# cremebrule/rgb-proprioceptive-pose-estimator

Hardware: AMD Instinct MI355X
Metric: images/sec (train step, 224x224 bs256 per GPU) (higher is better)
Workload: dtype bf16; 1 GPU; NaiveObjectStateEstimator train step (BASELINE.json configs[1]): ResNet-50 trunk + bn1 aux head + proprio MLP [1024,256,64] + PoseDistanceLoss(combined, alpha 0.5) + Adam; model=no, images_per_gpu=256, global_batch=256, resolution=224, latent_dim=512, parallelism=dp1, launch=eager, nan_loss_steps=0, params_finite=True

## Files before the change

### include/rpe_hip.h

```cpp
#ifndef RPE_HIP_H
#define RPE_HIP_H

#ifdef __cplusplus
extern "C" {
#endif

#define RPE_ABI_VERSION 3

enum { RPE_F32 = 0, RPE_BF16 = 1, RPE_F16 = 2 };
enum {
    RPE_OK = 0,
    RPE_ERR_SHAPE = 1,
    RPE_ERR_DTYPE = 2,
    RPE_ERR_ALIGN = 3,
    RPE_ERR_HIP = 4,
    RPE_ERR_WORKSPACE = 5,
    RPE_ERR_STATE = 6
};

int rpe_abi_version(void);
const char* rpe_build_id(void);
const char* rpe_last_error(void);

typedef struct {
// ... 57 lines not shown
                             const float* invstd, const float* mean, const float* c1c2, float* dw, void* scratch, long scratch_bytes, void* stream);
long rpe_conv1x1_dgrad_bn_t_workspace_bytes(const rpe_conv_desc* d, int P);
int rpe_conv1x1_dgrad_bn_t(const rpe_conv_desc* d, int dtype, const void* dy, const void* w_crsk, void* dz, const void* addend, const rpe_bn_bwd_epilogue* bn,
                           const void* a_prev, int P, float* t_out, void* workspace, long workspace_bytes, void* stream);
int rpe_bn_backward_coeffs_t(int dtype, const float* stats_part, int tiles, int C, long rows, const float* dzt_a, const void* w, int Ci, const float* mean,
                             const float* invstd, float* dgamma, float* dbeta, float* c1c2, double* dpart, void* stream);
int rpe_conv1x1_wgrad_combine(const rpe_conv_desc* d, const float* dzt_a, const float* gram, const float* w_master, const float* gamma, const float* invstd,
                              const float* mean, const float* c1c2, float* dw, void* stream);
int rpe_bn_backward_coeffs(const float* stats_part, int tiles, int C, long rows, float* dgamma, float* dbeta, float* c1c2, double* dpart, void* stream);
int rpe_bn_backward_apply_dz(int dtype, const void* dz, const void* y, const float* mean, const float* invstd, const float* gamma, const float* c1c2,
                             void* dy, long rows, int C, void* stream);
int rpe_conv2d_wgrad(const rpe_conv_desc* d, int dtype, const void* x, const void* dy, float* dw_krsc, void* stream);
long rpe_conv2d_wgrad_workspace_bytes(const rpe_conv_desc* d, int dtype);
int rpe_conv2d_wgrad_det(const rpe_conv_desc* d, int dtype, const void* x, const void* dy, float* dw_krsc, void* workspace, long workspace_bytes,
                         void* stream);

#define RPE_STEM_PAD 3
long rpe_x4_bytes(int dtype, int B, int H, int W);
int rpe_stem_conv_fwd(int dtype, const void* x4, const void* w_packed, void* y, float* stats_part, int B, int H, int W, void* stream);
int rpe_stem_conv_fwd_affine(int dtype, const void* x4, const void* w_packed, void* out, const float* bias, int relu, int B, int H, int W,
                             void* stream);
int rpe_stem_conv_wgrad(int dtype, const void* x4, const void* dy, float* dw_packed, int B, int H, int W, void* stream);
long rpe_stem_conv_wgrad_workspace_bytes(int dtype, int B, int H, int W);
int rpe_stem_conv_wgrad_det(int dtype, const void* x4, const void* dy, float* dw_packed, int B, int H, int W, void* workspace, long workspace_bytes,
                            void* stream);

int rpe_pack_conv_weight(int dtype, const float* w_krsc, void* w_fwd, void* w_dgrad, int Co, int R, int S, int Ci, void* stream);
typedef struct {
    const float* src;
    void* wf;
    void* wd;
    int Co, RS, Ci;
    int pad_;
    long start;
    const float* scale;
} rpe_pack_desc;
int rpe_pack_conv_weights_multi(int dtype, const rpe_pack_desc* table_dev, int nlayers, long total, void* stream);
int rpe_pack_stem_weight(int dtype, const float* w_oihw, const float* scale, void* out, void* stream);
int rpe_unpack_stem_grad(const float* d_packed, float* dw_oihw, void* stream);

int rpe_stage_image_nhwc4(int dtype, const float* img_nchw, void* out, int B, int H, int W, void* stream);

int rpe_stage_frames_u8(int dtype, const unsigned char* frames, void* out, int B, int Hs, int Ws, int H, int W, const float* mean3_host,
                        const float* std3_host, void* stream);
int rpe_stage_frames_u8_resized(int dtype, const unsigned char* frames, void* out, int B, int Hs, int Ws, int Hr, int Wr, int top, int left, int H, int W,
                                const int* xb, const int* xk, int ksx, const int* yb, const int* yk, int ksy, unsigned char* tmp, const float* mean3_host,
                                const float* std3_host, void* stream);

int rpe_stage_depth_f32_resized(const float* frames, float* out, int B, int Hs, int Ws, int Hr, int Wr, int top, int left, int H, int W,
                                const int* xb, const double* xk, int ksx, const int* yb, const double* yk, int ksy, void* stream);

typedef struct {
    unsigned long long seed;
    int qb_lo, qb_hi, qc_lo, qc_hi, qs_lo, qs_hi;
    int noise_q;
    unsigned erase_thresh;
    int eh_lo, eh_hi, ew_lo, ew_hi;
    int fill_mode;
    unsigned char fill_rgb[3];
    int group;
} rpe_augment_desc;
int rpe_augment_frames_u8(const unsigned char* in, unsigned char* out, int B, int Hs, int Ws, const rpe_augment_desc* d, unsigned* state, int* params,
                          unsigned long long* sums, void* stream);

typedef struct {
    unsigned long long seed;
    unsigned gauss_thresh, motion_thresh;
    int n_levels;
    int radius[8];
    int taps[8][9];
    int n_lengths;
    int n_dirs;
    int dir_cx[16], dir_cy[16];
    int group;
} rpe_blur_desc;
int rpe_blur_frames_u8(const unsigned char* in, unsigned char* out, int B, int Hs, int Ws, const rpe_blur_desc* d, const unsigned* state, int* params,
                       void* stream);

typedef struct {
    unsigned long long seed;
    int E, T, S, stride, N;
    int shuffle;
} rpe_sample_desc;
int rpe_sample_windows(const rpe_sample_desc* d, const int* sel, unsigned* state, int* index, void* stream);
int rpe_sample_windows_ragged(const rpe_sample_desc* d, const int* sel, const int* lengths, unsigned* state, int* index, void* stream);
int rpe_gather_rows(const void* pool, void* out, long row_bytes, long T, const int* index, int S, int N, void* stream);

typedef struct {
    unsigned long long seed;
    int S, N;
    int num_scales;
    double sigma[8];
    double rho;
} rpe_measure_desc;
int rpe_measurement_noise(const float* x0, float* out, const rpe_measure_desc* d, unsigned* state, int* picks, void* stream);

typedef struct {
    unsigned long long seed;
    double n0, n1, n2;
    double q, inv_q;
    double lo, hi;
    unsigned drop_thresh;
    int hole_lo, hole_hi;
    int hh_lo, hh_hi, hw_lo, hw_hi;
    float hole_value, occluder_value;
    int group;
} rpe_depth_augment_desc;
int rpe_augment_depth_f32(const float* in, float* out, int B, int Hs, int Ws, const rpe_depth_augment_desc* d, unsigned* state, int* params,
                          const int* rgb_params, int rgb_group, void* stream);

typedef struct {
    unsigned long long seed;
    unsigned thresh;
    float scale;
} rpe_dropout_desc;
int rpe_dropout_begin(unsigned* state, int* picks, void* stream);
int rpe_dropout_rows_f32(const float* x, float* out, long n, int ld, int c0, int c1, int site, const int* picks, const rpe_dropout_desc* d, void* stream);

#define RPE_BN_DPART_DOUBLES(C) ((long)RPE_BN_MAX_SLICES * 2 * (C) + 64)
#define RPE_BN_MAX_SLICES 256
int rpe_bn_finalize(const float* part, int tiles, int C, long count, const float* gamma, const float* beta, float* running_mean,
                    float* running_var, long long* num_batches, float momentum, float eps, float* scale, float* shift,
                    float* save_mean, float* save_invstd, double* dpart, void* stream);
int rpe_bn_eval_affine(int C, const float* gamma, const float* beta, const float* running_mean, const float* running_var, float eps,
                       float* scale, float* shift, void* stream);
int rpe_bn_apply(int dtype, const void* y, const void* residual, void* out, const float* scale, const float* shift, long rows, int C,
                 int relu, void* stream);
int rpe_bn_apply_mask(int dtype, const void* y, const void* residual, void* out, const float* scale, const float* shift, long rows, int C,
                      unsigned char* relu_mask, void* stream);
int rpe_bn_apply_res_bn(int dtype, const void* y, const void* res_y, const float* res_scale, const float* res_shift, void* out, const float* scale,
                        const float* shift, long rows, int C, int relu, unsigned char* relu_mask, void* stream);
int rpe_bn_backward(int dtype, const void* dA, const void* a_out, const void* y, const float* mean, const float* invstd,
                    const float* gamma, float* dgamma, float* dbeta, void* dy, void* dz_out, long rows, int C, float* part,
                    long part_floats, float* c1c2, double* dpart, void* stream);

int rpe_bn_backward_reduce(int dtype, const void* dA, const void* a_out, const void* y, const float* mean, const float* invstd, const float* gamma,
                           float* dgamma, float* dbeta, long rows, int C, float* part, long part_floats, float* c1c2, double* dpart, void* stream);
int rpe_bn_backward_from_dz(int dtype, const void* dz, const void* y, const float* mean, const float* invstd, const float* gamma,
                            const float* stats_part, int tiles, float* dgamma, float* dbeta, void* dy, long rows, int C, float* c1c2,
                            double* dpart, void* stream);

int rpe_maxpool3x3s2_fwd(int dtype, const void* x, void* out, unsigned char* idx, int B, int H, int W, int C, void* stream);
int rpe_bn_apply_maxpool3x3s2(int dtype, const void* y, const float* scale, const float* shift, void* a, void* out, unsigned char* idx, int B, int H,
                              int W, int C, void* stream);
int rpe_bn_apply_maxpool3x3s2_aux(int dtype, const void* y, const float* scale, const float* shift, void* a, void* out, unsigned char* idx, int B, int H,
                                  int W, const float* aux_w, const float* aux_bias, const float* depth_feat, float* aux_out, long ld_aux_out, float* aux_raw,
                                  unsigned char* aux_idx, void* stream);
int rpe_maxpool3x3s2_bwd(int dtype, const void* dout, const unsigned char* idx, const void* addend, void* dx, int B, int H, int W, int C,
                         void* stream);
int rpe_stem_bwd(int dtype, const void* dpool, const unsigned char* pool_idx, const void* y, const float* scale, const float* shift, const float* mean,
                 const float* invstd, const float* gamma, const float* aux_dout, long aux_ld, const float* aux_depth_feat,
                 const unsigned char* aux_idx, const float* aux_w, float* dgamma, float* dbeta, void* dy, int B, int H, int W, float* part,
                 long part_floats, float* c1c2, double* dpart, void* stream);
int rpe_avgpool_fwd(int dtype, const void* x, float* out, int B, int HW, int C, void* stream);
int rpe_avgpool_bwd(int dtype, const float* dout, void* dx, int B, int HW, int C, void* stream);

int rpe_aux_head_fwd(int dtype, const void* a1, const float* w, const float* bias, const float* depth_feat, float* out, long ld_out,
                     float* raw, unsigned char* idx, int B, int H, int W, void* stream);
int rpe_aux_head_bwd(int dtype, const float* dout, long ld_dout, const void* a1, const float* w, const float* depth_feat, const float* raw,
                     const unsigned char* idx, void* d_a1, float* dw, float* dbias, float* d_depth_feat, int B, int H, int W, void* stream);
long rpe_aux_head_bwd_workspace_floats(int dtype, int B, int H, int W);
int rpe_aux_head_bwd_det(int dtype, const float* dout, long ld_dout, const void* a1, const float* w, const float* depth_feat, const float* raw,
                         const unsigned char* idx, void* d_a1, float* dw, float* dbias, float* d_depth_feat, int B, int H, int W, float* workspace,
                         long workspace_floats, void* stream);
int rpe_aux_head_bwd_det_y(int dtype, const float* dout, long ld_dout, const void* y, const float* bn_scale, const float* bn_shift, const float* w,
                           const float* depth_feat, const float* raw, const unsigned char* idx, float* dw, float* dbias, float* d_depth_feat, int B, int H,
                           int W, float* workspace, long workspace_floats, void* stream);
int rpe_depth_head_fwd(const float* depth, const float* w, const float* b, float* feat, float* xhat, int B, int H, int W, void* stream);
int rpe_depth_head_bwd(const float* d_feat, const float* xhat, long n, float* dw, float* db, void* stream);
int rpe_aux_head_fwd_c(int dtype, const void* x, int C, const float* w, const float* bias, const float* depth_feat, float* out, long ld_out,
                       float* raw, unsigned char* idx, int B, int H, int W, void* stream);
int rpe_aux_head_bwd_c(int dtype, const float* dout, long ld_dout, const void* x, int C, const float* w, const float* depth_feat, const float* raw,
                       const unsigned char* idx, void* d_x, float* dw, float* dbias, float* d_depth_feat, int B, int H, int W, void* stream);
int rpe_depth_head_fwd_pools(const float* depth, const float* w, const float* b, float* feat, float* xhat, int B, int H, int W, int pools, void* stream);
int rpe_tensor_add(int dtype, void* dst, const void* src, long n, void* stream);

int rpe_feature_planes(int dtype, const void* x_nhwc, int image, int H, int W, int C, float* out_chw_f32, float* minmax, void* stream);
int rpe_feature_planes_batch(int dtype, const void* x_nhwc, int B, int H, int W, int C, float* out_bchw_f32, float* minmax, void* stream);
int rpe_feature_mosaic(const float* planes, const float* minmax, int C, int H, int W, int cols, int gutter, int flip_y, unsigned char* out_u8,
                       void* stream);

typedef struct {
    int Hs, Ws;
    int ph, pw;
    int sy, sx;
    unsigned char fill_rgb[3];
} rpe_occlusion_desc;
long rpe_occlusion_grid(const rpe_occlusion_desc* d, int* gy, int* gx);
int rpe_occlude_grid_u8(const unsigned char* frame, unsigned char* out, int B, int k0, const rpe_occlusion_desc* d, void* stream);
int rpe_pose_displacement(const float* pred, const float* ref, long n, float* pos, float* ori, void* stream);
int rpe_saliency_map(const float* scores, int M, const rpe_occlusion_desc* d, float* maps, float* minmax, void* stream);
int rpe_saliency_overlay_u8(const unsigned char* frame, const float* map, const float* minmax, const unsigned char* table, int Hs, int Ws,
                            int alpha_q8, int fade, unsigned char* out, void* stream);

#define RPE_OVERLAY_INVALID (-2147483647 - 1)
#define RPE_OVERLAY_NEAR 0.0009765625
#define RPE_OVERLAY_CLAMP_Q4 131072
#define RPE_OVERLAY_AXIS_Q4 8192
#define RPE_OVERLAY_MAX_SETS 4
#define RPE_OVERLAY_MAX_TRAIL 64
#define RPE_OVERLAY_MAX_RADIUS_Q4 256
#define RPE_OVERLAY_MAX_SIDE 4096
int rpe_project_poses(const float* poses, const double* cam, const int* cam_index, long F, int G, int C, double axis_len, const float* pos_err,
                      const float* ori_err, double pos_full, double ori_full, int width, int* points, int* bars, void* stream);
typedef struct {
    unsigned char rgb[3];
    unsigned char axis_rgb[9];
    int alpha_q8;
    int r_q4;
    int hw_q4;
    int trail;
    int trail_r_q4;
} rpe_overlay_style;
int rpe_draw_poses_u8(const unsigned char* frames, unsigned char* out, long n, int Hs, int Ws, const int* points, const int* bars, long first, int G,
                      const rpe_overlay_style* styles, int frames_per_episode, int bar_px, const unsigned char* bar_rgb, int flip, void* stream);

int rpe_linear_fwd(int dtype, const void* x, int ldx, const void* w, int ldw, const float* bias, void* y, int ldy, int M, int N, int K,
                   int relu, const void* addend, int ld_add, void* stream);
long rpe_linear_fwd_workspace_bytes(int dtype, int M, int N, int K);
int rpe_linear_fwd_ws(int dtype, const void* x, int ldx, const void* w, int ldw, const float* bias, void* y, int ldy, int M, int N, int K,
                      int relu, const void* addend, int ld_add, void* workspace, long workspace_bytes, void* stream);
int rpe_linear_wgrad(int dtype, const void* dy, int lddy, const void* x, int ldx, float* dw, int lddw, int M, int N, int K, void* stream);
long rpe_linear_wgrad_workspace_bytes(int dtype, int M, int N, int K);
int rpe_linear_wgrad_det(int dtype, const void* dy, int lddy, const void* x, int ldx, float* dw, int lddw, int M, int N, int K, int accumulate,
                         void* workspace, long workspace_bytes, void* stream);
int rpe_transpose_f32(const float* in, float* out, int rows, int cols, int ldi, int ldo, void* stream);
int rpe_relu_bwd(const float* out, const float* dy, float* dx, long n, void* stream);
int rpe_colsum(const float* x, long rows, int cols, int ld, float* out, int accumulate, void* stream);
int rpe_copy2d(const float* src, int ld_src, float* dst, int ld_dst, long rows, int cols, void* stream);

int rpe_lstm_cell_fwd(float* gates, const float* b_ih, const float* b_hh, const float* c_prev, float* c_out, float* h_out, int N, int Hd,
                      void* stream);
int rpe_lstm_cell_bwd(const float* gates_act, const float* c_prev, const float* c_cur, const float* dh, float* dc_io, float* dgates, int N,
                      int Hd, void* stream);

int rpe_pose_loss(const float* pred, const float* truth, long n, int metric, int mode, float scale, float alpha, float eps, float* out3,
                  float* grad, void* stream);

int rpe_pose_loss_masked(const float* pred, const float* truth, const unsigned char* valid, long n, int metric, int mode, float scale, float alpha,
                         float eps, float* out3, float* grad, void* stream);

int rpe_pose_errors(const float* pred, const float* truth, long n, float eps, float* pos_err, float* ori_err, float* pose_unit,
                    void* stream);

int rpe_error_stats(const float* err, int E, int T, double* out, void* stream);
int rpe_error_stats_ragged(const float* err, int E, int T, const int* lengths, double* out, void* stream);

int rpe_adam_step(float* p, const float* g, float* m, float* v, long n, double lr, double beta1, double beta2, double eps, int step,
                  void* stream);

int rpe_amp_unscale(float* grads, long n, float* state, void* stream);
int rpe_amp_update(float* state, float growth_factor, float backoff_factor, int growth_interval, void* stream);
int rpe_adam_step_amp(float* p, const float* g, float* m, float* v, long n, double lr, double beta1, double beta2, double eps, const float* state,
                      void* stream);

long rpe_grad_sumsq_rows(long n);
int rpe_grad_sumsq(const float* g, long n, double* partials, void* stream);
int rpe_clip_coef(const double* partials, long rows, double max_norm, float* state, void* stream);
int rpe_adamw_step_clip(float* p, const float* g, float* m, float* v, long n, double lr, double beta1, double beta2, double eps,
                        double weight_decay, const float* state, int use_clip, void* stream);

int rpe_lr_schedule(const float* state, int kind, long warmup_steps, double warmup_start_factor, long total_steps, double min_factor,
                    long step_size, double gamma, float* sched, void* stream);
int rpe_adamw_step_sched(float* p, const float* g, float* m, float* v, float* ema, long n, double lr, double beta1, double beta2, double eps,
                         double weight_decay, double ema_decay, const float* state, const float* sched, int use_clip, void* stream);
int rpe_swap_f32(float* a, float* b, long n, void* stream);

#define RPE_PARAM_STATS_COLS 10
#define RPE_PARAM_STATS_PART_COLS 8
long rpe_param_stats_rows(long numel);
int rpe_param_stats(const float* p, const float* g, const float* m, const float* v, const long* table, const long* table_host, int T,
                    double* partials, double beta1, double beta2, double eps, const float* state, long every, void* stream);
int rpe_param_stats_finalize(const double* partials, const long* table, int T, double* out, const float* state, long every, void* stream);

typedef struct rpe_resnet50 rpe_resnet50_t;

#define RPE_RESNET50_NUM_CONV 53
#define RPE_RESNET50_NUM_PARAMS 161
#define RPE_RESNET50_NUM_BUFFERS 106

int rpe_resnet50_create(rpe_resnet50_t** out, int batch, int height, int width, int dtype, int latent_dim);
int rpe_resnet_create(rpe_resnet50_t** out, int depth, int batch, int height, int width, int dtype, int latent_dim);
void rpe_resnet50_destroy(rpe_resnet50_t* e);
long rpe_resnet50_workspace_bytes(const rpe_resnet50_t* e);
const char* rpe_resnet50_param_name(const rpe_resnet50_t* e, int i);
long rpe_resnet50_param_numel(const rpe_resnet50_t* e, int i);
int rpe_resnet50_bind(rpe_resnet50_t* e, void* workspace, long workspace_bytes, float* const* params_host, float* const* grads_host,
                      float* const* running_host, long long* const* num_batches_host);
int rpe_resnet50_pack_weights(rpe_resnet50_t* e, void* stream);
int rpe_resnet50_weights_changed(rpe_resnet50_t* e);
int rpe_resnet50_side_stream_info(const rpe_resnet50_t* e, int* candidates, int* concurrent);
int rpe_resnet50_set_aux_head(rpe_resnet50_t* e, const float* w, const float* bias, const float* depth_feat, float* out, long ld_out, float* raw,
                              unsigned char* idx);
int rpe_resnet50_aux_head_bwd(rpe_resnet50_t* e, const float* dout, long ld_dout, const float* w, const float* depth_feat, const float* raw,
                              const unsigned char* idx, float* dw, float* dbias, float* d_depth_feat, float* workspace, long workspace_floats, void* stream);
int rpe_resnet50_forward(rpe_resnet50_t* e, const float* img_nchw, float* features, long ld_features, int training, void* stream);
int rpe_resnet50_forward_u8(rpe_resnet50_t* e, const unsigned char* frames, int Hs, int Ws, const float* mean3_host, const float* std3_host,
                            float* features, long ld_features, int training, void* stream);
typedef struct {
    int Hr, Wr, top, left, ksx, ksy;
    const int *xb, *xk, *yb, *yk;
    unsigned char* tmp;
} rpe_resize_plan;
int rpe_resnet50_forward_u8_resized(rpe_resnet50_t* e, const unsigned char* frames, int Hs, int Ws, const rpe_resize_plan* rs, const float* mean3_host,
                                    const float* std3_host, float* features, long ld_features, int training, void* stream);
const void* rpe_resnet50_early_feature(const rpe_resnet50_t* e);
// ... 25 lines not shown
```

### rgb-proprioceptive-pose-estimator_amd/_lib.py

```python
import ctypes
import os

import torch
from ctypes import POINTER, Structure, c_char_p, c_double, c_float, c_int, c_long, c_void_p

_HERE = os.path.dirname(os.path.abspath(__file__))
LIB_PATH = os.environ.get("RPE_LIB_PATH") or os.path.join(_HERE, "librpe_hip.so")

RPE_F32, RPE_BF16, RPE_F16 = 0, 1, 2
ABI_VERSION = 3
PARAM_STATS_COLS, PARAM_STATS_PART_COLS = 10, 8


class RpeError(RuntimeError):
    """A librpe_hip.so entry point returned a non-zero status."""


class BnBwdEpilogue(Structure):
    _fields_ = [(n, c_void_p) for n in ("y", "a_out", "mean", "invstd", "scale", "shift", "stats_part", "a_mask")]


class ResizePlan(Structure):
    _fields_ = [(n, c_int) for n in ("Hr", "Wr", "top", "left", "ksx", "ksy")] + [(n, c_void_p) for n in ("xb", "xk", "yb", "yk", "tmp")]


class ConvDesc(Structure):
    _fields_ = [(n, c_int) for n in ("batch", "in_h", "in_w", "in_c", "out_c", "kh", "kw", "stride", "pad")]


class PackDesc(Structure):
    _fields_ = [("src", c_void_p), ("wf", c_void_p), ("wd", c_void_p), ("Co", c_int), ("RS", c_int), ("Ci", c_int), ("pad_", c_int), ("start", c_long),
                ("scale", c_void_p)]


class AugmentDesc(Structure):
    _fields_ = ([("seed", ctypes.c_ulonglong)] + [(n, c_int) for n in ("qb_lo", "qb_hi", "qc_lo", "qc_hi", "qs_lo", "qs_hi", "noise_q")]
                + [("erase_thresh", ctypes.c_uint)] + [(n, c_int) for n in ("eh_lo", "eh_hi", "ew_lo", "ew_hi", "fill_mode")]
                + [("fill_rgb", ctypes.c_ubyte * 3), ("group", c_int)])


class BlurDesc(Structure):
    _fields_ = [("seed", ctypes.c_ulonglong), ("gauss_thresh", ctypes.c_uint), ("motion_thresh", ctypes.c_uint), ("n_levels", c_int), ("radius", c_int * 8),
                ("taps", (c_int * 9) * 8), ("n_lengths", c_int), ("n_dirs", c_int), ("dir_cx", c_int * 16), ("dir_cy", c_int * 16), ("group", c_int)]


class SampleDesc(Structure):
    _fields_ = [("seed", ctypes.c_ulonglong)] + [(n, c_int) for n in ("E", "T", "S", "stride", "N", "shuffle")]


class MeasureDesc(Structure):
    _fields_ = [("seed", ctypes.c_ulonglong)] + [(n, c_int) for n in ("S", "N", "num_scales")] + [("sigma", c_double * 8), ("rho", c_double)]


class DropoutDesc(Structure):
    _fields_ = [("seed", ctypes.c_ulonglong), ("thresh", ctypes.c_uint), ("scale", c_float)]


class DepthAugmentDesc(Structure):
    _fields_ = ([("seed", ctypes.c_ulonglong)] + [(n, c_double) for n in ("n0", "n1", "n2", "q", "inv_q", "lo", "hi")] + [("drop_thresh", ctypes.c_uint)]
                + [(n, c_int) for n in ("hole_lo", "hole_hi", "hh_lo", "hh_hi", "hw_lo", "hw_hi")] + [("hole_value", c_float), ("occluder_value", c_float),
                                                                                                       ("group", c_int)])


class OcclusionDesc(Structure):
    _fields_ = [(n, c_int) for n in ("Hs", "Ws", "ph", "pw", "sy", "sx")] + [("fill_rgb", ctypes.c_ubyte * 3)]


class OverlayStyle(Structure):
    _fields_ = [("rgb", ctypes.c_ubyte * 3), ("axis_rgb", ctypes.c_ubyte * 9)] + [(n, c_int) for n in ("alpha_q8", "r_q4", "hw_q4", "trail", "trail_r_q4")]


OVERLAY_INVALID, OVERLAY_NEAR, OVERLAY_CLAMP_Q4, OVERLAY_AXIS_Q4 = -2 ** 31, 2.0 ** -10, 2 ** 17, 2 ** 13
OVERLAY_MAX_SETS, OVERLAY_MAX_TRAIL, OVERLAY_MAX_RADIUS_Q4, OVERLAY_MAX_SIDE = 4, 64, 256, 4096

P, I, L, F, D = c_void_p, c_int, c_long, c_float, c_double
PD = POINTER(ConvDesc)

_SPEC = {
    "rpe_abi_version": (I, []),
    "rpe_last_error": (c_char_p, []),
    "rpe_build_id": (c_char_p, []),
    "rpe_x4_bytes": (L, [I, I, I, I]),
    "rpe_conv_out_hw": (I, [PD, POINTER(c_int), POINTER(c_int)]),
    "rpe_conv_stats_tiles": (L, [L]),
    "rpe_conv2d_fwd": (I, [PD, I, P, P, P, P, P]),
    "rpe_conv2d_fwd_affine": (I, [PD, I, P, P, P, P, P, I, P]),
    "rpe_conv2d_fwd_affine_workspace_bytes": (L, [PD, I]),
    "rpe_conv2d_fwd_affine_ws": (I, [PD, I, P, P, P, P, P, I, P, L, P]),
    "rpe_conv2d_dgrad": (I, [PD, I, P, P, P, P, P]),
    "rpe_conv2d_dgrad_stats_tiles": (L, [PD, I]),
    "rpe_conv2d_fwd_stats_tiles": (L, [PD, I]),
    "rpe_conv2d_dgrad_bn": (I, [PD, I, P, P, P, P, POINTER(BnBwdEpilogue), P]),
    "rpe_conv1x1s2_dgrad_compact": (I, [PD, I, P, P, P, P]),
    "rpe_conv2d_dgrad_sub": (I, [PD, I, P, P, P, P, P]),
    "rpe_conv2d_dgrad_bn_sub": (I, [PD, I, P, P, P, P, POINTER(BnBwdEpilogue), P]),
    "rpe_conv1x1_dgrad_kcat_y_sub": (I, [PD, I, P, P, P, P, P, P, POINTER(BnBwdEpilogue), P]),
    "rpe_bn_backward_reduce": (I, [I, P, P, P, P, P, P, P, P, L, I, P, L, P, P, P]),
    "rpe_bn_backward_from_dz": (I, [I, P, P, P, P, P, P, I, P, P, P, L, I, P, P, P]),
    "rpe_bn_bwd_fold_scratch_bytes": (L, [I, I, I]),
    "rpe_bn_bwd_fold_conv1x1": (I, [I, I, I, P, P, P, P, P, P, P, P, P, L, P]),
    "rpe_conv1x1_dgrad_kcat": (I, [PD, I, P, P, P, P, P, POINTER(BnBwdEpilogue), P]),
    "rpe_bn_bwd_fold_y_conv1x1": (I, [I, I, I, P, P, P, P, P, P, P, P]),
    "rpe_conv1x1_dgrad_kcat_y": (I, [PD, I, P, P, P, P, P, P, POINTER(BnBwdEpilogue), P]),
    "rpe_conv1x1_wgrad_folded_y_scratch_bytes": (L, [PD, I]),
    "rpe_conv1x1_wgrad_folded_y": (I, [PD, I, P, P, P, P, P, P, P, P, P, L, P]),
    "rpe_conv1x1_wgrad_folded_scratch_bytes": (L, [PD, I]),
    "rpe_conv1x1_wgrad_folded": (I, [PD, I, P, P, P, P, P, P, P, P, P, L, P]),
    "rpe_bn_backward_coeffs": (I, [P, I, I, L, P, P, P, P, P]),
    "rpe_bn_backward_apply_dz": (I, [I, P, P, P, P, P, P, P, L, I, P]),
    "rpe_conv2d_wgrad": (I, [PD, I, P, P, P, P]),
    "rpe_conv2d_wgrad_workspace_bytes": (L, [PD, I]),
    "rpe_conv2d_wgrad_det": (I, [PD, I, P, P, P, P, L, P]),
    "rpe_stem_conv_fwd": (I, [I, P, P, P, P, I, I, I, P]),
    "rpe_stem_conv_fwd_affine": (I, [I, P, P, P, P, I, I, I, I, P]),
    "rpe_stem_conv_wgrad": (I, [I, P, P, P, I, I, I, P]),
    "rpe_stem_conv_wgrad_workspace_bytes": (L, [I, I, I, I]),
    "rpe_stem_conv_wgrad_det": (I, [I, P, P, P, I, I, I, P, L, P]),
    "rpe_pack_conv_weight": (I, [I, P, P, P, I, I, I, I, P]),
    "rpe_pack_conv_weights_multi": (I, [I, P, I, L, P]),
    "rpe_pack_stem_weight": (I, [I, P, P, P, P]),
    "rpe_unpack_stem_grad": (I, [P, P, P]),
    "rpe_stage_image_nhwc4": (I, [I, P, P, I, I, I, P]),
    "rpe_stage_frames_u8": (I, [I, P, P, I, I, I, I, I, POINTER(c_float), POINTER(c_float), P]),
    "rpe_stage_frames_u8_resized": (I, [I, P, P, I, I, I, I, I, I, I, I, I, P, P, I, P, P, I, P, POINTER(c_float), POINTER(c_float), P]),
    "rpe_stage_depth_f32_resized": (I, [P, P, I, I, I, I, I, I, I, I, I, P, P, I, P, P, I, P]),
    "rpe_augment_frames_u8": (I, [P, P, I, I, I, POINTER(AugmentDesc), P, P, P, P]),
    "rpe_blur_frames_u8": (I, [P, P, I, I, I, POINTER(BlurDesc), P, P, P]),
    "rpe_augment_depth_f32": (I, [P, P, I, I, I, POINTER(DepthAugmentDesc), P, P, P, I, P]),
    "rpe_sample_windows": (I, [POINTER(SampleDesc), P, P, P, P]),
    "rpe_sample_windows_ragged": (I, [POINTER(SampleDesc), P, P, P, P, P]),
    "rpe_gather_rows": (I, [P, P, L, L, P, I, I, P]),
    "rpe_measurement_noise": (I, [P, P, POINTER(MeasureDesc), P, P, P]),
    "rpe_dropout_begin": (I, [P, P, P]),
    "rpe_dropout_rows_f32": (I, [P, P, L, I, I, I, I, P, POINTER(DropoutDesc), P]),
    "rpe_bn_finalize": (I, [P, I, I, L, P, P, P, P, P, F, F, P, P, P, P, P, P]),
    "rpe_bn_eval_affine": (I, [I, P, P, P, P, F, P, P, P]),
    "rpe_bn_apply": (I, [I, P, P, P, P, P, L, I, I, P]),
    "rpe_bn_apply_mask": (I, [I, P, P, P, P, P, L, I, P, P]),
    "rpe_conv1x1_dgrad_bn_t_workspace_bytes": (L, [PD, I]),
    "rpe_conv1x1_dgrad_bn_t": (I, [PD, I, P, P, P, P, POINTER(BnBwdEpilogue), P, I, P, P, L, P]),
    "rpe_bn_backward_coeffs_t": (I, [I, P, I, I, L, P, P, I, P, P, P, P, P, P, P]),
    "rpe_conv1x1_wgrad_combine": (I, [PD, P, P, P, P, P, P, P, P, P]),
    "rpe_bn_apply_gram_workspace_bytes": (L, [I, L, I]),
    "rpe_bn_apply_gram": (I, [I, P, P, P, P, L, I, P, P, L, P]),
    "rpe_gram_ones_row": (L, [I]),
    "rpe_gram_workspace_bytes": (L, [I, L, I]),
    "rpe_gram": (I, [I, P, L, I, P, P, L, P]),
    "rpe_bn_stats_from_gram": (I, [I, P, I, I, P, I, L, P, P, P, P, P, c_float, c_float, P, P, P, P, P]),
    "rpe_conv1x1_fwd_bn": (I, [PD, I, P, P, P, P, P, P, P, P, P, P, P]),
    "rpe_bn_apply_res_bn": (I, [I, P, P, P, P, P, P, P, L, I, I, P, P]),
    "rpe_bn_backward": (I, [I, P, P, P, P, P, P, P, P, P, P, L, I, P, L, P, P, P]),
    "rpe_maxpool3x3s2_fwd": (I, [I, P, P, P, I, I, I, I, P]),
    "rpe_bn_apply_maxpool3x3s2": (I, [I, P, P, P, P, P, P, I, I, I, I, P]),
    "rpe_maxpool3x3s2_bwd": (I, [I, P, P, P, P, I, I, I, I, P]),
    "rpe_stem_bwd": (I, [I, P, P, P, P, P, P, P, P, P, L, P, P, P, P, P, P, I, I, I, P, L, P, P, P]),
    "rpe_avgpool_fwd": (I, [I, P, P, I, I, I, P]),
    "rpe_avgpool_bwd": (I, [I, P, P, I, I, I, P]),
    "rpe_aux_head_fwd": (I, [I, P, P, P, P, P, L, P, P, I, I, I, P]),
    "rpe_aux_head_bwd": (I, [I, P, L, P, P, P, P, P, P, P, P, P, I, I, I, P]),
    "rpe_aux_head_bwd_workspace_floats": (L, [I, I, I, I]),
    "rpe_aux_head_bwd_det": (I, [I, P, L, P, P, P, P, P, P, P, P, P, I, I, I, P, L, P]),
    "rpe_depth_head_fwd": (I, [P, P, P, P, P, I, I, I, P]),
    "rpe_depth_head_bwd": (I, [P, P, L, P, P, P]),
    "rpe_linear_fwd": (I, [I, P, I, P, I, P, P, I, I, I, I, I, P, I, P]),
    "rpe_linear_fwd_workspace_bytes": (L, [I, I, I, I]),
    "rpe_linear_fwd_ws": (I, [I, P, I, P, I, P, P, I, I, I, I, I, P, I, P, L, P]),
    "rpe_linear_wgrad": (I, [I, P, I, P, I, P, I, I, I, I, P]),
    "rpe_linear_wgrad_workspace_bytes": (L, [I, I, I, I]),
    "rpe_linear_wgrad_det": (I, [I, P, I, P, I, P, I, I, I, I, I, P, L, P]),
    "rpe_transpose_f32": (I, [P, P, I, I, I, I, P]),
    "rpe_relu_bwd": (I, [P, P, P, L, P]),
    "rpe_colsum": (I, [P, L, I, I, P, I, P]),
    "rpe_copy2d": (I, [P, I, P, I, L, I, P]),
    "rpe_lstm_cell_fwd": (I, [P, P, P, P, P, P, I, I, P]),
    "rpe_lstm_cell_bwd": (I, [P, P, P, P, P, P, I, I, P]),
    "rpe_pose_loss": (I, [P, P, L, I, I, F, F, F, P, P, P]),
    "rpe_pose_loss_masked": (I, [P, P, P, L, I, I, F, F, F, P, P, P]),
    "rpe_pose_errors": (I, [P, P, L, F, P, P, P, P]),
    "rpe_error_stats": (I, [P, I, I, P, P]),
    "rpe_error_stats_ragged": (I, [P, I, I, P, P, P]),
    "rpe_adam_step": (I, [P, P, P, P, L, D, D, D, D, I, P]),
    "rpe_amp_unscale": (I, [P, L, P, P]),
    "rpe_amp_update": (I, [P, F, F, I, P]),
    "rpe_adam_step_amp": (I, [P, P, P, P, L, D, D, D, D, P, P]),
    "rpe_grad_sumsq_rows": (L, [L]),
    "rpe_grad_sumsq": (I, [P, L, P, P]),
    "rpe_clip_coef": (I, [P, L, D, P, P]),
    "rpe_adamw_step_clip": (I, [P, P, P, P, L, D, D, D, D, D, P, I, P]),
    "rpe_lr_schedule": (I, [P, I, L, D, L, D, L, D, P, P]),
    "rpe_adamw_step_sched": (I, [P, P, P, P, P, L, D, D, D, D, D, D, P, P, I, P]),
    "rpe_swap_f32": (I, [P, P, L, P]),
    "rpe_param_stats_rows": (L, [L]),
    "rpe_param_stats": (I, [P, P, P, P, P, P, I, P, D, D, D, P, L, P]),
    "rpe_param_stats_finalize": (I, [P, P, I, P, P, L, P]),
    "rpe_resnet50_create": (I, [POINTER(c_void_p), I, I, I, I, I]),
    "rpe_resnet_create": (I, [POINTER(c_void_p), I, I, I, I, I, I]),
    "rpe_resnet50_destroy": (None, [P]),
    "rpe_resnet50_workspace_bytes": (L, [P]),
    "rpe_resnet50_param_name": (c_char_p, [P, I]),
    "rpe_resnet50_param_numel": (L, [P, I]),
    "rpe_resnet50_bind": (I, [P, P, L, POINTER(c_void_p), POINTER(c_void_p), POINTER(c_void_p), POINTER(c_void_p)]),
    "rpe_resnet50_pack_weights": (I, [P, P]),
    "rpe_resnet50_weights_changed": (I, [P]),
    "rpe_resnet50_forward": (I, [P, P, P, L, I, P]),
    "rpe_resnet50_forward_u8": (I, [P, P, I, I, POINTER(c_float), POINTER(c_float), P, L, I, P]),
    "rpe_resnet50_forward_u8_resized": (I, [P, P, I, I, POINTER(ResizePlan), POINTER(c_float), POINTER(c_float), P, L, I, P]),
    "rpe_resnet50_early_feature": (c_void_p, [P]),
    "rpe_resnet50_early_grad": (c_void_p, [P]),
    "rpe_resnet50_backward": (I, [P, P, L, I, P]),
    "rpe_resnet50_profile": (I, [P, I]),
    "rpe_resnet50_profile_read": (I, [P, POINTER(c_float), POINTER(c_int), POINTER(c_double), POINTER(c_double)]),
    "rpe_resnet50_backward_begin": (I, [P, P, L, P]),
    "rpe_resnet50_backward_blocks": (I, [P, I, I, P]),
    "rpe_resnet50_backward_end": (I, [P, I, P]),
    "rpe_resnet50_backward_frozen": (I, [P, P, L, P]),
    "rpe_resnet50_set_aux_grad": (I, [P, P, L, P, P, P]),
    "rpe_resnet50_profile_kernels": (L, [P, P, L]),
    "rpe_last_kernel_name": (c_char_p, []),
    "rpe_set_walk_direction": (None, [I]),
    "rpe_conv2d_wgrad_halo_min_width": (I, [I]),
    "rpe_resnet50_set_aux_head": (I, [P, P, P, P, P, L, P, P]),
    "rpe_resnet50_aux_head_bwd": (I, [P, P, L, P, P, P, P, P, P, P, P, L, P]),
    "rpe_aux_head_bwd_det_y": (I, [I, P, L, P, P, P, P, P, P, P, P, P, P, I, I, I, P, L, P]),
    "rpe_bn_apply_maxpool3x3s2_aux": (I, [I, P, P, P, P, P, P, I, I, I, P, P, P, P, L, P, P, P]),
    "rpe_resnet50_side_stream_info": (I, [P, POINTER(c_int), POINTER(c_int)]),
    "rpe_resnet50_tensor": (I, [P, c_char_p, POINTER(c_void_p), POINTER(c_long), POINTER(c_int)]),
    "rpe_resnet50_set_hook_grad": (I, [P, I, P]),
    "rpe_resnet50_set_stem_raw": (I, [P, I]),
    "rpe_aux_head_fwd_c": (I, [I, P, I, P, P, P, P, L, P, P, I, I, I, P]),
    "rpe_aux_head_bwd_c": (I, [I, P, L, P, I, P, P, P, P, P, P, P, P, I, I, I, P]),
    "rpe_depth_head_fwd_pools": (I, [P, P, P, P, P, I, I, I, I, P]),
    "rpe_tensor_add": (I, [I, P, P, L, P]),
    "rpe_feature_planes": (I, [I, P, I, I, I, I, P, P, P]),
    "rpe_feature_planes_batch": (I, [I, P, I, I, I, I, P, P, P]),
    "rpe_feature_mosaic": (I, [P, P, I, I, I, I, I, I, P, P]),
    "rpe_occlusion_grid": (L, [POINTER(OcclusionDesc), POINTER(c_int), POINTER(c_int)]),
    "rpe_occlude_grid_u8": (I, [P, P, I, I, POINTER(OcclusionDesc), P]),
    "rpe_pose_displacement": (I, [P, P, L, P, P, P]),
    "rpe_saliency_map": (I, [P, I, POINTER(OcclusionDesc), P, P, P]),
    "rpe_saliency_overlay_u8": (I, [P, P, P, P, I, I, I, I, P, P]),
    "rpe_project_poses": (I, [P, P, P, L, I, I, D, P, P, D, D, I, P, P, P]),
    "rpe_draw_poses_u8": (I, [P, P, L, I, I, P, P, L, I, POINTER(OverlayStyle), I, I, POINTER(ctypes.c_ubyte), I, P]),
}
_NOT_STATUS = {"rpe_abi_version", "rpe_conv2d_wgrad_halo_min_width", "rpe_grad_sumsq_rows", "rpe_param_stats_rows"}

EXPORTS = tuple(_SPEC)


def _load():
    if not os.path.exists(LIB_PATH):
        raise ImportError(
            "librpe_hip.so not found at %s -- build it with `python __graft_entry__.py build` "
            "(hipcc --offload-arch=gfx950); there is no fallback path." % LIB_PATH
        )
    lib = ctypes.CDLL(LIB_PATH)
    for name, (res, args) in _SPEC.items():
        try:
            fn = getattr(lib, name)
        except AttributeError as e:
            raise ImportError("librpe_hip.so does not export %s (stale build?)" % name) from e
        fn.restype = res
        fn.argtypes = args
    if lib.rpe_abi_version() != ABI_VERSION:
        raise ImportError("librpe_hip.so ABI version %d != expected %d" % (lib.rpe_abi_version(), ABI_VERSION))
    return lib


_raw = _load()


class _Checked:

    def __getattr__(self, name):
        fn = getattr(_raw, name)
        res = _SPEC[name][0]
        if res is I and name not in _NOT_STATUS:

            def call(*a, _fn=fn, _name=name):
                rc = _fn(*a)
                if rc != 0:
                    raise RpeError("%s failed (%d): %s" % (_name, rc, _raw.rpe_last_error().decode()))
                return 0

            setattr(self, name, call)
            return call
        setattr(self, name, fn)
        return fn


lib = _Checked()
raw = _raw
```

### rgb-proprioceptive-pose-estimator_amd/csrc/engine.hip

```cpp
#include <stdlib.h>
#include <string.h>

#include <string>
#include <vector>

#include "common.h"

using namespace rpe;

namespace {

struct ConvL {
    std::string name, bn;
    rpe_conv_desc d;
    int Ho, Wo;
    long rows;
    int p_w, p_g, p_b;
    int bn_i;
    void* wf = nullptr;
    void* wd = nullptr;
    void* y = nullptr;
    void* a = nullptr;
    void* dy = nullptr;
    float *scale = nullptr, *shift = nullptr, *mean = nullptr, *invstd = nullptr;
    float* c1c2 = nullptr;
};

struct Block {
    int c1, c2, c3, cd;
    int out = -1;
    int layer = 0;
    bool first = false;
    void* dz = nullptr;
    float* gram = nullptr;
    float* dzt_a = nullptr;
    bool t_ready = false;
    unsigned char* relu_mask = nullptr;
};

struct Named {
    std::string name;
    const void* ptr;
    long rows;
    int ch;
};

}

struct rpe_resnet50 {
    int B, H, W, dtype, latent;
    int feat = 2048;
    bool basic = false;
    size_t esz;
    std::vector<ConvL> convs;
    std::vector<Block> blocks;
    std::vector<std::string> pnames;
    std::vector<long> pnumel;
    std::vector<float*> params, grads, running;
    std::vector<long long*> nbt;
    bool bound = false, fwd_done = false;
    long ws_bytes = 0;
    char* ws = nullptr;
    struct Slot { void** dst; long bytes; };
    std::vector<Slot> slots;
    void* x4 = nullptr;
    void* pool = nullptr;
    unsigned char* pool_idx = nullptr;
    float* pooled = nullptr;
    float* d_pooled = nullptr;
    float* fc_wt = nullptr;
    int latent_pad = 0;
    void* early_grad = nullptr;
    void* G[2] = {nullptr, nullptr};
    void* d_pool = nullptr;
    float* stats_part = nullptr;
    float* stats_part2 = nullptr;
    long stats_floats = 0;
    float* bwd_part = nullptr;
    long bwd_part_floats = 0;
    float* c1c2 = nullptr;
    double* dpart = nullptr;
    double* dpart2 = nullptr;
    const float* aux_dout = nullptr; long aux_ld = 0; const float* aux_df = nullptr; const unsigned char* aux_idx = nullptr; const float* aux_w = nullptr;
    struct { const float *w = nullptr, *bias = nullptr, *depth_feat = nullptr; float* out = nullptr; long ld = 0; float* raw = nullptr; unsigned char* idx = nullptr; } aux_fwd;
    bool a1_valid = false;
    float* stem_dw = nullptr;
    bool fold = true;
    void* w_kcat = nullptr;
    float* fold_bias = nullptr;
    void* fold_scratch = nullptr;
    long fold_scratch_bytes = 0;
    void* wfold_scratch = nullptr;
    long wfold_scratch_bytes = 0;
    bool fold1 = false;
    int fold1_max = 128;
    bool fold_w = true;
    int fold_w_max = 256;
    void* main_slab = nullptr;
    long main_slab_bytes = 0;
    void* wg_slab = nullptr;
    long wg_slab_bytes = 0;
    std::vector<Named> named;
    int train_mode = 0;
    int fused_tiles = 0;
    int bwd_next = -2;
    rpe_pack_desc* pack_tab = nullptr;
    const void* hook_grad[4] = {nullptr, nullptr, nullptr, nullptr};
    bool stem_raw = false;
    void* fc_ws = nullptr;
    long fc_ws_bytes = 0;
    bool y3free = false;
    bool y3_keep = false;
    bool t_fused = false;
    bool apply_gram = true;
    int y3free_max = 128;
    void* gram_ws = nullptr;
    long gram_ws_bytes = 0;
    void* sk_ws = nullptr;
    long sk_ws_bytes = 0;
    rpe_pack_desc* pack_tab_fold = nullptr;
    int pack_state = 0;
    long pack_total = 0;
    char* gspan_lo = nullptr;
    size_t gspan_bytes = 0;
    bool profiling = false;
    struct Span { int cat; hipEvent_t a, b; int name_id; double flops, bytes; };
    std::vector<std::string> kernel_names;
    double pending_flops = 0, pending_bytes = 0;
    std::vector<Span> spans;
    std::vector<hipEvent_t> ev_pool;
    size_t ev_next = 0;
    hipEvent_t cur_a = nullptr;
    int cur_cat = 0;
    hipStream_t side = nullptr;
    bool overlap = true;
    int side_tries = 0;
    int side_concurrent = -1;
    std::vector<hipStream_t> side_rejects;
    bool capturing = false;
    bool walk_alt = getenv("RPE_NO_WALK_ALT") == nullptr;
    int walk_next = 0;
    std::vector<hipEvent_t> sync_pool;
    size_t sync_next = 0;
    double flops[RPE_PROF_NUM] = {0};
    double bytes[RPE_PROF_NUM] = {0};
};

extern "C" const char* rpe_last_kernel_name(void);
static int kernel_id(rpe_resnet50* e) {
    const char* n = rpe_last_kernel_name();
    for (size_t i = 0; i < e->kernel_names.size(); ++i)
        if (e->kernel_names[i] == n) return (int)i;
    e->kernel_names.push_back(n);
    return (int)e->kernel_names.size() - 1;
}

static hipEvent_t next_event(rpe_resnet50* e) {
    if (e->ev_next == e->ev_pool.size()) {
        hipEvent_t ev;
        if (hipEventCreate(&ev) != hipSuccess) return nullptr;
        e->ev_pool.push_back(ev);
    }
    return e->ev_pool[e->ev_next++];
}

static void prof_close(rpe_resnet50* e, hipStream_t s, bool reopen) {
    hipEvent_t b = next_event(e);
    if (!e->cur_a || !b) { e->cur_a = nullptr; return; }
    (void)hipEventRecord(b, s);
    e->spans.push_back({e->cur_cat, e->cur_a, b, kernel_id(e), e->pending_flops, e->pending_bytes});
    e->pending_flops = 0; e->pending_bytes = 0;
    e->cur_a = reopen ? b : nullptr;
}
static void prof_hook_split(void* ctx, hipStream_t s) { prof_close((rpe_resnet50*)ctx, s, true); }
#define PROF(e, cat, stream, call)                                                   \
    do {                                                                             \
        if ((e)->profiling) { (e)->cur_a = next_event(e); (e)->cur_cat = (cat);      \
            if ((e)->cur_a) (void)hipEventRecord((e)->cur_a, (hipStream_t)(stream)); \
            rpe::g_prof_hook = {prof_hook_split, (e)}; }                             \
        const int err__ = (call);                                                    \
        rpe::g_prof_hook = {nullptr, nullptr};                                       \
        if (err__) return err__;                                                     \
        if ((e)->profiling) prof_close((e), (hipStream_t)(stream), false);           \
    } while (0)

struct WalkScope {
    rpe_resnet50* e; bool alt; int mode0, next0;
    WalkScope(rpe_resnet50* e_, bool alt_) : e(e_), alt(alt_ && e_->walk_alt), mode0(rpe::g_walk_mode), next0(rpe::g_walk_next) {
        rpe::g_walk_mode = alt ? 2 : 0;
        if (alt) rpe::g_walk_next = e->walk_next;
    }
    ~WalkScope() {
        if (alt) e->walk_next = rpe::g_walk_next;
        rpe::g_walk_mode = mode0; rpe::g_walk_next = next0;
    }
};

static int add_conv(rpe_resnet50* e, const std::string& name, const std::string& bn, int in_h, int in_w, int in_c, int out_c, int k,
                    int stride, int pad) {
    ConvL c;
    c.name = name; c.bn = bn;
    c.d = rpe_conv_desc{e->B, in_h, in_w, in_c, out_c, k, k, stride, pad};
    c.Ho = (in_h + 2 * pad - k) / stride + 1;
    c.Wo = (in_w + 2 * pad - k) / stride + 1;
    c.rows = (long)e->B * c.Ho * c.Wo;
    c.bn_i = (int)e->convs.size();
    c.p_w = (int)e->pnames.size();
    e->pnames.push_back(name + ".weight"); e->pnumel.push_back((long)out_c * in_c * k * k);
    c.p_g = (int)e->pnames.size();
    e->pnames.push_back(bn + ".weight"); e->pnumel.push_back(out_c);
    c.p_b = (int)e->pnames.size();
    e->pnames.push_back(bn + ".bias"); e->pnumel.push_back(out_c);
    e->convs.push_back(c);
    return (int)e->convs.size() - 1;
}

static void want(rpe_resnet50* e, void** dst, long bytes) {
    bytes = (bytes + 255) / 256 * 256;
    e->slots.push_back({dst, bytes});
    e->ws_bytes += bytes;
}

extern "C" int rpe_resnet_create(rpe_resnet50_t** out, int depth, int batch, int height, int width, int dtype, int latent_dim);
extern "C" int rpe_resnet50_create(rpe_resnet50_t** out, int batch, int height, int width, int dtype, int latent_dim) {
    return rpe_resnet_create(out, 50, batch, height, width, dtype, latent_dim);
}

extern "C" int rpe_resnet_create(rpe_resnet50_t** out, int depth, int batch, int height, int width, int dtype, int latent_dim) {
    if (!out) return rpe_set_error(RPE_ERR_SHAPE, "resnet50_create: null out");
    if (depth != 18 && depth != 34 && depth != 50 && depth != 101 && depth != 152)
        return rpe_set_error(RPE_ERR_SHAPE, "resnet_create: depth must be 18, 34 (BasicBlock) or 50, 101, 152 (bottleneck)");
    if (batch <= 0 || latent_dim <= 0) return rpe_set_error(RPE_ERR_SHAPE, "resnet50_create: bad batch/latent");
    if (height < 32 || width < 32 || (height % 32) || (width % 32)) return rpe_set_error(RPE_ERR_SHAPE, "resnet50_create: H, W must be multiples of 32");
    if (dtype != RPE_F32 && dtype != RPE_BF16 && dtype != RPE_F16) return rpe_set_error(RPE_ERR_DTYPE, "resnet50_create: dtype must be RPE_F32, RPE_BF16 or RPE_F16");
    rpe_resnet50* e = new rpe_resnet50();
    e->B = batch; e->H = height; e->W = width; e->dtype = dtype; e->latent = latent_dim;
    e->esz = dtype == RPE_F32 ? 4 : 2;
    e->basic = depth == 18 || depth == 34;
    e->feat = e->basic ? 512 : 2048;
    add_conv(e, "conv1", "bn1", height, width, 3, 64, 7, 2, 3);
    int h = e->convs[0].Ho / 2, w = e->convs[0].Wo / 2;
    int inpl = 64;
    const int planes[4] = {64, 128, 256, 512}, strides[4] = {1, 2, 2, 2};
    const int nblk18[4] = {2, 2, 2, 2};
    const int nblk50[4] = {3, depth == 152 ? 8 : 4, (depth == 50 || depth == 34) ? 6 : (depth == 101 ? 23 : 36), 3};
    const int* nblk = depth == 18 ? nblk18 : nblk50;
    for (int li = 0; li < 4; ++li) {
        for (int b = 0; b < nblk[li]; ++b) {
            const std::string p = "layer" + std::to_string(li + 1) + "." + std::to_string(b);
            const int s = b == 0 ? strides[li] : 1;
            Block blk;
            blk.layer = li + 1; blk.first = b == 0;
            if (e->basic) {
                blk.c1 = add_conv(e, p + ".conv1", p + ".bn1", h, w, inpl, planes[li], 3, s, 1);
                const int h2 = e->convs[blk.c1].Ho, w2 = e->convs[blk.c1].Wo;
                blk.c2 = add_conv(e, p + ".conv2", p + ".bn2", h2, w2, planes[li], planes[li], 3, 1, 1);
                blk.c3 = -1; blk.cd = -1; blk.out = blk.c2;
                if (b == 0 && (s != 1 || inpl != planes[li])) blk.cd = add_conv(e, p + ".downsample.0", p + ".downsample.1", h, w, inpl, planes[li], 1, s, 0);
                e->blocks.push_back(blk);
                inpl = planes[li];
                h = h2; w = w2;
                continue;
            }
            blk.c1 = add_conv(e, p + ".conv1", p + ".bn1", h, w, inpl, planes[li], 1, 1, 0);
            blk.c2 = add_conv(e, p + ".conv2", p + ".bn2", h, w, planes[li], planes[li], 3, s, 1);
            const int h2 = e->convs[blk.c2].Ho, w2 = e->convs[blk.c2].Wo;
            blk.c3 = add_conv(e, p + ".conv3", p + ".bn3", h2, w2, planes[li], planes[li] * 4, 1, 1, 0);
            blk.cd = -1; blk.out = blk.c3;
            if (b == 0) blk.cd = add_conv(e, p + ".downsample.0", p + ".downsample.1", h, w, inpl, planes[li] * 4, 1, s, 0);
            e->blocks.push_back(blk);
            inpl = planes[li] * 4;
            h = h2; w = w2;
        }
    }
    e->pnames.push_back("fc.weight"); e->pnumel.push_back((long)latent_dim * e->feat);
    e->pnames.push_back("fc.bias"); e->pnumel.push_back(latent_dim);
    e->latent_pad = (latent_dim + 3) / 4 * 4;

    const size_t es = e->esz;
    want(e, &e->x4, rpe_x4_bytes(dtype, batch, height, width));
    long max_act = 0;
    for (auto& c : e->convs) {
        const long n = c.rows * c.d.out_c;
        if (n > max_act) max_act = n;
        want(e, &c.y, n * es);
        want(e, &c.a, n * es);
        want(e, &c.dy, n * es);
        const long wn = (long)c.d.out_c * c.d.kh * c.d.kw * c.d.in_c;
        if (&c == &e->convs[0]) {
            want(e, &c.wf, 64L * 256 * es);
        } else {
            want(e, &c.wf, wn * es);
            want(e, &c.wd, wn * es);
        }
        want(e, (void**)&c.scale, c.d.out_c * 4L);
        want(e, (void**)&c.shift, c.d.out_c * 4L);
        want(e, (void**)&c.mean, c.d.out_c * 4L);
        want(e, (void**)&c.invstd, c.d.out_c * 4L);
        want(e, (void**)&c.c1c2, 2L * c.d.out_c * 4);
        const long sf = (rpe_conv2d_fwd_stats_tiles(&c.d, dtype) + 2) * 2 * c.d.out_c;
        if (sf > e->stats_floats) e->stats_floats = sf;
        const long sf2 = (rpe_conv2d_dgrad_stats_tiles(&c.d, dtype) + 4) * 2 * c.d.in_c;
        if (sf2 > e->stats_floats) e->stats_floats = sf2;
    }
    const ConvL& st = e->convs[0];
    const long pool_n = (long)batch * (st.Ho / 2) * (st.Wo / 2) * 64;
    want(e, &e->pool, pool_n * es);
    want(e, (void**)&e->pool_idx, pool_n);
    want(e, (void**)&e->pooled, (long)batch * e->feat * 4);
    want(e, (void**)&e->d_pooled, (long)batch * e->feat * 4);
    want(e, (void**)&e->fc_wt, (long)e->feat * e->latent_pad * 4);
    want(e, &e->early_grad, st.rows * 64 * es);
    for (int i = 0; i < 2; ++i) want(e, &e->G[i], max_act * es);
    for (auto& b : e->blocks) {
        const ConvL& c3 = e->convs[b.out];
        want(e, &b.dz, c3.rows * c3.d.out_c * es);
        if (dtype != RPE_F32) want(e, (void**)&b.relu_mask, c3.rows * c3.d.out_c / 8);
    }
    want(e, &e->d_pool, (long)batch * (e->convs[0].Ho / 2) * (e->convs[0].Wo / 2) * 64 * es);
    want(e, (void**)&e->stats_part, e->stats_floats * 4);
    want(e, (void**)&e->stats_part2, e->stats_floats * 4);
    e->bwd_part_floats = 1024L * 2 * 2048;
    want(e, (void**)&e->bwd_part, e->bwd_part_floats * 4);
    want(e, (void**)&e->c1c2, 2 * 2048 * 4L);
    want(e, (void**)&e->dpart, RPE_BN_DPART_DOUBLES(2048) * 8);
    want(e, (void**)&e->dpart2, RPE_BN_DPART_DOUBLES(2048) * 8);
    want(e, (void**)&e->stem_dw, 64L * 256 * 4);
    e->fold = !e->basic && getenv("RPE_NO_BN_FOLD") == nullptr;
    if (e->fold) {
        long wk = 0;
        for (auto& b : e->blocks) {
            const rpe_conv_desc& d = e->convs[b.c3].d;
            const long sb = rpe_bn_bwd_fold_scratch_bytes(dtype, d.out_c, d.in_c);
            if (sb > e->fold_scratch_bytes) e->fold_scratch_bytes = sb;
            const long w = (long)d.in_c * (d.out_c + d.in_c) * (long)es;
            if (w > wk) wk = w;
            const rpe_conv_desc& d1 = e->convs[b.c1].d;
            const long w1 = (long)d1.in_c * 2 * d1.out_c * (long)es;
            if (w1 > wk) wk = w1;
        }
        e->fold1 = getenv("RPE_BN1_FOLD") != nullptr;
        if (getenv("RPE_BN1_FOLD_MAX")) e->fold1_max = atoi(getenv("RPE_BN1_FOLD_MAX"));
        e->fold_w = getenv("RPE_NO_WGRAD_FOLD") == nullptr;
        if (e->fold_w) {
            if (getenv("RPE_WGRAD_FOLD_MAX")) e->fold_w_max = atoi(getenv("RPE_WGRAD_FOLD_MAX"));
            for (auto& b : e->blocks) {
                if (e->convs[b.c3].d.in_c > e->fold_w_max) continue;
                const long sb = rpe_conv1x1_wgrad_folded_scratch_bytes(&e->convs[b.c3].d, dtype);
                if (sb > e->wfold_scratch_bytes) e->wfold_scratch_bytes = sb;
            }
            if (e->fold1)
                for (auto& b : e->blocks) {
                    if (e->convs[b.c1].d.out_c > e->fold1_max) continue;
                    const long sb = rpe_conv1x1_wgrad_folded_y_scratch_bytes(&e->convs[b.c1].d, dtype);
                    if (sb > e->wfold_scratch_bytes) e->wfold_scratch_bytes = sb;
                }
            if (e->wfold_scratch_bytes > 0) want(e, &e->wfold_scratch, e->wfold_scratch_bytes);
        }
        want(e, &e->w_kcat, wk);
        want(e, (void**)&e->fold_bias, 2048L * 4);
        want(e, &e->fold_scratch, e->fold_scratch_bytes);
    }
    e->y3free = dtype != RPE_F32 && e->fold && e->fold_w && !e->fold1 && !getenv("RPE_NO_Y3FREE") && !getenv("RPE_NO_RELU_MASK") &&
                !getenv("RPE_WGRAD_ATOMIC");
    long y3_slab = 0;
    if (e->y3free) {
        if (getenv("RPE_Y3FREE_MAX")) e->y3free_max = atoi(getenv("RPE_Y3FREE_MAX"));
        e->y3_keep = getenv("RPE_Y3_KEEP") != nullptr;
        e->apply_gram = getenv("RPE_NO_APPLY_GRAM") == nullptr;
        e->t_fused = getenv("RPE_T_FUSE") != nullptr;
        for (auto& b : e->blocks) {
            const ConvL& c3 = e->convs[b.c3];
            if (c3.d.in_c > e->y3free_max || c3.d.in_c > 256 || (c3.d.in_c % 64)) continue;
            want(e, (void**)&b.gram, (long)(rpe_gram_ones_row(c3.d.in_c) + 1) * c3.d.in_c * 4);
            want(e, (void**)&b.dzt_a, (long)c3.d.out_c * c3.d.in_c * 4);
            const long wsb = rpe_gram_workspace_bytes(dtype, c3.rows, c3.d.in_c);
            if (wsb > e->gram_ws_bytes) e->gram_ws_bytes = wsb;
            const long wsb2 = rpe_bn_apply_gram_workspace_bytes(dtype, c3.rows, c3.d.in_c);
            if (wsb2 > e->gram_ws_bytes) e->gram_ws_bytes = wsb2;
            const long tb = rpe_conv2d_wgrad_workspace_bytes(&c3.d, dtype);
            if (tb > y3_slab) y3_slab = tb;
            rpe_conv_desc dn = c3.d; dn.in_c = c3.d.out_c; dn.out_c = c3.d.in_c;
            const long tb2 = rpe_conv1x1_dgrad_bn_t_workspace_bytes(&dn, c3.d.in_c);
            if (tb2 > y3_slab) y3_slab = tb2;
        }
        if (e->gram_ws_bytes > 0) want(e, &e->gram_ws, e->gram_ws_bytes);
    }
    if (!getenv("RPE_WGRAD_ATOMIC")) {
        for (size_t i = 1; i < e->convs.size(); ++i) {
            const long b = rpe_conv2d_wgrad_workspace_bytes(&e->convs[i].d, dtype);
            if (b > e->wg_slab_bytes) e->wg_slab_bytes = b;
        }
        if (e->wg_slab_bytes > 0) want(e, &e->wg_slab, e->wg_slab_bytes);
        e->main_slab_bytes = rpe_stem_conv_wgrad_workspace_bytes(dtype, batch, height, width);
        const long fcb = rpe_linear_wgrad_workspace_bytes(RPE_F32, batch, latent_dim, e->feat);
        if (fcb > e->main_slab_bytes) e->main_slab_bytes = fcb;
        if (y3_slab > e->main_slab_bytes) e->main_slab_bytes = y3_slab;
        if (e->main_slab_bytes > 0) want(e, &e->main_slab, e->main_slab_bytes);
    }
    {
        const long f = rpe_linear_fwd_workspace_bytes(RPE_F32, batch, latent_dim, e->feat), d = rpe_linear_fwd_workspace_bytes(RPE_F32, batch, e->feat, e->latent_pad);
        e->fc_ws_bytes = f > d ? f : d;
        if (e->fc_ws_bytes > 0 && getenv("RPE_NO_LINEAR_SPLITK") == nullptr) want(e, &e->fc_ws, e->fc_ws_bytes);
    }
    if (getenv("RPE_NO_SPLITK") == nullptr) {
        for (size_t i = 1; i < e->convs.size(); ++i) {
            const long sb = rpe_conv2d_fwd_affine_workspace_bytes(&e->convs[i].d, dtype);
            if (sb > e->sk_ws_bytes) e->sk_ws_bytes = sb;
        }
        if (e->sk_ws_bytes > 0) want(e, &e->sk_ws, e->sk_ws_bytes);
    }
    want(e, (void**)&e->pack_tab, (long)(e->convs.size() + 8) * sizeof(rpe_pack_desc));
    want(e, (void**)&e->pack_tab_fold, (long)(e->convs.size() + 8) * sizeof(rpe_pack_desc));
    for (auto& c : e->convs) {
        const double mnk = 2.0 * (double)c.rows * c.d.out_c * (double)(c.d.kh * c.d.kw * c.d.in_c);
        const double in_b = (double)batch * c.d.in_h * c.d.in_w * c.d.in_c * es, out_b = (double)c.rows * c.d.out_c * es;
        e->flops[RPE_PROF_CONV_FWD] += mnk;   e->bytes[RPE_PROF_CONV_FWD] += in_b + out_b;
        e->flops[RPE_PROF_CONV_WGRAD] += mnk; e->bytes[RPE_PROF_CONV_WGRAD] += in_b + out_b;
        if (&c != &e->convs[0]) { e->flops[RPE_PROF_CONV_DGRAD] += mnk; e->bytes[RPE_PROF_CONV_DGRAD] += in_b + out_b; }
        e->bytes[RPE_PROF_BN_FWD] += 2 * out_b;
        e->bytes[RPE_PROF_BN_BWD] += 3 * out_b;
    }
    *out = e;
    return 0;
}

extern "C" int rpe_resnet50_profile(rpe_resnet50_t* e, int enable) {
    if (!e) return rpe_set_error(RPE_ERR_STATE, "resnet50_profile: null engine");
    e->profiling = enable != 0;
    e->spans.clear();
    e->ev_next = 0;
    return 0;
}

extern "C" int rpe_resnet50_profile_read(rpe_resnet50_t* e, float* ms, int* launches, double* flops, double* bytes) {
    if (!e) return rpe_set_error(RPE_ERR_STATE, "resnet50_profile_read: null engine");
    for (int i = 0; i < RPE_PROF_NUM; ++i) { ms[i] = 0.f; launches[i] = 0; flops[i] = e->flops[i]; bytes[i] = e->bytes[i]; }
    for (auto& sp : e->spans) {
        if (hipError_t he = hipEventSynchronize(sp.b)) return rpe_set_error_hip(he, __FILE__, __LINE__);
        float t = 0.f;
        if (hipError_t he = hipEventElapsedTime(&t, sp.a, sp.b)) return rpe_set_error_hip(he, __FILE__, __LINE__);
        ms[sp.cat] += t;
        launches[sp.cat] += 1;
    }
    return 0;
}

extern "C" long rpe_resnet50_profile_kernels(rpe_resnet50_t* e, char* buf, long buflen) {
    if (!e || !buf || buflen <= 0) return -1;
    const size_t nk = e->kernel_names.size();
    std::vector<double> ms(nk, 0.0), fl(nk, 0.0), by(nk, 0.0);
    std::vector<int> cnt(nk, 0);
    for (auto& sp : e->spans) {
        if (sp.name_id < 0 || (size_t)sp.name_id >= nk) continue;
        if (hipEventSynchronize(sp.b) != hipSuccess) return -1;
        float t = 0.f;
        if (hipEventElapsedTime(&t, sp.a, sp.b) != hipSuccess) return -1;
        ms[sp.name_id] += t; fl[sp.name_id] += sp.flops; by[sp.name_id] += sp.bytes; cnt[sp.name_id] += 1;
    }
    long off = 0;
    for (size_t i = 0; i < nk; ++i) {
        if (!cnt[i]) continue;
        const int w = snprintf(buf + off, (size_t)(buflen - off), "%s;%d;%.6f;%.0f;%.0f\n", e->kernel_names[i].c_str(), cnt[i], ms[i], fl[i], by[i]);
        if (w < 0 || off + w >= buflen) break;
        off += w;
    }
    return off;
}

extern "C" void rpe_resnet50_destroy(rpe_resnet50_t* e) {
    if (!e) return;
    for (auto ev : e->ev_pool) (void)hipEventDestroy(ev);
    for (auto ev : e->sync_pool) (void)hipEventDestroy(ev);
    if (e->side) (void)hipStreamDestroy(e->side);
    for (auto st : e->side_rejects) (void)hipStreamDestroy(st);
    delete e;
}
extern "C" long rpe_resnet50_workspace_bytes(const rpe_resnet50_t* e) { return e ? e->ws_bytes : 0; }
extern "C" const char* rpe_resnet50_param_name(const rpe_resnet50_t* e, int i) {
    return (e && i >= 0 && i < (int)e->pnames.size()) ? e->pnames[i].c_str() : nullptr;
}
extern "C" long rpe_resnet50_param_numel(const rpe_resnet50_t* e, int i) {
    return (e && i >= 0 && i < (int)e->pnumel.size()) ? e->pnumel[i] : -1;
}

extern "C" int rpe_resnet50_bind(rpe_resnet50_t* e, void* workspace, long workspace_bytes, float* const* params_host, float* const* grads_host,
                                 float* const* running_host, long long* const* num_batches_host) {
    if (!e || !workspace || !params_host) return rpe_set_error(RPE_ERR_SHAPE, "resnet50_bind: null argument");
    if (workspace_bytes < e->ws_bytes) return rpe_set_error(RPE_ERR_WORKSPACE, "resnet50_bind: workspace smaller than rpe_resnet50_workspace_bytes()");
    if (((uintptr_t)workspace) & 255) return rpe_set_error(RPE_ERR_ALIGN, "resnet50_bind: workspace must be 256-byte aligned");
    e->ws = (char*)workspace;
    char* p = e->ws;
    for (auto& s : e->slots) { *s.dst = p; p += s.bytes; }
    const int np = (int)e->pnames.size(), nb = (int)e->convs.size();
    e->params.assign(params_host, params_host + np);
    if (grads_host) e->grads.assign(grads_host, grads_host + np); else e->grads.assign(np, nullptr);
    if (running_host) e->running.assign(running_host, running_host + 2 * nb); else e->running.assign(2 * nb, nullptr);
    if (num_batches_host) e->nbt.assign(num_batches_host, num_batches_host + nb); else e->nbt.assign(nb, nullptr);
    for (int i = 0; i < np; ++i)
        if (!e->params[i] || (((uintptr_t)e->params[i]) & 15)) return rpe_set_error(RPE_ERR_ALIGN, "resnet50_bind: parameter pointers must be non-null and 16-byte aligned");
    e->named.clear();
    for (auto& c : e->convs) {
        e->named.push_back({c.name + ".y", c.y, c.rows, c.d.out_c});
        e->named.push_back({c.name + ".a", c.a, c.rows, c.d.out_c});
    }
    e->named.push_back({"pool", e->pool, (long)e->B * (e->convs[0].Ho / 2) * (e->convs[0].Wo / 2), 64});
    e->named.push_back({"x4", e->x4, (long)e->B * (e->H + 2 * RPE_STEM_PAD) * (e->W + 2 * RPE_STEM_PAD), 4});
    for (int i = 0; i < 2; ++i) e->named.push_back({"G" + std::to_string(i), e->G[i], 0, 0});
    {
        std::vector<rpe_pack_desc> tab;
        long start = 0;
        for (size_t i = 1; i < e->convs.size(); ++i) {
            ConvL& c = e->convs[i];
            rpe_pack_desc d;
            d.src = e->params[c.p_w];
            d.wf = e->dtype == RPE_F32 ? nullptr : c.wf;
            d.wd = c.wd;
            d.Co = c.d.out_c; d.RS = c.d.kh * c.d.kw; d.Ci = c.d.in_c; d.pad_ = 0;
            d.scale = nullptr;
            d.start = start;
            start += (long)d.Co * d.RS * d.Ci;
            tab.push_back(d);
        }
        e->pack_total = start;
        if (hipError_t he = hipMemcpy(e->pack_tab, tab.data(), tab.size() * sizeof(rpe_pack_desc), hipMemcpyHostToDevice))
            return rpe_set_error_hip(he, __FILE__, __LINE__);
        for (size_t i = 1; i < e->convs.size(); ++i) {
            ConvL& c = e->convs[i];
            tab[i - 1].wf = c.wf;
            tab[i - 1].wd = nullptr;
            tab[i - 1].scale = c.scale;
        }
        if (hipError_t he = hipMemcpy(e->pack_tab_fold, tab.data(), tab.size() * sizeof(rpe_pack_desc), hipMemcpyHostToDevice))
            return rpe_set_error_hip(he, __FILE__, __LINE__);
        e->pack_state = 0;
        if (hipError_t he = hipMemset(e->x4, 0, (size_t)rpe_x4_bytes(e->dtype, e->B, e->H, e->W))) return rpe_set_error_hip(he, __FILE__, __LINE__);
        if (hipError_t he = hipMemset(e->dpart, 0, 64 * sizeof(double))) return rpe_set_error_hip(he, __FILE__, __LINE__);
        if (hipError_t he = hipMemset(e->dpart2, 0, 64 * sizeof(double))) return rpe_set_error_hip(he, __FILE__, __LINE__);
    }
    e->gspan_lo = nullptr; e->gspan_bytes = 0;
    if (grads_host) {
        char *lo = nullptr, *hi = nullptr;
        size_t sum = 0;
        bool ok = true;
        for (int i = 0; i < np; ++i) {
            if (!e->grads[i]) { ok = false; break; }
            char* a = (char*)e->grads[i];
            char* b = a + (size_t)e->pnumel[i] * 4;
            if (!lo || a < lo) lo = a;
            if (!hi || b > hi) hi = b;
// ... 42 lines not shown

static double conv_in_bytes(const rpe_resnet50* e, const ConvL& c) { return (double)c.d.batch * c.d.in_h * c.d.in_w * c.d.in_c * e->esz; }
static double conv_out_bytes(const rpe_resnet50* e, const ConvL& c) { return (double)c.rows * c.d.out_c * e->esz; }
static double conv_flops(const ConvL& c) { return 2.0 * (double)c.rows * c.d.out_c * (double)(c.d.kh * c.d.kw * c.d.in_c); }

static const void* fwd_weight(rpe_resnet50* e, ConvL& c) {
    return (e->dtype == RPE_F32 && &c != &e->convs[0] && e->train_mode) ? (const void*)e->params[c.p_w] : c.wf;
}

static int fold_for_eval(rpe_resnet50* e, void* stream) {
    for (auto& c : e->convs) {
        float* rm = e->running[2 * c.bn_i];
        float* rv = e->running[2 * c.bn_i + 1];
        if (!rm || !rv) return rpe_set_error(RPE_ERR_STATE, "resnet50_forward: eval mode needs running statistics");
        TRY(rpe_bn_eval_affine(c.d.out_c, e->params[c.p_g], e->params[c.p_b], rm, rv, 1e-5f, c.scale, c.shift, stream));
    }
    TRY(rpe_pack_stem_weight(e->dtype, e->params[e->convs[0].p_w], e->stem_raw ? nullptr : e->convs[0].scale, e->convs[0].wf, stream));
    TRY(rpe_pack_conv_weights_multi(e->dtype, e->pack_tab_fold, (int)e->convs.size() - 1, e->pack_total, stream));
    e->pack_state = 2;
    return 0;
}

extern char** environ;
static bool profiler_attached() {
    const char* pre = getenv("LD_PRELOAD");
    if (pre && (strstr(pre, "rocprof") || strstr(pre, "rocprofiler"))) return true;
    for (char** e = environ; e && *e; ++e)
        if (!strncmp(*e, "ROCPROF", 7) || !strncmp(*e, "ROCP_TOOL", 9)) return true;
    return false;
}
__global__ void side_probe_spin_kernel(long ticks) {
    const long t0 = wall_clock64();
    while (wall_clock64() - t0 < ticks) __builtin_amdgcn_s_sleep(16);
}
__global__ void side_probe_empty_kernel() {}
static int side_probe(hipStream_t caller, hipStream_t cand) {
    hipEvent_t spin_done = nullptr, cand_done = nullptr;
    if (hipEventCreateWithFlags(&spin_done, hipEventDisableTiming) != hipSuccess || hipEventCreateWithFlags(&cand_done, hipEventDisableTiming) != hipSuccess) return -1;
    int res = -1;
    hipLaunchKernelGGL(side_probe_spin_kernel, dim3(1), dim3(64), 0, caller, 20000L);
    if (hipEventRecord(spin_done, caller) == hipSuccess) {
        hipLaunchKernelGGL(side_probe_empty_kernel, dim3(1), dim3(64), 0, cand);
        if (hipEventRecord(cand_done, cand) == hipSuccess && hipEventSynchronize(cand_done) == hipSuccess) {
            const hipError_t q = hipEventQuery(spin_done);
            res = q == hipErrorNotReady ? 1 : (q == hipSuccess ? 0 : -1);
        }
    }
    (void)hipEventSynchronize(spin_done);
    (void)hipGetLastError();
    (void)hipEventDestroy(spin_done);
    (void)hipEventDestroy(cand_done);
    return res;
}

static int ensure_side(rpe_resnet50* e, hipStream_t caller = nullptr) {
    if (e->overlap && !e->side) {
        if (getenv("RPE_NO_OVERLAP")) e->overlap = false;
        else {
            int least = 0, greatest = 0;
            HIPTRY(hipDeviceGetStreamPriorityRange(&least, &greatest));
            static const bool low = getenv("RPE_SIDE_LOW_PRIO") != nullptr;
            const int skip = getenv("RPE_TEST_STREAM_SKIP") ? atoi(getenv("RPE_TEST_STREAM_SKIP")) : 0;
            for (int i = 0; i < skip; ++i) { hipStream_t d; HIPTRY(hipStreamCreateWithFlags(&d, hipStreamNonBlocking)); }
            static const bool no_probe = getenv("RPE_NO_SIDE_PROBE") != nullptr || profiler_attached();
            for (int t = 0; t < 4 && !e->side; ++t) {
                hipStream_t cand = nullptr;
                HIPTRY(hipStreamCreateWithPriority(&cand, hipStreamNonBlocking, low ? least : 0));
                e->side_tries = t + 1;
                const int r = (no_probe || e->capturing) ? -1 : side_probe(caller, cand);
                if (r != 0 || t == 3) { e->side = cand; e->side_concurrent = r; }
                else e->side_rejects.push_back(cand);
            }
        }
    }
    return 0;
}

static int conv_bn(rpe_resnet50* e, ConvL& c, const void* x, const void* residual, int relu, void* stream, bool second_set = false,
                   unsigned char* relu_mask = nullptr, const ConvL* res_bn = nullptr, bool stats_only = false, float* gram_out = nullptr) {
    const bool train = e->train_mode != 0;
    float* stats = second_set ? e->stats_part2 : e->stats_part;
    double* dpart = second_set ? e->dpart2 : e->dpart;
    e->pending_flops = conv_flops(c);
    e->pending_bytes = conv_in_bytes(e, c) + conv_out_bytes(e, c);
    if (!train) {
        if (&c == &e->convs[0] && e->stem_raw) {
            PROF(e, RPE_PROF_CONV_FWD, stream, rpe_stem_conv_fwd(e->dtype, x, c.wf, c.y, nullptr, e->B, e->H, e->W, stream));
            PROF(e, RPE_PROF_BN_FWD, stream, rpe_bn_apply(e->dtype, c.y, nullptr, c.a, c.scale, c.shift, c.rows, c.d.out_c, relu, stream));
        } else
        if (&c == &e->convs[0]) PROF(e, RPE_PROF_CONV_FWD, stream, rpe_stem_conv_fwd_affine(e->dtype, x, c.wf, c.a, c.shift, relu, e->B, e->H, e->W, stream));
        else if (e->sk_ws && !second_set)
            PROF(e, RPE_PROF_CONV_FWD, stream, rpe_conv2d_fwd_affine_ws(&c.d, e->dtype, x, c.wf, c.a, c.shift, residual, relu, e->sk_ws, e->sk_ws_bytes, stream));
        else PROF(e, RPE_PROF_CONV_FWD, stream, rpe_conv2d_fwd_affine(&c.d, e->dtype, x, c.wf, c.a, c.shift, residual, relu, stream));
        return 0;
    }
    if (&c == &e->convs[0]) PROF(e, RPE_PROF_CONV_FWD, stream, rpe_stem_conv_fwd(e->dtype, x, c.wf, c.y, stats, e->B, e->H, e->W, stream));
    else PROF(e, RPE_PROF_CONV_FWD, stream, rpe_conv2d_fwd(&c.d, e->dtype, x, fwd_weight(e, c), c.y, stats, stream));
    float* rm = e->running[2 * c.bn_i];
    float* rv = e->running[2 * c.bn_i + 1];
    e->pending_bytes = 0;
    PROF(e, RPE_PROF_BN_FWD, stream, rpe_bn_finalize(stats, (int)rpe_conv2d_fwd_stats_tiles(&c.d, e->dtype), c.d.out_c, c.rows, e->params[c.p_g], e->params[c.p_b], rm, rv,
                        e->nbt[c.bn_i], 0.1f, 1e-5f, c.scale, c.shift, c.mean, c.invstd, dpart, stream));
    if (stats_only) return 0;
    e->pending_bytes = conv_out_bytes(e, c) * (2.0 + (residual ? 1.0 : 0.0) + ((relu_mask && relu) ? 1.0 / 16 : 0.0));
    if (res_bn) {
        PROF(e, RPE_PROF_BN_FWD, stream, rpe_bn_apply_res_bn(e->dtype, c.y, res_bn->y, res_bn->scale, res_bn->shift, c.a, c.scale, c.shift, c.rows, c.d.out_c, relu,
                                                            relu ? relu_mask : nullptr, stream));
        return 0;
    }
    if (gram_out) {
        if (residual || !relu) return rpe_set_error(RPE_ERR_STATE, "trunk engine: the fused apply + Gram pass takes no residual");
        PROF(e, RPE_PROF_BN_FWD, stream, rpe_bn_apply_gram(e->dtype, c.y, c.a, c.scale, c.shift, c.rows, c.d.out_c, gram_out, e->gram_ws, e->gram_ws_bytes, stream));
        return 0;
    }
    if (relu_mask && relu) PROF(e, RPE_PROF_BN_FWD, stream, rpe_bn_apply_mask(e->dtype, c.y, residual, c.a, c.scale, c.shift, c.rows, c.d.out_c, relu_mask, stream));
    else PROF(e, RPE_PROF_BN_FWD, stream, rpe_bn_apply(e->dtype, c.y, residual, c.a, c.scale, c.shift, c.rows, c.d.out_c, relu, stream));
    return 0;
}

static int capture_guard(rpe_resnet50* e, void* stream, const char* who) {
    hipStreamCaptureStatus st = hipStreamCaptureStatusNone;
    if (hipStreamIsCapturing((hipStream_t)stream, &st) != hipSuccess) { (void)hipGetLastError(); e->capturing = false; return 0; }
    e->capturing = st != hipStreamCaptureStatusNone;
    if (!e->capturing) return 0;
    if (e->profiling) return rpe_set_error(RPE_ERR_STATE, "trunk engine: per-launch profiling events cannot be recorded inside a stream capture");
    if (e->overlap && !e->side && !getenv("RPE_NO_OVERLAP")) {
        char msg[160];
        snprintf(msg, sizeof(msg), "%s: called under stream capture before any eager pass created the second stream -- run the step eagerly once, then capture", who);
        return rpe_set_error(RPE_ERR_STATE, msg);
    }
    return 0;
}

static int forward_impl(rpe_resnet50_t* e, const float* img_nchw, const unsigned char* frames, int Hs, int Ws, const float* mean3, const float* std3,
                        float* features, long ld_features, int training, void* stream, const rpe_resize_plan* rs = nullptr) {
    if (!e || !e->bound) return rpe_set_error(RPE_ERR_STATE, "resnet50_forward: engine not bound");
    if ((!img_nchw && !frames) || !features || ld_features < e->latent) return rpe_set_error(RPE_ERR_SHAPE, "resnet50_forward: bad img/features");
    TRY(capture_guard(e, stream, "resnet50_forward"));
    e->train_mode = training;
    if (training) e->walk_next = 0;
    WalkScope walk(e, training != 0);
    if (training && e->pack_state != 1) TRY(rpe_resnet50_pack_weights(e, stream));
    if (!training && e->pack_state != 2) TRY(fold_for_eval(e, stream));
    if (frames && rs) PROF(e, RPE_PROF_OTHER, stream, rpe_stage_frames_u8_resized(e->dtype, frames, e->x4, e->B, Hs, Ws, rs->Hr, rs->Wr, rs->top, rs->left, e->H, e->W,
                                                                                    rs->xb, rs->xk, rs->ksx, rs->yb, rs->yk, rs->ksy, rs->tmp, mean3, std3, stream));
    else if (frames) PROF(e, RPE_PROF_OTHER, stream, rpe_stage_frames_u8(e->dtype, frames, e->x4, e->B, Hs, Ws, e->H, e->W, mean3, std3, stream));
    else PROF(e, RPE_PROF_OTHER, stream, rpe_stage_image_nhwc4(e->dtype, img_nchw, e->x4, e->B, e->H, e->W, stream));
    ConvL& st = e->convs[0];
    TRY(ensure_side(e, (hipStream_t)stream));
    e->sync_next = 0;
    static const bool pool_fuse_ok = getenv("RPE_NO_POOL_FUSE") == nullptr;
    const bool aux_here = e->aux_fwd.w != nullptr;
    e->a1_valid = true;
    if (training && pool_fuse_ok && !((st.Ho | st.Wo) & 1)) {
        TRY(conv_bn(e, st, e->x4, nullptr, 1, stream, false, nullptr, nullptr, true));
        if (aux_here) {
            e->pending_bytes = conv_out_bytes(e, st) * 1.25 + (double)e->B * (st.Ho / 2) * (st.Wo / 2) * (64 + 9);
            PROF(e, RPE_PROF_BN_FWD, stream, rpe_bn_apply_maxpool3x3s2_aux(e->dtype, st.y, st.scale, st.shift, nullptr, e->pool, e->pool_idx, e->B, st.Ho, st.Wo,
                                                                          e->aux_fwd.w, e->aux_fwd.bias, e->aux_fwd.depth_feat, e->aux_fwd.out, e->aux_fwd.ld,
                                                                          e->aux_fwd.raw, e->aux_fwd.idx, stream));
            e->a1_valid = false;
        } else {
        e->pending_bytes = conv_out_bytes(e, st) * 2.25 + (double)e->B * (st.Ho / 2) * (st.Wo / 2) * 64;
        PROF(e, RPE_PROF_BN_FWD, stream, rpe_bn_apply_maxpool3x3s2(e->dtype, st.y, st.scale, st.shift, st.a, e->pool, e->pool_idx, e->B, st.Ho, st.Wo, 64, stream));
        }
    } else {
        TRY(conv_bn(e, st, e->x4, nullptr, 1, stream));
        e->pending_bytes = conv_out_bytes(e, st) * 1.25 + (double)e->B * (st.Ho / 2) * (st.Wo / 2) * 64;
        PROF(e, RPE_PROF_OTHER, stream, rpe_maxpool3x3s2_fwd(e->dtype, st.a, e->pool, e->pool_idx, e->B, st.Ho, st.Wo, 64, stream));
        if (aux_here)
            TRY(rpe_aux_head_fwd(e->dtype, st.a, e->aux_fwd.w, e->aux_fwd.bias, e->aux_fwd.depth_feat, e->aux_fwd.out, e->aux_fwd.ld, e->aux_fwd.raw, e->aux_fwd.idx,
                                 e->B, st.Ho, st.Wo, stream));
    }
    e->aux_fwd.w = nullptr;
    const void* x = e->pool;
    static const bool fwd_overlap = getenv("RPE_NO_FWD_OVERLAP") == nullptr;
    static const bool ds_fuse_ok = getenv("RPE_NO_DS_FUSE") == nullptr;
    const bool fuse_ds = ds_fuse_ok && training;
    for (auto& b : e->blocks) {
        ConvL &c1 = e->convs[b.c1], &c2 = e->convs[b.c2], &c3 = e->convs[b.out];
        const void* idn = x;
        hipEvent_t ds_done = nullptr;
        if (b.cd >= 0 && e->overlap && e->side && fwd_overlap && training) {
            ConvL& cd = e->convs[b.cd];
            hipEvent_t x_ready = sync_event(e);
            ds_done = sync_event(e);
            if (!x_ready || !ds_done) return event_error(e);
            HIPTRY(hipEventRecord(x_ready, (hipStream_t)stream));
            HIPTRY(hipStreamWaitEvent(e->side, x_ready, 0));
            { WalkScope up(e, false); TRY(conv_bn(e, cd, x, nullptr, 0, e->side, true, nullptr, nullptr, fuse_ds)); }
            HIPTRY(hipEventRecord(ds_done, e->side));
            idn = cd.a;
        }
        TRY(conv_bn(e, c1, x, nullptr, 1, stream));
        if (e->basic) {
            static const bool use_mask_b = getenv("RPE_NO_RELU_MASK") == nullptr;
            if (b.cd >= 0 && !ds_done) { ConvL& cd = e->convs[b.cd]; TRY(conv_bn(e, cd, x, nullptr, 0, stream, false, nullptr, nullptr, fuse_ds)); idn = cd.a; }
            if (ds_done) HIPTRY(hipStreamWaitEvent((hipStream_t)stream, ds_done, 0));
            if (b.cd >= 0 && fuse_ds) TRY(conv_bn(e, c2, c1.a, e->convs[b.cd].y, 1, stream, false, use_mask_b ? b.relu_mask : nullptr, &e->convs[b.cd]));
            else TRY(conv_bn(e, c2, c1.a, idn, 1, stream, false, use_mask_b ? b.relu_mask : nullptr));
            x = c2.a;
            continue;
        }
        const bool y3f_fwd = training && b.gram && b.relu_mask;
        const bool fused_gram = y3f_fwd && e->apply_gram && (c2.d.out_c == 64 || c2.d.out_c == 128);
        TRY(conv_bn(e, c2, c1.a, nullptr, 1, stream, false, nullptr, nullptr, false, fused_gram ? b.gram : nullptr));
        if (b.cd >= 0 && !ds_done) { ConvL& cd = e->convs[b.cd]; TRY(conv_bn(e, cd, x, nullptr, 0, stream, false, nullptr, nullptr, fuse_ds)); idn = cd.a; }
        if (ds_done) HIPTRY(hipStreamWaitEvent((hipStream_t)stream, ds_done, 0));
        static const bool use_mask = getenv("RPE_NO_RELU_MASK") == nullptr;
        if (y3f_fwd) {
            const ConvL* cdp = (b.cd >= 0 && fuse_ds) ? &e->convs[b.cd] : nullptr;
            if (!fused_gram) {
                e->pending_flops = 2.0 * (double)c3.rows * c3.d.in_c * c3.d.in_c;
                e->pending_bytes = conv_in_bytes(e, c3);
                PROF(e, RPE_PROF_BN_FWD, stream, rpe_gram(e->dtype, c2.a, c3.rows, c3.d.in_c, b.gram, e->gram_ws, e->gram_ws_bytes, stream));
            }
            e->pending_bytes = 0;
            PROF(e, RPE_PROF_BN_FWD, stream, rpe_bn_stats_from_gram(e->dtype, c3.wf, c3.d.out_c, c3.d.in_c, b.gram, (int)rpe_gram_ones_row(c3.d.in_c), c3.rows,
                                                                    e->params[c3.p_g], e->params[c3.p_b], e->running[2 * c3.bn_i], e->running[2 * c3.bn_i + 1],
                                                                    e->nbt[c3.bn_i], 0.1f, 1e-5f, c3.scale, c3.shift, c3.mean, c3.invstd, stream));
            e->pending_flops = conv_flops(c3);
            e->pending_bytes = conv_in_bytes(e, c3) + conv_out_bytes(e, c3) * (2.0 + (e->y3_keep ? 1.0 : 0.0) + 1.0 / 16);
            PROF(e, RPE_PROF_CONV_FWD, stream, rpe_conv1x1_fwd_bn(&c3.d, e->dtype, c2.a, c3.wf, c3.a, e->y3_keep ? c3.y : nullptr, c3.scale, c3.shift,
                                                                 cdp ? cdp->y : idn, cdp ? cdp->scale : nullptr, cdp ? cdp->shift : nullptr, b.relu_mask, stream));
        } else
        if (b.cd >= 0 && fuse_ds) TRY(conv_bn(e, c3, c2.a, e->convs[b.cd].y, 1, stream, false, use_mask ? b.relu_mask : nullptr, &e->convs[b.cd]));
        else
        TRY(conv_bn(e, c3, c2.a, idn, 1, stream, false, use_mask ? b.relu_mask : nullptr));
        x = c3.a;
    }
    ConvL& last = e->convs[e->blocks.back().out];
    TRY(rpe_avgpool_fwd(e->dtype, last.a, e->pooled, e->B, last.Ho * last.Wo, e->feat, stream));
    const int np = (int)e->pnames.size();
    TRY(rpe_linear_fwd_ws(RPE_F32, e->pooled, e->feat, e->params[np - 2], e->feat, e->params[np - 1], features, (int)ld_features, e->B, e->latent, e->feat, 0,
                          nullptr, 0, e->fc_ws, e->fc_ws ? e->fc_ws_bytes : 0, stream));
    e->fwd_done = training != 0;
    return 0;
}

extern "C" int rpe_resnet50_forward(rpe_resnet50_t* e, const float* img_nchw, float* features, long ld_features, int training, void* stream) {
    return forward_impl(e, img_nchw, nullptr, 0, 0, nullptr, nullptr, features, ld_features, training, stream);
}

extern "C" int rpe_resnet50_forward_u8(rpe_resnet50_t* e, const unsigned char* frames, int Hs, int Ws, const float* mean3_host,
                                       const float* std3_host, float* features, long ld_features, int training, void* stream) {
    if (!frames) return rpe_set_error(RPE_ERR_SHAPE, "resnet50_forward_u8: null frames");
    return forward_impl(e, nullptr, frames, Hs, Ws, mean3_host, std3_host, features, ld_features, training, stream);
}

extern "C" int rpe_resnet50_forward_u8_resized(rpe_resnet50_t* e, const unsigned char* frames, int Hs, int Ws, const rpe_resize_plan* rs,
                                               const float* mean3_host, const float* std3_host, float* features, long ld_features, int training, void* stream) {
    if (!frames || !rs) return rpe_set_error(RPE_ERR_SHAPE, "resnet50_forward_u8_resized: null frames / resize plan");
    return forward_impl(e, nullptr, frames, Hs, Ws, mean3_host, std3_host, features, ld_features, training, stream, rs);
}

extern "C" const void* rpe_resnet50_early_feature(const rpe_resnet50_t* e) { return (e && e->a1_valid) ? e->convs[0].a : nullptr; }
extern "C" void* rpe_resnet50_early_grad(rpe_resnet50_t* e) { return e ? e->early_grad : nullptr; }

static int bn_back(rpe_resnet50* e, ConvL& c, const void* dA, int relu, void* dy, void* dz_out, void* stream) {
    e->pending_bytes = conv_out_bytes(e, c) * ((relu ? 3.0 : 2.0) + 3.0 + (dz_out ? 1.0 : 0.0));
    PROF(e, RPE_PROF_BN_BWD, stream, rpe_bn_backward(e->dtype, dA, relu ? c.a : nullptr, c.y, c.mean, c.invstd, e->params[c.p_g], e->grads[c.p_g], e->grads[c.p_b], dy,
                           dz_out, c.rows, c.d.out_c, e->bwd_part, e->bwd_part_floats, e->c1c2, e->dpart, stream));
    return 0;
}

static int dgrad_fused(rpe_resnet50* e, ConvL& c, const void* dy, void* dz, const void* addend, ConvL* bnl, int mask_mode, void* stream,
                       const unsigned char* relu_mask = nullptr, bool no_y = false, const void* t_a = nullptr, int t_p = 0, float* t_out = nullptr,
                       bool sub_addend = false) {
    rpe_bn_bwd_epilogue ep;
    ep.y = no_y ? nullptr : bnl->y;
    ep.a_mask = mask_mode == 1 ? relu_mask : nullptr;
    ep.a_out = (mask_mode == 1 && !ep.a_mask) ? bnl->a : nullptr;
    ep.mean = bnl->mean; ep.invstd = bnl->invstd;
    ep.scale = mask_mode == 2 ? bnl->scale : nullptr;
    ep.shift = mask_mode == 2 ? bnl->shift : nullptr;
    ep.stats_part = e->stats_part;
    e->pending_flops = conv_flops(c);
    e->pending_bytes = conv_out_bytes(e, c) + conv_in_bytes(e, c) * ((no_y ? 1.0 : 2.0) + (mask_mode == 1 ? (ep.a_mask ? 1.0 / 16 : 1.0) : 0.0) +
                                                                      (addend ? (sub_addend ? 0.25 : 1.0) : 0.0));
    e->fused_tiles = (int)rpe_conv2d_dgrad_stats_tiles(&c.d, e->dtype);
    if (t_out) {
        e->pending_flops += 2.0 * (double)c.rows * c.d.in_c * t_p;
        e->pending_bytes += conv_in_bytes(e, c) * (double)t_p / c.d.in_c;
        PROF(e, RPE_PROF_CONV_DGRAD, stream, rpe_conv1x1_dgrad_bn_t(&c.d, e->dtype, dy, c.wd, dz, addend, &ep, t_a, t_p, t_out, e->main_slab, e->main_slab_bytes, stream));
        return 0;
    }
    if (sub_addend) PROF(e, RPE_PROF_CONV_DGRAD, stream, rpe_conv2d_dgrad_bn_sub(&c.d, e->dtype, dy, c.wd, dz, addend, &ep, stream));
    else PROF(e, RPE_PROF_CONV_DGRAD, stream, rpe_conv2d_dgrad_bn(&c.d, e->dtype, dy, c.wd, dz, addend, &ep, stream));
    return 0;
}

static int bn_from_dz(rpe_resnet50* e, ConvL& c, const void* dz, void* dy, void* stream) {
    e->pending_bytes = conv_out_bytes(e, c) * 3.0;
    PROF(e, RPE_PROF_BN_BWD, stream, rpe_bn_backward_from_dz(e->dtype, dz, c.y, c.mean, c.invstd, e->params[c.p_g], e->stats_part,
                                                              e->fused_tiles, e->grads[c.p_g], e->grads[c.p_b], dy, c.rows,
                                                              c.d.out_c, e->c1c2, e->dpart, stream));
    return 0;
}

static int wgrad_on(rpe_resnet50* e, ConvL& c, const void* x, const void* dy, hipStream_t run) {
    float* dw = e->grads[c.p_w];
    e->pending_flops = conv_flops(c);
    e->pending_bytes = conv_in_bytes(e, c) + conv_out_bytes(e, c);
    if (e->wg_slab) {
        PROF(e, RPE_PROF_CONV_WGRAD, run, rpe_conv2d_wgrad_det(&c.d, e->dtype, x, dy, dw, e->wg_slab, e->wg_slab_bytes, run));
        return 0;
    }
    if (!e->gspan_lo) HIPTRY(hipMemsetAsync(dw, 0, (size_t)e->pnumel[c.p_w] * 4, run));
    PROF(e, RPE_PROF_CONV_WGRAD, run, rpe_conv2d_wgrad(&c.d, e->dtype, x, dy, dw, run));
    return 0;
}

template <typename F> static int to_side(rpe_resnet50* e, void* stream, F work) {
    if (!(e->overlap && e->side)) return work((hipStream_t)stream);
    hipEvent_t ready = sync_event(e);
    if (!ready) return event_error(e);
    HIPTRY(hipEventRecord(ready, (hipStream_t)stream));
    HIPTRY(hipStreamWaitEvent(e->side, ready, 0));
    WalkScope up(e, false);
    return work(e->side);
}
static int wgrad(rpe_resnet50* e, ConvL& c, const void* x, const void* dy, void* stream) {
    ConvL* cp = &c;
    return to_side(e, stream, [e, cp, x, dy](hipStream_t run) { return wgrad_on(e, *cp, x, dy, run); });
}
static int conv1x1_backward_folded(rpe_resnet50* e, ConvL& c, const void* dz, ConvL& behind, void* stream, const Block* y3f = nullptr) {
    const void* x = behind.a;
    if (y3f) {
        e->pending_flops = conv_flops(c);
        e->pending_bytes = conv_in_bytes(e, c) + conv_out_bytes(e, c);
        if (y3f->t_ready) {
        } else
        PROF(e, RPE_PROF_CONV_WGRAD, stream, rpe_conv2d_wgrad_det(&c.d, e->dtype, x, dz, y3f->dzt_a, e->main_slab, e->main_slab_bytes, stream));
        e->pending_bytes = 0;
        PROF(e, RPE_PROF_BN_BWD, stream, rpe_bn_backward_coeffs_t(e->dtype, e->stats_part, e->fused_tiles, c.d.out_c, c.rows, y3f->dzt_a, c.wf, c.d.in_c, c.mean, c.invstd,
                                                                   e->grads[c.p_g], e->grads[c.p_b], c.c1c2, e->dpart, stream));
    } else {
    e->pending_bytes = 0;
    PROF(e, RPE_PROF_BN_BWD, stream, rpe_bn_backward_coeffs(e->stats_part, e->fused_tiles, c.d.out_c, c.rows, e->grads[c.p_g], e->grads[c.p_b], c.c1c2, e->dpart, stream));
    }
    ConvL* cp = &c;
    auto side_part = [e, cp, dz, x, y3f](hipStream_t run) -> int {
    ConvL& c = *cp;
    float* dw = e->grads[c.p_w];
    if (y3f) {
        e->pending_flops = 2.0 * (double)c.d.out_c * c.d.in_c * c.d.in_c;
        e->pending_bytes = 0;
        PROF(e, RPE_PROF_CONV_WGRAD, run, rpe_conv1x1_wgrad_combine(&c.d, y3f->dzt_a, y3f->gram, e->params[c.p_w], e->params[c.p_g], c.invstd, c.mean, c.c1c2, dw, run));
    } else
    if (e->fold_w && e->wfold_scratch && c.d.in_c <= e->fold_w_max) {
        e->pending_flops = conv_flops(c) * (1.0 + (double)c.d.in_c / c.d.out_c);
        e->pending_bytes = conv_out_bytes(e, c) + 3.0 * conv_in_bytes(e, c);
        PROF(e, RPE_PROF_CONV_WGRAD, run, rpe_conv1x1_wgrad_folded(&c.d, e->dtype, dz, x, e->params[c.p_w], e->params[c.p_g], c.invstd, c.mean, c.c1c2, dw,
                                                                  e->wfold_scratch, e->wfold_scratch_bytes, run));
    } else {
    e->pending_bytes = conv_out_bytes(e, c) * 3.0;
    PROF(e, RPE_PROF_BN_BWD, run, rpe_bn_backward_apply_dz(e->dtype, dz, c.y, c.mean, c.invstd, e->params[c.p_g], c.c1c2, c.dy, c.rows, c.d.out_c, run));
    e->pending_flops = conv_flops(c);
    e->pending_bytes = conv_in_bytes(e, c) + conv_out_bytes(e, c);
    if (e->wg_slab) {
        PROF(e, RPE_PROF_CONV_WGRAD, run, rpe_conv2d_wgrad_det(&c.d, e->dtype, x, c.dy, dw, e->wg_slab, e->wg_slab_bytes, run));
    } else {
        if (!e->gspan_lo) HIPTRY(hipMemsetAsync(dw, 0, (size_t)e->pnumel[c.p_w] * 4, run));
        PROF(e, RPE_PROF_CONV_WGRAD, run, rpe_conv2d_wgrad(&c.d, e->dtype, x, c.dy, dw, run));
    }
    }
    return 0;
    };
    TRY(to_side(e, stream, side_part));
    e->pending_bytes = 0;
    PROF(e, RPE_PROF_BN_BWD, stream, rpe_bn_bwd_fold_conv1x1(e->dtype, c.d.out_c, c.d.in_c, fwd_weight(e, c), c.wd, e->params[c.p_g], c.invstd, c.mean, c.c1c2,
                                                              e->w_kcat, e->fold_bias, e->fold_scratch, e->fold_scratch_bytes, stream));
    rpe_bn_bwd_epilogue ep;
    ep.y = behind.y; ep.a_mask = nullptr; ep.a_out = nullptr;
    ep.mean = behind.mean; ep.invstd = behind.invstd; ep.scale = behind.scale; ep.shift = behind.shift;
    ep.stats_part = e->stats_part;
    e->pending_flops = conv_flops(c) * (1.0 + (double)c.d.in_c / c.d.out_c);
    e->pending_bytes = conv_out_bytes(e, c) + conv_in_bytes(e, c) * 3.0;
    e->fused_tiles = (int)rpe_conv2d_dgrad_stats_tiles(&c.d, e->dtype);
    PROF(e, RPE_PROF_CONV_DGRAD, stream, rpe_conv1x1_dgrad_kcat(&c.d, e->dtype, dz, x, e->w_kcat, e->fold_bias, behind.dy, &ep, stream));
    return 0;
}

static int join_side(rpe_resnet50* e, hipStream_t s) {
    if (e->overlap && e->side) {
        hipEvent_t done = sync_event(e);
        if (!done) return event_error(e);
        HIPTRY(hipEventRecord(done, e->side));
// ... 61 lines not shown
            TRY(bn_from_dz(e, c1, c1.dy, c1.dy, stream));
            TRY(wgrad(e, c1, x_in, c1.dy, stream));
            const void* shortcut = gA;
            if (b.cd >= 0) {
                ConvL& cd = e->convs[b.cd];
                shortcut = e->G[0];
                TRY(bn_back(e, cd, gA, 0, cd.dy, nullptr, stream));
                TRY(wgrad(e, cd, x_in, cd.dy, stream));
                e->pending_flops = conv_flops(cd);
                e->pending_bytes = conv_out_bytes(e, cd) + conv_in_bytes(e, cd) * (hook_in ? 2.0 : 1.0);
                PROF(e, RPE_PROF_CONV_DGRAD, stream, rpe_conv2d_dgrad(&cd.d, e->dtype, cd.dy, cd.wd, e->G[0], hook_in, stream));
            }
            static const bool use_mask_b = getenv("RPE_NO_RELU_MASK") == nullptr;
            if (bi > 0) {
                const Block& pb = e->blocks[bi - 1];
                TRY(dgrad_fused(e, c1, c1.dy, gD, shortcut, &e->convs[pb.out], 1, stream, use_mask_b ? pb.relu_mask : nullptr));
            } else {
                e->pending_flops = conv_flops(c1);
                e->pending_bytes = conv_out_bytes(e, c1) + conv_in_bytes(e, c1) * 2.0;
                PROF(e, RPE_PROF_CONV_DGRAD, stream, rpe_conv2d_dgrad(&c1.d, e->dtype, c1.dy, c1.wd, gD, shortcut, stream));
            }
            continue;
        }
        static const bool ds_fold_ok = getenv("RPE_NO_DS_FOLD") == nullptr;
        const bool y3f = b.gram && b.relu_mask && !e->y3_keep;
        if (e->fold && c3.d.in_c <= 256 && e->train_mode) {
            TRY(conv1x1_backward_folded(e, c3, gA, c2, stream, y3f ? &b : nullptr));
        } else {
            if (bi == (int)e->blocks.size() - 1) TRY(bn_back(e, c3, gA, 1, c3.dy, gA, stream));
            else TRY(bn_from_dz(e, c3, gA, c3.dy, stream));
            TRY(wgrad(e, c3, c2.a, c3.dy, stream));
            TRY(dgrad_fused(e, c3, c3.dy, c2.dy, nullptr, &c2, 2, stream));
        }
        TRY(bn_from_dz(e, c2, c2.dy, c2.dy, stream));
        TRY(wgrad(e, c2, c1.a, c2.dy, stream));
        TRY(dgrad_fused(e, c2, c2.dy, c1.dy, nullptr, &c1, 2, stream));
        const bool fold_c1 = e->fold && e->fold1 && e->fold_w && e->wfold_scratch && e->train_mode && c1.d.out_c <= e->fold1_max && (c1.d.out_c % 64) == 0 &&
                             (c1.d.in_c % 64) == 0;
        if (fold_c1) {
            e->pending_bytes = 0;
            PROF(e, RPE_PROF_BN_BWD, stream, rpe_bn_backward_coeffs(e->stats_part, e->fused_tiles, c1.d.out_c, c1.rows, e->grads[c1.p_g], e->grads[c1.p_b], c1.c1c2,
                                                                    e->dpart, stream));
            ConvL* cp = &c1;
            TRY(to_side(e, stream, [e, cp, x_in](hipStream_t run) -> int {
                ConvL& c = *cp;
                e->pending_flops = conv_flops(c) * 2.0;
                e->pending_bytes = 2.0 * conv_out_bytes(e, c) + conv_in_bytes(e, c);
                PROF(e, RPE_PROF_CONV_WGRAD, run, rpe_conv1x1_wgrad_folded_y(&c.d, e->dtype, c.dy, c.y, x_in, e->params[c.p_g], c.invstd, c.mean, c.c1c2, e->grads[c.p_w],
                                                                            e->wfold_scratch, e->wfold_scratch_bytes, run));
                return 0;
            }));
        } else {
            TRY(bn_from_dz(e, c1, c1.dy, c1.dy, stream));
            TRY(wgrad(e, c1, x_in, c1.dy, stream));
        }
        bool t_here = false;
        if (!fold_c1 && bi > 0) {
            const Block& pb = e->blocks[bi - 1];
            const ConvL& p3 = e->convs[pb.c3];
            t_here = pb.gram && pb.relu_mask && !e->y3_keep && e->t_fused && (p3.d.in_c == 64 || p3.d.in_c == 128) && (c1.d.in_c % 128) == 0 && c1.d.kh == 1 &&
                     c1.d.stride == 1;
        }
        const void* shortcut = gA;
        bool sub_addend = false;
        if (b.cd >= 0) {
            ConvL& cd = e->convs[b.cd];
            shortcut = e->G[0];
            const long zero_filled_tiles = 4L * (((long)cd.d.batch * (cd.d.in_h / 2) * (cd.d.in_w / 2) + 127) / 128) * ((cd.d.in_c + 127) / 128);
            sub_addend = zero_filled_tiles >= compact_min_tiles() && !hook_in && !t_here && cd.d.kh == 1 && cd.d.kw == 1 && cd.d.stride == 2 && cd.d.pad == 0 && !(cd.d.in_h & 1) && !(cd.d.in_w & 1) &&
                         c1.d.kh == 1 && c1.d.kw == 1 && c1.d.stride == 1 && c1.d.pad == 0;
            if (ds_fold_ok && e->fold && e->train_mode && e->fold_w && e->wfold_scratch && !hook_in && cd.d.kh == 1 && cd.d.stride == 1 &&
                       cd.d.pad == 0 && cd.d.in_c <= e->fold_w_max && (cd.d.out_c % 128) == 0 && (cd.d.in_c % 64) == 0) {
                e->pending_bytes = conv_out_bytes(e, cd) * 2.0;
                PROF(e, RPE_PROF_BN_BWD, stream, rpe_bn_backward_reduce(e->dtype, gA, nullptr, cd.y, cd.mean, cd.invstd, e->params[cd.p_g], e->grads[cd.p_g],
                                                                        e->grads[cd.p_b], cd.rows, cd.d.out_c, e->bwd_part, e->bwd_part_floats, cd.c1c2, e->dpart, stream));
                {
                    ConvL* cp = &cd;
                    auto side_part = [e, cp, gA, x_in](hipStream_t run) -> int {
                        ConvL& c = *cp;
                        e->pending_flops = conv_flops(c) * (1.0 + (double)c.d.in_c / c.d.out_c);
                        e->pending_bytes = conv_out_bytes(e, c) + 3.0 * conv_in_bytes(e, c);
                        PROF(e, RPE_PROF_CONV_WGRAD, run, rpe_conv1x1_wgrad_folded(&c.d, e->dtype, gA, x_in, e->params[c.p_w], e->params[c.p_g], c.invstd, c.mean, c.c1c2,
                                                                                  e->grads[c.p_w], e->wfold_scratch, e->wfold_scratch_bytes, run));
                        return 0;
                    };
                    TRY(to_side(e, stream, side_part));
                }
                e->pending_bytes = 0;
                PROF(e, RPE_PROF_BN_BWD, stream, rpe_bn_bwd_fold_conv1x1(e->dtype, cd.d.out_c, cd.d.in_c, fwd_weight(e, cd), cd.wd, e->params[cd.p_g], cd.invstd, cd.mean,
                                                                          cd.c1c2, e->w_kcat, e->fold_bias, e->fold_scratch, e->fold_scratch_bytes, stream));
                e->pending_flops = conv_flops(cd) * (1.0 + (double)cd.d.in_c / cd.d.out_c);
                e->pending_bytes = conv_out_bytes(e, cd) + conv_in_bytes(e, cd) * 2.0;
                PROF(e, RPE_PROF_CONV_DGRAD, stream, rpe_conv1x1_dgrad_kcat(&cd.d, e->dtype, gA, x_in, e->w_kcat, e->fold_bias, e->G[0], nullptr, stream));
            } else {
                TRY(bn_back(e, cd, gA, 0, cd.dy, nullptr, stream));
                TRY(wgrad(e, cd, x_in, cd.dy, stream));
                e->pending_flops = conv_flops(cd);
                if (sub_addend) {
                    e->pending_bytes = conv_out_bytes(e, cd) + conv_in_bytes(e, cd) * 0.25;
                    PROF(e, RPE_PROF_CONV_DGRAD, stream, rpe_conv1x1s2_dgrad_compact(&cd.d, e->dtype, cd.dy, cd.wd, e->G[0], stream));
                } else {
                    e->pending_bytes = conv_out_bytes(e, cd) + conv_in_bytes(e, cd) * (hook_in ? 2.0 : 1.0);
                    PROF(e, RPE_PROF_CONV_DGRAD, stream, rpe_conv2d_dgrad(&cd.d, e->dtype, cd.dy, cd.wd, e->G[0], hook_in, stream));
                }
            }
        }
        static const bool use_mask = getenv("RPE_NO_RELU_MASK") == nullptr;
        if (fold_c1) {
            e->pending_bytes = 0;
            PROF(e, RPE_PROF_BN_BWD, stream, rpe_bn_bwd_fold_y_conv1x1(e->dtype, c1.d.out_c, c1.d.in_c, c1.wd, e->params[c1.p_g], c1.invstd, c1.mean, c1.c1c2, e->w_kcat,
                                                                        e->fold_bias, stream));
            rpe_bn_bwd_epilogue ep;
            const rpe_bn_bwd_epilogue* epp = nullptr;
            double extra = 0.0;
            if (bi > 0) {
                ConvL& p3 = e->convs[e->blocks[bi - 1].c3];
                unsigned char* mk = use_mask ? e->blocks[bi - 1].relu_mask : nullptr;
                ep.y = p3.y; ep.a_mask = mk; ep.a_out = mk ? nullptr : p3.a;
                ep.mean = p3.mean; ep.invstd = p3.invstd; ep.scale = nullptr; ep.shift = nullptr;
                ep.stats_part = e->stats_part;
                epp = &ep;
                extra = 1.0 + (mk ? 1.0 / 16 : 1.0);
            }
            e->pending_flops = conv_flops(c1) * 2.0;
            e->pending_bytes = 2.0 * conv_out_bytes(e, c1) + conv_in_bytes(e, c1) * ((sub_addend ? 1.25 : 2.0) + extra);
            e->fused_tiles = (int)rpe_conv2d_dgrad_stats_tiles(&c1.d, e->dtype);
            if (sub_addend) PROF(e, RPE_PROF_CONV_DGRAD, stream, rpe_conv1x1_dgrad_kcat_y_sub(&c1.d, e->dtype, c1.dy, c1.y, e->w_kcat, e->fold_bias, gD, shortcut, epp, stream));
            else PROF(e, RPE_PROF_CONV_DGRAD, stream, rpe_conv1x1_dgrad_kcat_y(&c1.d, e->dtype, c1.dy, c1.y, e->w_kcat, e->fold_bias, gD, shortcut, epp, stream));
        } else
        if (bi > 0) {
            const Block& pb = e->blocks[bi - 1];
            const bool pb_y3f = pb.gram && pb.relu_mask && !e->y3_keep;
            const ConvL& p3 = e->convs[pb.c3];
            e->blocks[bi - 1].t_ready = t_here;
            TRY(dgrad_fused(e, c1, c1.dy, gD, shortcut, &e->convs[pb.c3], 1, stream, use_mask ? pb.relu_mask : nullptr, pb_y3f,
                            t_here ? e->convs[pb.c2].a : nullptr, p3.d.in_c, t_here ? pb.dzt_a : nullptr, sub_addend));
        } else if (sub_addend) {
            PROF(e, RPE_PROF_CONV_DGRAD, stream, rpe_conv2d_dgrad_sub(&c1.d, e->dtype, c1.dy, c1.wd, gD, shortcut, stream));
        } else {
            PROF(e, RPE_PROF_CONV_DGRAD, stream, rpe_conv2d_dgrad(&c1.d, e->dtype, c1.dy, c1.wd, gD, shortcut, stream));
        }
    }
    e->bwd_next = bi;
    if (join) TRY(join_side(e, (hipStream_t)stream));
    return 0;
}

extern "C" int rpe_resnet50_backward_end(rpe_resnet50_t* e, int use_d_early, void* stream) {
    if (!e || !e->bound || e->bwd_next != -1) return rpe_set_error(RPE_ERR_STATE, "resnet50_backward_end: blocks not finished");
    hipStream_t s = (hipStream_t)stream;
    WalkScope walk(e, true);
    void *g0 = e->d_pool, *g1 = e->convs[0].dy;
    ConvL& st = e->convs[0];
    static const bool unfused = getenv("RPE_STEM_UNFUSED") != nullptr;
    if ((use_d_early && !e->aux_dout) || unfused || e->hook_grad[0]) {
        if (use_d_early && e->aux_dout) return rpe_set_error(RPE_ERR_STATE, "resnet50_backward_end: the unfused stem backward (RPE_STEM_UNFUSED, a hook on conv1) needs the dense early gradient");
        PROF(e, RPE_PROF_OTHER, stream, rpe_maxpool3x3s2_bwd(e->dtype, g0, e->pool_idx, use_d_early ? e->early_grad : nullptr, g1, e->B, st.Ho, st.Wo, 64, stream));
        TRY(bn_back(e, st, g1, 1, g1, nullptr, stream));
        if (e->hook_grad[0]) TRY(rpe_tensor_add(e->dtype, g1, e->hook_grad[0], st.rows * 64, stream));
    } else {
        const bool aux = use_d_early != 0;
        e->pending_bytes = conv_out_bytes(e, st) * 3.0 + 2.0 * (double)e->B * (st.Ho / 2) * (st.Wo / 2) * 64 * (e->esz + 1);
        PROF(e, RPE_PROF_BN_BWD, stream, rpe_stem_bwd(e->dtype, g0, e->pool_idx, st.y, st.scale, st.shift, st.mean, st.invstd, e->params[st.p_g],
                                                      aux ? e->aux_dout : nullptr, e->aux_ld, aux ? e->aux_df : nullptr, aux ? e->aux_idx : nullptr,
                                                      aux ? e->aux_w : nullptr, e->grads[st.p_g], e->grads[st.p_b], g1, e->B, st.Ho, st.Wo,
                                                      e->bwd_part, e->bwd_part_floats, e->c1c2, e->dpart, stream));
    }
    e->aux_dout = nullptr;
    for (int i = 0; i < 4; ++i) e->hook_grad[i] = nullptr;
    if (hipError_t he = hipMemsetAsync(e->stem_dw, 0, 64 * 256 * 4, s)) return rpe_set_error_hip(he, __FILE__, __LINE__);
    if (e->main_slab) PROF(e, RPE_PROF_CONV_WGRAD, stream, rpe_stem_conv_wgrad_det(e->dtype, e->x4, g1, e->stem_dw, e->B, e->H, e->W, e->main_slab, e->main_slab_bytes, stream));
    else PROF(e, RPE_PROF_CONV_WGRAD, stream, rpe_stem_conv_wgrad(e->dtype, e->x4, g1, e->stem_dw, e->B, e->H, e->W, stream));
    TRY(rpe_unpack_stem_grad(e->stem_dw, e->grads[st.p_w], stream));
    TRY(join_side(e, s));
    e->bwd_next = -2;
    return 0;
}

extern "C" int rpe_resnet50_set_aux_head(rpe_resnet50_t* e, const float* w, const float* bias, const float* depth_feat, float* out, long ld_out, float* raw,
                                         unsigned char* idx) {
    if (!e) return rpe_set_error(RPE_ERR_STATE, "resnet50_set_aux_head: null engine");
    if (w && (!bias || !out || !raw || !idx || ld_out < (long)(e->convs[0].Ho / 2) * (e->convs[0].Wo / 2)))
        return rpe_set_error(RPE_ERR_SHAPE, "resnet50_set_aux_head: bias, the output columns (row pitch >= (H/4)(W/4)), raw and idx are required");
    e->aux_fwd.w = w; e->aux_fwd.bias = bias; e->aux_fwd.depth_feat = depth_feat; e->aux_fwd.out = out; e->aux_fwd.ld = ld_out; e->aux_fwd.raw = raw; e->aux_fwd.idx = idx;
    return 0;
}

extern "C" int rpe_resnet50_aux_head_bwd(rpe_resnet50_t* e, const float* dout, long ld_dout, const float* w, const float* depth_feat, const float* raw,
                                         const unsigned char* idx, float* dw, float* dbias, float* d_depth_feat, float* workspace, long workspace_floats,
                                         void* stream) {
    if (!e || !e->bound || !e->fwd_done) return rpe_set_error(RPE_ERR_STATE, "resnet50_aux_head_bwd: no training-mode forward to differentiate");
    const ConvL& st = e->convs[0];
    return rpe_aux_head_bwd_det_y(e->dtype, dout, ld_dout, st.y, st.scale, st.shift, w, depth_feat, raw, idx, dw, dbias, d_depth_feat, e->B, st.Ho, st.Wo, workspace,
                                  workspace_floats, stream);
}

extern "C" int rpe_resnet50_side_stream_info(const rpe_resnet50_t* e, int* candidates, int* concurrent) {
    if (!e || !candidates || !concurrent) return rpe_set_error(RPE_ERR_SHAPE, "resnet50_side_stream_info: null argument");
    *candidates = e->side_tries; *concurrent = e->side_concurrent;
    return 0;
}

extern "C" int rpe_resnet50_set_aux_grad(rpe_resnet50_t* e, const float* aux_dout, long aux_ld, const float* aux_depth_feat,
                                         const unsigned char* aux_idx, const float* aux_w) {
    if (!e) return rpe_set_error(RPE_ERR_STATE, "resnet50_set_aux_grad: null engine");
    if (aux_dout && (!aux_idx || !aux_w || aux_ld <= 0)) return rpe_set_error(RPE_ERR_SHAPE, "resnet50_set_aux_grad: winner indices, weight and row pitch are required");
    e->aux_dout = aux_dout; e->aux_ld = aux_ld; e->aux_df = aux_depth_feat; e->aux_idx = aux_idx; e->aux_w = aux_w;
    return 0;
}

extern "C" int rpe_resnet50_set_hook_grad(rpe_resnet50_t* e, int layer, const void* dense_grad) {
    if (!e || layer < 0 || layer > 3) return rpe_set_error(RPE_ERR_SHAPE, "resnet50_set_hook_grad: layer 0 (conv1's raw output) or 1..3 (layer outputs)");
    e->hook_grad[layer] = dense_grad;
    return 0;
}

extern "C" int rpe_resnet50_set_stem_raw(rpe_resnet50_t* e, int on) {
    if (!e) return rpe_set_error(RPE_ERR_STATE, "resnet50_set_stem_raw: null engine");
    if (e->stem_raw != (on != 0)) { e->stem_raw = on != 0; if (e->pack_state == 2) e->pack_state = 0; }
    return 0;
}

extern "C" int rpe_resnet50_backward_frozen(rpe_resnet50_t* e, const float* d_features, long ld_d_features, void* stream) {
    if (!e || !e->bound) return rpe_set_error(RPE_ERR_STATE, "resnet50_backward_frozen: engine not bound");
    if (!e->fwd_done) return rpe_set_error(RPE_ERR_STATE, "resnet50_backward_frozen: no training-mode forward to differentiate");
    const int np = (int)e->pnames.size();
    if (!d_features || !e->grads[np - 2] || !e->grads[np - 1]) return rpe_set_error(RPE_ERR_STATE, "resnet50_backward_frozen: fc gradient tensors were not bound");
    hipStream_t s = (hipStream_t)stream;
    float* dWfc = e->grads[np - 2];
    if (e->main_slab) {
        TRY(rpe_linear_wgrad_det(RPE_F32, d_features, (int)ld_d_features, e->pooled, e->feat, dWfc, e->feat, e->B, e->latent, e->feat, 0, e->main_slab, e->main_slab_bytes, stream));
    } else {
        HIPTRY(hipMemsetAsync(dWfc, 0, (size_t)e->latent * e->feat * 4, s));
        TRY(rpe_linear_wgrad(RPE_F32, d_features, (int)ld_d_features, e->pooled, e->feat, dWfc, e->feat, e->B, e->latent, e->feat, stream));
    }
    TRY(rpe_colsum(d_features, e->B, e->latent, (int)ld_d_features, e->grads[np - 1], 0, stream));
    e->aux_dout = nullptr;
    for (int i = 0; i < 4; ++i) e->hook_grad[i] = nullptr;
    e->bwd_next = -2;
    return 0;
}

extern "C" int rpe_resnet50_backward(rpe_resnet50_t* e, const float* d_features, long ld_d_features, int use_d_early, void* stream) {
    TRY(rpe_resnet50_backward_begin(e, d_features, ld_d_features, stream));
    TRY(rpe_resnet50_backward_blocks(e, 1 << 20, 0, stream));
    return rpe_resnet50_backward_end(e, use_d_early, stream);
}

extern "C" int rpe_resnet50_tensor(const rpe_resnet50_t* e, const char* name, const void** ptr, long* rows, int* channels) {
    if (!e || !e->bound || !name) return rpe_set_error(RPE_ERR_STATE, "resnet50_tensor: engine not bound");
    for (auto& n : e->named)
        if (n.name == name) { *ptr = n.ptr; *rows = n.rows; *channels = n.ch; return 0; }
    return rpe_set_error(RPE_ERR_SHAPE, "resnet50_tensor: unknown tensor name");
}
```

### rgb-proprioceptive-pose-estimator_amd/csrc/norm.hip

```cpp
#include "common.h"
#include <cstdlib>

namespace rpe {

struct BnFwdFin {
    double count;
    const float *gamma, *beta;
    float *running_mean, *running_var;
    long long* num_batches;
    float momentum, eps;
    float *scale, *shift, *save_mean, *save_invstd;
    __device__ void operator()(int c, double s, double q) const {
        const float g = gamma[c], bt = beta[c];
        const float* rmp = running_mean ? running_mean : gamma;
        const float* rvp = running_var ? running_var : gamma;
        const float rm = rmp[c], rv = rvp[c];
        const double mean = s / count;
        double var = q / count - mean * mean;
        if (var < 0.0) var = 0.0;
        const float invstd = (float)(1.0 / sqrt(var + (double)eps));
        const float sc = g * invstd;
        scale[c] = sc;
        shift[c] = bt - (float)mean * sc;
        save_mean[c] = (float)mean;
        save_invstd[c] = invstd;
        if (running_mean) {
            const double unb = count > 1.0 ? var * count / (count - 1.0) : var;
            running_mean[c] = (1.f - momentum) * rm + momentum * (float)mean;
            running_var[c] = (1.f - momentum) * rv + momentum * (float)unb;
        }
        if (num_batches && c == 0) *num_batches += 1;
    }
};
struct BnBwdFin {
    double count;
    float *dgamma, *dbeta, *c1, *c2;
    __device__ void operator()(int c, double s, double q) const {
        if (dbeta) dbeta[c] = (float)s;
        if (dgamma) dgamma[c] = (float)q;
        c1[c] = (float)(s / count);
        c2[c] = (float)(q / count);
    }
};

template <typename T> struct BnBwdFinT {
    static constexpr bool kDot = true;
    double count;
    float *dgamma, *dbeta, *c1, *c2;
    const float* Tm;
    const T* w;
    int Ci;
    const float *mean, *invstd;
    __device__ double dot(int c, int part, int nparts) const {
        double r = 0.0;
        for (int k0 = part; k0 < Ci; k0 += 16 * nparts) {
            float tv[16], wv[16];
#pragma unroll
            for (int u = 0; u < 16; ++u) {
                const int k = k0 + u * nparts;
                tv[u] = k < Ci ? Tm[(long)c * Ci + k] : 0.f;
                wv[u] = k < Ci ? Elem<T>::to_f(w[(long)c * Ci + k]) : 0.f;
            }
#pragma unroll
            for (int u = 0; u < 16; ++u) r += (double)tv[u] * (double)wv[u];
        }
        return r;
    }
    __device__ void operator()(int c, double s, double d) const {
        const float is_ = invstd[c], mu_ = mean[c];
        const double q = (double)is_ * (d - (double)mu_ * s);
        if (dbeta) dbeta[c] = (float)s;
        if (dgamma) dgamma[c] = (float)q;
        c1[c] = (float)(s / count);
        c2[c] = (float)(q / count);
    }
};
template <typename Fin, typename = void> struct FinHasDot { static constexpr bool value = false; };
template <typename Fin> struct FinHasDot<Fin, decltype((void)Fin::kDot)> { static constexpr bool value = true; };

template <typename Fin>
__global__ __launch_bounds__(256) void reduce_finalize_kernel(const float* __restrict__ part, int tiles, int C, int NS, double* dpart,
                                                             unsigned* counters, const Fin fin) {
    __shared__ double sh[2][8][32];
    __shared__ int last;
    const int cl = threadIdx.x & 31, rl = threadIdx.x >> 5;
    const int c = blockIdx.x * 32 + cl;
    double s = 0.0, q = 0.0;
    if (c < C) {
        const int st = 8 * NS;
        int t = blockIdx.y + rl * NS;
        constexpr bool NOQ = FinHasDot<Fin>::value;
        for (; t + 3 * st < tiles; t += 4 * st) {
            const float a0 = part[((long)t * 2 + 0) * C + c], b0 = NOQ ? 0.f : part[((long)t * 2 + 1) * C + c];
            const float a1 = part[((long)(t + st) * 2 + 0) * C + c], b1 = NOQ ? 0.f : part[((long)(t + st) * 2 + 1) * C + c];
            const float a2 = part[((long)(t + 2 * st) * 2 + 0) * C + c], b2 = NOQ ? 0.f : part[((long)(t + 2 * st) * 2 + 1) * C + c];
            const float a3 = part[((long)(t + 3 * st) * 2 + 0) * C + c], b3 = NOQ ? 0.f : part[((long)(t + 3 * st) * 2 + 1) * C + c];
            s += ((double)a0 + (double)a1) + ((double)a2 + (double)a3);
            q += ((double)b0 + (double)b1) + ((double)b2 + (double)b3);
        }
        for (; t < tiles; t += st) {
            s += (double)part[((long)t * 2 + 0) * C + c];
            if (!NOQ) q += (double)part[((long)t * 2 + 1) * C + c];
        }
    }
    sh[0][rl][cl] = s;
    sh[1][rl][cl] = q;
    __syncthreads();
    if (rl == 0) {
        for (int i = 1; i < 8; ++i) { s += sh[0][i][cl]; q += sh[1][i][cl]; }
    }
    if (NS > 1) {
        if (rl == 0 && c < C) {
            __hip_atomic_store(&dpart[((long)blockIdx.y * 2 + 0) * C + c], s, __ATOMIC_RELAXED, __HIP_MEMORY_SCOPE_AGENT);
            __hip_atomic_store(&dpart[((long)blockIdx.y * 2 + 1) * C + c], q, __ATOMIC_RELAXED, __HIP_MEMORY_SCOPE_AGENT);
        }
        asm volatile("s_waitcnt vmcnt(0)" ::: "memory");
        __syncthreads();
        if (threadIdx.x == 0) {
            const unsigned prev = __hip_atomic_fetch_add(&counters[blockIdx.x], 1u, __ATOMIC_RELAXED, __HIP_MEMORY_SCOPE_AGENT);
            last = prev == (unsigned)NS - 1;
            if (last) __hip_atomic_store(&counters[blockIdx.x], 0u, __ATOMIC_RELAXED, __HIP_MEMORY_SCOPE_AGENT);
        }
        __syncthreads();
        if (!last) return;
        s = 0.0; q = 0.0;
        if (c < C) {
            double vs[8], vq[8];
#pragma unroll
            for (int u = 0; u < 8; ++u) {
                const int i = rl + 8 * u, ic = i < NS ? i : 0;
                vs[u] = __hip_atomic_load(&dpart[((long)ic * 2 + 0) * C + c], __ATOMIC_RELAXED, __HIP_MEMORY_SCOPE_AGENT);
                vq[u] = __hip_atomic_load(&dpart[((long)ic * 2 + 1) * C + c], __ATOMIC_RELAXED, __HIP_MEMORY_SCOPE_AGENT);
            }
#pragma unroll
            for (int u = 0; u < 8; ++u)
                if (rl + 8 * u >= NS) { vs[u] = 0.0; vq[u] = 0.0; }
#pragma unroll
            for (int u = 0; u < 8; ++u) { s += vs[u]; q += vq[u]; }
        }
        sh[0][rl][cl] = s;
        sh[1][rl][cl] = q;
        __syncthreads();
        if (rl == 0) {
            for (int i = 1; i < 8; ++i) { s += sh[0][i][cl]; q += sh[1][i][cl]; }
        }
    }
    if constexpr (FinHasDot<Fin>::value) {
        const int dc = blockIdx.x * 32 + (threadIdx.x >> 3), part = threadIdx.x & 7;
        double d = dc < C ? fin.dot(dc, part, 8) : 0.0;
        d += __shfl_xor(d, 1); d += __shfl_xor(d, 2); d += __shfl_xor(d, 4);
        __syncthreads();
        if (part == 0) sh[0][0][threadIdx.x >> 3] = d;
        __syncthreads();
// ... 279 lines not shown
        float best[CE];
        unsigned char bi[CE];
        const unsigned char first = (unsigned char)((oh == 0 ? 3 : 0) + (ow == 0 ? 1 : 0));
#pragma unroll
        for (int e = 0; e < CE; ++e) { best[e] = -INFINITY; bi[e] = first; }
        for (int kh = 0; kh < 3; ++kh) {
            const int ih = oh * 2 - 1 + kh;
            if (ih < 0 || ih >= H) continue;
            for (int kw = 0; kw < 3; ++kw) {
                const int iw = ow * 2 - 1 + kw;
                if (iw < 0 || iw >= W) continue;
                float v[CE];
                chunk_to_f<T>(*(const u32x4*)(x + (((long)b * H + ih) * W + iw) * C + cc * CE), v);
#pragma unroll
                for (int e = 0; e < CE; ++e)
                    if (v[e] > best[e] || v[e] != v[e]) { best[e] = v[e]; bi[e] = (unsigned char)(kh * 3 + kw); }
            }
        }
        *(u32x4*)(out + i * CE) = f_to_chunk<T>(best);
        store_winners<CE>(idx + i * CE, bi);
    }
}

template <int CE>
__device__ __forceinline__ float stem_aux_dot(const float* v, const float* w) {
#pragma clang fp contract(off)
    float d = 0.f;
#pragma unroll
    for (int e = 0; e < CE; ++e) d += v[e] * w[e];
    return d;
}
struct StemAuxFwd {
    const float *w, *bias, *depth_feat;
    float* out; long ld_out;
    float* raw; unsigned char* idx;
};
template <typename T, bool AUX>
__global__ __launch_bounds__(256) void bn_apply_maxpool_kernel(const T* __restrict__ y, const float* __restrict__ scale, const float* __restrict__ shift,
                                                              T* __restrict__ a, T* __restrict__ out, unsigned char* __restrict__ idx,
                                                              int B, int H, int W, int C, int Ho, int Wo, const StemAuxFwd aux, int rev) {
    constexpr int CE = Elem<T>::kChunk;
    const int cpr = C / CE;
    const long total = (long)B * Ho * Wo * cpr;
    const long span = (long)gridDim.x * blockDim.x;
    const int bx = xcd_remap_dir(blockIdx.x, gridDim.x, rev);
    for (long i = (long)bx * blockDim.x + threadIdx.x; i < total; i += span) {
        const int cc = (int)(i % cpr);
        long pix = i / cpr;
        const int ow = (int)(pix % Wo); pix /= Wo;
        const int oh = (int)(pix % Ho);
        const int b = (int)(pix / Ho);
        float sc[CE], sh[CE], aw[CE], ad[4] = {0.f, 0.f, 0.f, 0.f};
#pragma unroll
        for (int e = 0; e < CE; ++e) { sc[e] = scale[cc * CE + e]; sh[e] = shift[cc * CE + e]; aw[e] = AUX ? aux.w[cc * CE + e] : 0.f; }
        u32x4 raw[9];
        bool ok[9];
#pragma unroll
        for (int k = 0; k < 9; ++k) {
            const int ih = oh * 2 - 1 + k / 3, iw = ow * 2 - 1 + k % 3;
            ok[k] = ih >= 0 && ih < H && iw >= 0 && iw < W;
            const int ihc = ih < 0 ? 0 : (ih >= H ? H - 1 : ih), iwc = iw < 0 ? 0 : (iw >= W ? W - 1 : iw);
            raw[k] = *(const u32x4*)(y + (((long)b * H + ihc) * W + iwc) * C + cc * CE);
        }
        float best[CE];
        unsigned char bi[CE];
#pragma unroll
        for (int e = 0; e < CE; ++e) { best[e] = -INFINITY; bi[e] = 0; }
#pragma unroll
        for (int k = 0; k < 9; ++k) {
            if (!ok[k]) continue;
            float v[CE];
            chunk_to_f<T>(raw[k], v);
#pragma unroll
            for (int e = 0; e < CE; ++e) v[e] = fmaxf(fmaf(v[e], sc[e], sh[e]), 0.f);
            const u32x4 packed = f_to_chunk<T>(v);
            if (k / 3 >= 1 && k % 3 >= 1 && a) {
                const int ih = oh * 2 - 1 + k / 3, iw = ow * 2 - 1 + k % 3;
                *(u32x4*)(a + (((long)b * H + ih) * W + iw) * C + cc * CE) = packed;
            }
            chunk_to_f<T>(packed, v);
            if (AUX && k / 3 >= 1 && k % 3 >= 1) {
                ad[(k / 3 - 1) * 2 + (k % 3 - 1)] = stem_aux_dot<CE>(v, aw);
            }
#pragma unroll
            for (int e = 0; e < CE; ++e)
                if (v[e] > best[e] || v[e] != v[e]) { best[e] = v[e]; bi[e] = (unsigned char)k; }
        }
        *(u32x4*)(out + i * CE) = f_to_chunk<T>(best);
        store_winners<CE>(idx + i * CE, bi);
        if (AUX) {
            const float bv = aux.bias[0];
            float bestd = -INFINITY;
            int bk = 0;
#pragma unroll
            for (int k = 0; k < 4; ++k) {
                float d = ad[k];
                for (int o = 1; o < cpr; o <<= 1) d += __shfl_xor(d, o);
                d += bv;
                if (d > bestd || d != d) { bestd = d; bk = k; }
            }
            if (cc == 0) {
                const long pos = (long)oh * Wo + ow, flat = (long)b * Ho * Wo + pos;
                const float df = aux.depth_feat ? aux.depth_feat[flat] : 1.f;
                aux.out[(long)b * aux.ld_out + pos] = bestd * df;
                aux.raw[flat] = bestd;
                aux.idx[flat] = (unsigned char)bk;
            }
        }
    }
}

template <typename T>
__global__ __launch_bounds__(256) void maxpool_bwd_kernel(const T* __restrict__ dout, const unsigned char* __restrict__ idx,
                                                         const T* __restrict__ addend, T* __restrict__ dx,
                                                         int B, int H, int W, int C, int Ho, int Wo) {
    constexpr int CE = Elem<T>::kChunk;
    const int cpr = C / CE;
    const long total = (long)B * H * W * cpr;
    for (long i = (long)blockIdx.x * blockDim.x + threadIdx.x; i < total; i += (long)gridDim.x * blockDim.x) {
        const int cc = (int)(i % cpr);
        long pix = i / cpr;
        const int w = (int)(pix % W); pix /= W;
        const int h = (int)(pix % H);
        const int b = (int)(pix / H);
        float acc[CE];
        if (addend) chunk_to_f<T>(*(const u32x4*)(addend + i * CE), acc);
        else {
#pragma unroll
            for (int e = 0; e < CE; ++e) acc[e] = 0.f;
        }
        for (int kh = 0; kh < 3; ++kh) {
            const int t = h + 1 - kh;
            if (t < 0 || (t & 1)) continue;
            const int oh = t >> 1;
            if (oh >= Ho) continue;
            for (int kw = 0; kw < 3; ++kw) {
                const int u = w + 1 - kw;
                if (u < 0 || (u & 1)) continue;
                const int ow = u >> 1;
                if (ow >= Wo) continue;
                const long o = (((long)b * Ho + oh) * Wo + ow) * C + cc * CE;
                float d[CE];
                chunk_to_f<T>(*(const u32x4*)(dout + o), d);
                const unsigned char* ip = idx + o;
#pragma unroll
                for (int e = 0; e < CE; ++e)
                    if (ip[e] == (unsigned char)(kh * 3 + kw)) acc[e] += d[e];
            }
        }
        *(u32x4*)(dx + i * CE) = f_to_chunk<T>(acc);
    }
}

struct StemAux {
    const float* dout;
    long ld;
    const float* depth_feat;
    const unsigned char* idx;
    const float* w;
};

template <typename T>
__device__ __forceinline__ void stem_dz_block(const T* __restrict__ dpool, const unsigned char* __restrict__ pidx, const StemAux& ax, const float* axw,
                                              const float* sc, const float* sh, const float (*yy)[Elem<T>::kChunk], int b, int oh, int ow, int c0,
                                              int Ho, int Wo, float (*dz)[Elem<T>::kChunk]) {
    constexpr int CE = Elem<T>::kChunk;
    const long o00 = (((long)b * Ho + oh) * Wo + ow) * 64 + c0;
    const bool right = ow + 1 < Wo, below = oh + 1 < Ho;
    float d[4][CE];
    unsigned long long taps[4];
    const long wo[4] = {o00, right ? o00 + 64 : o00, below ? o00 + (long)Wo * 64 : o00, (right && below) ? o00 + (long)Wo * 64 + 64 : o00};
    const bool wok[4] = {true, right, below, right && below};
    u32x4 wraw[4];
#pragma unroll
    for (int k = 0; k < 4; ++k) {
        wraw[k] = *(const u32x4*)(dpool + wo[k]);
        taps[k] = CE == 8 ? *(const unsigned long long*)(pidx + wo[k]) : (unsigned long long)*(const unsigned*)(pidx + wo[k]);
    }
    const long apos = (long)oh * Wo + ow, aflat = (long)b * Ho * Wo + apos;
    const unsigned char* awp = ax.dout ? ax.idx + aflat : pidx;
    const float* agp = ax.dout ? ax.dout + (long)b * ax.ld + apos : (const float*)dpool;
    const float* adp = (ax.dout && ax.depth_feat) ? ax.depth_feat + aflat : (const float*)dpool;
    const int awin = (int)*awp;
    const float ag = *agp, adf = *adp;
#pragma unroll
    for (int k = 0; k < 4; ++k) {
        chunk_to_f<T>(wraw[k], d[k]);
        if (!wok[k]) {
#pragma unroll
            for (int e = 0; e < CE; ++e) d[k][e] = 0.f;
            taps[k] = ~0ull;
        }
    }
#pragma unroll
    for (int e = 0; e < CE; ++e) {
        const unsigned t0 = (unsigned)(taps[0] >> (8 * e)) & 0xffu, t1 = (unsigned)(taps[1] >> (8 * e)) & 0xffu;
        const unsigned t2 = (unsigned)(taps[2] >> (8 * e)) & 0xffu, t3 = (unsigned)(taps[3] >> (8 * e)) & 0xffu;
        dz[0][e] = t0 == 4u ? d[0][e] : 0.f;
        dz[1][e] = (t0 == 5u ? d[0][e] : 0.f) + (t1 == 3u ? d[1][e] : 0.f);
        dz[2][e] = (t0 == 7u ? d[0][e] : 0.f) + (t2 == 1u ? d[2][e] : 0.f);
        dz[3][e] = (t0 == 8u ? d[0][e] : 0.f) + (t1 == 6u ? d[1][e] : 0.f) + (t2 == 2u ? d[2][e] : 0.f) + (t3 == 0u ? d[3][e] : 0.f);
    }
    if (ax.dout) {
        const int win = awin;
        float g = ag;
        if (ax.depth_feat) g *= adf;
#pragma unroll
        for (int k = 0; k < 4; ++k)
#pragma unroll
            for (int e = 0; e < CE; ++e) dz[k][e] += win == k ? g * axw[e] : 0.f;
    }
#pragma unroll
    for (int k = 0; k < 4; ++k)
#pragma unroll
        for (int e = 0; e < CE; ++e)
            if (!(fmaf(yy[k][e], sc[e], sh[e]) > 0.f)) dz[k][e] = 0.f;
}

template <typename T>
__global__ __launch_bounds__(256) void stem_bwd_reduce_kernel(const T* __restrict__ dpool, const unsigned char* __restrict__ pidx, const StemAux ax,
                                                             const T* __restrict__ y, const float* __restrict__ scale, const float* __restrict__ shift,
                                                             const float* __restrict__ mean, const float* __restrict__ invstd, int B, int H, int W,
                                                             int Ho, int Wo, int rows_per_block, float* __restrict__ part) {
    constexpr int CE = Elem<T>::kChunk, CPR = 64 / CE, PPB = 256 / CPR;
    __shared__ float sh[PPB][64][2];
    const int cc = threadIdx.x % CPR, pl = threadIdx.x / CPR, c0 = cc * CE;
    float sc[CE], sf[CE], mu[CE], is[CE], s1[CE], s2[CE];
#pragma unroll
    for (int e = 0; e < CE; ++e) { sc[e] = scale[c0 + e]; sf[e] = shift[c0 + e]; mu[e] = mean[c0 + e]; is[e] = invstd[c0 + e]; s1[e] = 0.f; s2[e] = 0.f; }
    float axw[CE];
#pragma unroll
    for (int e = 0; e < CE; ++e) axw[e] = ax.dout ? ax.w[c0 + e] : 0.f;
    const int row_end = min(B * Ho, ((int)blockIdx.x + 1) * rows_per_block);
    for (int row = blockIdx.x * rows_per_block; row < row_end; ++row) {
        const int b = row / Ho, oh = row - b * Ho;
        for (int ow = pl; ow < Wo; ow += PPB) {
            const long p00 = (((long)b * H + 2 * oh) * W + 2 * ow) * 64 + c0;
            float yy[4][CE], dz[4][CE];
            chunk_to_f<T>(*(const u32x4*)(y + p00), yy[0]);
            chunk_to_f<T>(*(const u32x4*)(y + p00 + 64), yy[1]);
            chunk_to_f<T>(*(const u32x4*)(y + p00 + (long)W * 64), yy[2]);
            chunk_to_f<T>(*(const u32x4*)(y + p00 + (long)W * 64 + 64), yy[3]);
            stem_dz_block<T>(dpool, pidx, ax, axw, sc, sf, yy, b, oh, ow, c0, Ho, Wo, dz);
#pragma unroll
            for (int k = 0; k < 4; ++k)
#pragma unroll
                for (int e = 0; e < CE; ++e) { s1[e] += dz[k][e]; s2[e] += dz[k][e] * (yy[k][e] - mu[e]) * is[e]; }
        }
    }
#pragma unroll
    for (int e = 0; e < CE; ++e) { sh[pl][c0 + e][0] = s1[e]; sh[pl][c0 + e][1] = s2[e]; }
    __syncthreads();
    if (threadIdx.x < 128) {
        const int c = threadIdx.x >> 1, which = threadIdx.x & 1;
        float t = 0.f;
        for (int k = 0; k < PPB; ++k) t += sh[k][c][which];
        part[((long)blockIdx.x * 2 + which) * 64 + c] = t;
    }
}

template <typename T>
__global__ __launch_bounds__(256) void stem_bwd_apply_kernel(const T* __restrict__ dpool, const unsigned char* __restrict__ pidx, const StemAux ax,
                                                            const T* __restrict__ y, const float* __restrict__ scale, const float* __restrict__ shift,
                                                            const float* __restrict__ mean, const float* __restrict__ invstd,
                                                            const float* __restrict__ gamma, const float* __restrict__ c1, const float* __restrict__ c2,
                                                            T* __restrict__ dy, int B, int H, int W, int Ho, int Wo, int rows_per_block) {
    constexpr int CE = Elem<T>::kChunk, CPR = 64 / CE, PPB = 256 / CPR;
    const int cc = threadIdx.x % CPR, pl = threadIdx.x / CPR, c0 = cc * CE;
    float sc[CE], sf[CE], k0[CE], k1[CE], k2[CE];
#pragma unroll
    for (int e = 0; e < CE; ++e) {
        sc[e] = scale[c0 + e]; sf[e] = shift[c0 + e];
        const float gi = gamma[c0 + e] * invstd[c0 + e];
        k0[e] = gi;
        k2[e] = -gi * invstd[c0 + e] * c2[c0 + e];
        k1[e] = -gi * c1[c0 + e] - k2[e] * mean[c0 + e];
    }
    float axw[CE];
#pragma unroll
    for (int e = 0; e < CE; ++e) axw[e] = ax.dout ? ax.w[c0 + e] : 0.f;
    const int row_end = min(B * Ho, ((int)blockIdx.x + 1) * rows_per_block);
    for (int row = blockIdx.x * rows_per_block; row < row_end; ++row) {
        const int b = row / Ho, oh = row - b * Ho;
        for (int ow = pl; ow < Wo; ow += PPB) {
            const long p00 = (((long)b * H + 2 * oh) * W + 2 * ow) * 64 + c0;
            const long off[4] = {p00, p00 + 64, p00 + (long)W * 64, p00 + (long)W * 64 + 64};
            float yy[4][CE], dz[4][CE];
#pragma unroll
            for (int k = 0; k < 4; ++k) chunk_to_f<T>(*(const u32x4*)(y + off[k]), yy[k]);
            stem_dz_block<T>(dpool, pidx, ax, axw, sc, sf, yy, b, oh, ow, c0, Ho, Wo, dz);
#pragma unroll
            for (int k = 0; k < 4; ++k) {
#pragma unroll
                for (int e = 0; e < CE; ++e) dz[k][e] = fmaf(k0[e], dz[k][e], fmaf(k2[e], yy[k][e], k1[e]));
                *(u32x4*)(dy + off[k]) = f_to_chunk<T>(dz[k]);
            }
        }
    }
}

template <typename T>
__global__ __launch_bounds__(256) void avgpool_fwd_kernel(const T* __restrict__ x, float* __restrict__ out, int B, int HW, int C) {
    constexpr int CE = Elem<T>::kChunk;
    const int cpr = C / CE;
    const long i = (long)blockIdx.x * blockDim.x + threadIdx.x;
    if (i >= (long)B * cpr) return;
    const int cc = (int)(i % cpr), b = (int)(i / cpr);
    float acc[CE];
#pragma unroll
    for (int e = 0; e < CE; ++e) acc[e] = 0.f;
    for (int p = 0; p < HW; ++p) {
        float v[CE];
        chunk_to_f<T>(*(const u32x4*)(x + ((long)b * HW + p) * C + cc * CE), v);
#pragma unroll
        for (int e = 0; e < CE; ++e) acc[e] += v[e];
    }
    const float inv = 1.f / (float)HW;
#pragma unroll
    for (int e = 0; e < CE; ++e) out[(long)b * C + cc * CE + e] = acc[e] * inv;
}

template <typename T>
__global__ __launch_bounds__(256) void avgpool_fwd_few_kernel(const T* __restrict__ x, float* __restrict__ out, int B, int HW, int C) {
    constexpr int CE = Elem<T>::kChunk;
    const int cpr = C / CE;
    const long i = ((long)blockIdx.x * blockDim.x + threadIdx.x) >> 3;
    const int sub = threadIdx.x & 7;
    const bool ok = i < (long)B * cpr;
    const int cc = ok ? (int)(i % cpr) : 0, b = ok ? (int)(i / cpr) : 0;
    float acc[CE];
#pragma unroll
    for (int e = 0; e < CE; ++e) acc[e] = 0.f;
    for (int p = sub; p < HW; p += 8) {
        float v[CE];
        chunk_to_f<T>(*(const u32x4*)(x + ((long)b * HW + p) * C + cc * CE), v);
#pragma unroll
        for (int e = 0; e < CE; ++e) acc[e] += v[e];
    }
#pragma unroll
    for (int e = 0; e < CE; ++e) {
        acc[e] += __shfl_xor(acc[e], 1, 64);
        acc[e] += __shfl_xor(acc[e], 2, 64);
        acc[e] += __shfl_xor(acc[e], 4, 64);
    }
    if (ok && sub == 0) {
        const float inv = 1.f / (float)HW;
#pragma unroll
        for (int e = 0; e < CE; ++e) out[(long)b * C + cc * CE + e] = acc[e] * inv;
    }
}

template <typename T>
__global__ __launch_bounds__(256) void avgpool_bwd_kernel(const float* __restrict__ dout, T* __restrict__ dx, int B, int HW, int C) {
    constexpr int CE = Elem<T>::kChunk;
    const int cpr = C / CE;
    const long total = (long)B * HW * cpr;
    const float inv = 1.f / (float)HW;
    for (long i = (long)blockIdx.x * blockDim.x + threadIdx.x; i < total; i += (long)gridDim.x * blockDim.x) {
        const int cc = (int)(i % cpr);
        const int b = (int)(i / ((long)cpr * HW));
        float v[CE];
#pragma unroll
        for (int e = 0; e < CE; ++e) v[e] = dout[(long)b * C + cc * CE + e] * inv;
        *(u32x4*)(dx + i * CE) = f_to_chunk<T>(v);
    }
}

__device__ __forceinline__ long x4_index(long b, int h, int w, int H, int W) {
    return ((b * (H + 2 * RPE_STEM_PAD) + h + RPE_STEM_PAD) * (long)(W + 2 * RPE_STEM_PAD) + w + RPE_STEM_PAD) * 4;
}
template <typename T>
// ... 553 lines not shown
```

Before: 14740 images/s.

## Fold stem BN backward into conv1 weight gradient via forward-side precomputed terms

Adds a folded stem backward path that computes the conv1 weight gradient directly from the BN-backward dz terms. During the forward pass it precomputes y-weighted im2col sums (s2) and im2col column sums, overlapped on a side stream. In backward, one kernel produces dz-weighted im2col partials and the dz statistics, and a combine kernel applies the BN backward algebra to yield dw, dgamma and dbeta. This avoids materialising the full stem dy tensor and running a separate wgrad over it, at the cost of extra forward-side work, new workspace, and only supporting 16-bit dtypes and large inputs.

```diff
diff --git a/include/rpe_hip.h b/include/rpe_hip.h
--- a/include/rpe_hip.h
+++ b/include/rpe_hip.h
@@ -233,6 +233,16 @@
                  const float* invstd, const float* gamma, const float* aux_dout, long aux_ld, const float* aux_depth_feat,
                  const unsigned char* aux_idx, const float* aux_w, float* dgamma, float* dbeta, void* dy, int B, int H, int W, float* part,
                  long part_floats, float* c1c2, double* dpart, void* stream);
+long rpe_stem_wgrad_dz_workspace_bytes(int dtype, int B, int H, int W);
+int rpe_stem_wgrad_dz_geometry(int dtype, int B, int H, int W, int* workgroups, int* tiles, int* tile_rows, int* tiles_per_workgroup);
+int rpe_stem_wgrad_dz(int dtype, const void* dpool, const unsigned char* pool_idx, const void* y, const float* scale, const float* shift, const float* mean,
+                      const float* invstd, const float* aux_dout, long aux_ld, const float* aux_depth_feat, const unsigned char* aux_idx,
+                      const float* aux_w, const void* x4, int B, int H, int W, void* workspace, long workspace_bytes, void* stream);
+long rpe_stem_im2col_colsum_workspace_bytes(int B, int H, int W);
+int rpe_stem_im2col_colsum(int dtype, const void* x4, float* colsum, int B, int H, int W, void* workspace, long workspace_bytes, void* stream);
+int rpe_stem_wgrad_combine(int dtype, void* workspace, long workspace_bytes, const float* s2_packed, const float* colsum, const float* mean,
+                           const float* invstd, const float* gamma, float* dgamma, float* dbeta, float* c1c2, float* dw_oihw, int B, int H, int W,
+                           void* stream);
 int rpe_avgpool_fwd(int dtype, const void* x, float* out, int B, int HW, int C, void* stream);
 int rpe_avgpool_bwd(int dtype, const float* dout, void* dx, int B, int HW, int C, void* stream);
 
diff --git a/rgb-proprioceptive-pose-estimator_amd/_lib.py b/rgb-proprioceptive-pose-estimator_amd/_lib.py
--- a/rgb-proprioceptive-pose-estimator_amd/_lib.py
+++ b/rgb-proprioceptive-pose-estimator_amd/_lib.py
@@ -154,6 +154,12 @@
     "rpe_bn_apply_maxpool3x3s2": (I, [I, P, P, P, P, P, P, I, I, I, I, P]),
     "rpe_maxpool3x3s2_bwd": (I, [I, P, P, P, P, I, I, I, I, P]),
     "rpe_stem_bwd": (I, [I, P, P, P, P, P, P, P, P, P, L, P, P, P, P, P, P, I, I, I, P, L, P, P, P]),
+    "rpe_stem_wgrad_dz_workspace_bytes": (L, [I, I, I, I]),
+    "rpe_stem_wgrad_dz_geometry": (I, [I, I, I, I, POINTER(c_int), POINTER(c_int), POINTER(c_int), POINTER(c_int)]),
+    "rpe_stem_wgrad_dz": (I, [I, P, P, P, P, P, P, P, P, L, P, P, P, P, I, I, I, P, L, P]),
+    "rpe_stem_im2col_colsum_workspace_bytes": (L, [I, I, I]),
+    "rpe_stem_im2col_colsum": (I, [I, P, P, I, I, I, P, L, P]),
+    "rpe_stem_wgrad_combine": (I, [I, P, L, P, P, P, P, P, P, P, P, P, I, I, I, P]),
     "rpe_avgpool_fwd": (I, [I, P, P, I, I, I, P]),
     "rpe_avgpool_bwd": (I, [I, P, P, I, I, I, P]),
     "rpe_aux_head_fwd": (I, [I, P, P, P, P, P, L, P, P, I, I, I, P]),
diff --git a/rgb-proprioceptive-pose-estimator_amd/csrc/engine.hip b/rgb-proprioceptive-pose-estimator_amd/csrc/engine.hip
--- a/rgb-proprioceptive-pose-estimator_amd/csrc/engine.hip
+++ b/rgb-proprioceptive-pose-estimator_amd/csrc/engine.hip
@@ -85,6 +85,9 @@
     struct { const float *w = nullptr, *bias = nullptr, *depth_feat = nullptr; float* out = nullptr; long ld = 0; float* raw = nullptr; unsigned char* idx = nullptr; } aux_fwd;
     bool a1_valid = false;
     float* stem_dw = nullptr;
+    bool stem_fold = false, stem_fold_ready = false;
+    float* stem_s2 = nullptr;
+    float* stem_colsum = nullptr;
     bool fold = true;
     void* w_kcat = nullptr;
     float* fold_bias = nullptr;
@@ -215,6 +218,12 @@
     return (int)e->convs.size() - 1;
 }
 
+static long stem_fold_min_rows() { return 1L << 19; }
+static bool stem_unfused() {
+    static const bool unfused = getenv("RPE_STEM_UNFUSED") != nullptr;
+    return unfused;
+}
+
 static void want(rpe_resnet50* e, void** dst, long bytes) {
     bytes = (bytes + 255) / 256 * 256;
     e->slots.push_back({dst, bytes});
@@ -396,6 +405,15 @@
         const long fcb = rpe_linear_wgrad_workspace_bytes(RPE_F32, batch, latent_dim, e->feat);
         if (fcb > e->main_slab_bytes) e->main_slab_bytes = fcb;
         if (y3_slab > e->main_slab_bytes) e->main_slab_bytes = y3_slab;
+        const long sfb = dtype != RPE_F32 ? rpe_stem_wgrad_dz_workspace_bytes(dtype, batch, st.Ho, st.Wo) : -1;
+        const long scb = rpe_stem_im2col_colsum_workspace_bytes(batch, st.Ho, st.Wo);
+        e->stem_fold = sfb > 0 && scb > 0 && st.rows >= stem_fold_min_rows() && e->main_slab_bytes > 0;
+        if (e->stem_fold) {
+            if (sfb > e->main_slab_bytes) e->main_slab_bytes = sfb;
+            if (scb > e->main_slab_bytes) e->main_slab_bytes = scb;
+            want(e, (void**)&e->stem_s2, 64L * 256 * 4);
+            want(e, (void**)&e->stem_colsum, 256L * 4);
+        }
         if (e->main_slab_bytes > 0) want(e, &e->main_slab, e->main_slab_bytes);
     }
     {
@@ -744,8 +762,39 @@
     static const bool pool_fuse_ok = getenv("RPE_NO_POOL_FUSE") == nullptr;
     const bool aux_here = e->aux_fwd.w != nullptr;
     e->a1_valid = true;
+    static const bool fwd_overlap = getenv("RPE_NO_FWD_OVERLAP") == nullptr;
+    hipEvent_t fold_done = nullptr;
+    e->stem_fold_ready = false;
+    auto stem_fold_fwd = [&]() -> int {
+        if (!(training && e->stem_fold && e->main_slab && !stem_unfused() && e->grads[st.p_w])) return 0;
+        hipStream_t run = (hipStream_t)stream;
+        const bool side = e->overlap && e->side && fwd_overlap;
+        if (side) {
+            hipEvent_t y_ready = sync_event(e);
+            fold_done = sync_event(e);
+            if (!y_ready || !fold_done) return event_error(e);
+            HIPTRY(hipEventRecord(y_ready, (hipStream_t)stream));
+            HIPTRY(hipStreamWaitEvent(e->side, y_ready, 0));
+            run = e->side;
+        }
+        auto work = [&]() -> int {
+            const double x4_bytes = (double)e->B * (e->H + 2 * RPE_STEM_PAD) * (e->W + 2 * RPE_STEM_PAD) * 4 * e->esz;
+            e->pending_flops = 2.0 * (double)st.rows * 64 * 256;
+            e->pending_bytes = conv_out_bytes(e, st) + x4_bytes;
+            PROF(e, RPE_PROF_CONV_WGRAD, run, rpe_stem_conv_wgrad_det(e->dtype, e->x4, st.y, e->stem_s2, e->B, e->H, e->W, e->main_slab, e->main_slab_bytes, run));
+            e->pending_bytes = x4_bytes;
+            PROF(e, RPE_PROF_CONV_WGRAD, run, rpe_stem_im2col_colsum(e->dtype, e->x4, e->stem_colsum, e->B, st.Ho, st.Wo, e->main_slab, e->main_slab_bytes, run));
+            return 0;
+        };
+        if (side) { WalkScope up(e, false); TRY(work()); }
+        else TRY(work());
+        if (side) HIPTRY(hipEventRecord(fold_done, e->side));
+        e->stem_fold_ready = true;
+        return 0;
+    };
     if (training && pool_fuse_ok && !((st.Ho | st.Wo) & 1)) {
         TRY(conv_bn(e, st, e->x4, nullptr, 1, stream, false, nullptr, nullptr, true));
+        TRY(stem_fold_fwd());
         if (aux_here) {
             e->pending_bytes = conv_out_bytes(e, st) * 1.25 + (double)e->B * (st.Ho / 2) * (st.Wo / 2) * (64 + 9);
             PROF(e, RPE_PROF_BN_FWD, stream, rpe_bn_apply_maxpool3x3s2_aux(e->dtype, st.y, st.scale, st.shift, nullptr, e->pool, e->pool_idx, e->B, st.Ho, st.Wo,
@@ -758,6 +807,7 @@
         }
     } else {
         TRY(conv_bn(e, st, e->x4, nullptr, 1, stream));
+        TRY(stem_fold_fwd());
         e->pending_bytes = conv_out_bytes(e, st) * 1.25 + (double)e->B * (st.Ho / 2) * (st.Wo / 2) * 64;
         PROF(e, RPE_PROF_OTHER, stream, rpe_maxpool3x3s2_fwd(e->dtype, st.a, e->pool, e->pool_idx, e->B, st.Ho, st.Wo, 64, stream));
         if (aux_here)
@@ -766,7 +816,6 @@
     }
     e->aux_fwd.w = nullptr;
     const void* x = e->pool;
-    static const bool fwd_overlap = getenv("RPE_NO_FWD_OVERLAP") == nullptr;
     static const bool ds_fuse_ok = getenv("RPE_NO_DS_FUSE") == nullptr;
     const bool fuse_ds = ds_fuse_ok && training;
     for (auto& b : e->blocks) {
@@ -826,6 +875,7 @@
     const int np = (int)e->pnames.size();
     TRY(rpe_linear_fwd_ws(RPE_F32, e->pooled, e->feat, e->params[np - 2], e->feat, e->params[np - 1], features, (int)ld_features, e->B, e->latent, e->feat, 0,
                           nullptr, 0, e->fc_ws, e->fc_ws ? e->fc_ws_bytes : 0, stream));
+    if (fold_done) HIPTRY(hipStreamWaitEvent((hipStream_t)stream, fold_done, 0));
     e->fwd_done = training != 0;
     return 0;
 }
@@ -1193,7 +1243,25 @@
     WalkScope walk(e, true);
     void *g0 = e->d_pool, *g1 = e->convs[0].dy;
     ConvL& st = e->convs[0];
-    static const bool unfused = getenv("RPE_STEM_UNFUSED") != nullptr;
+    const bool unfused = stem_unfused();
+    const bool folded = e->stem_fold && e->stem_fold_ready && e->main_slab && !(use_d_early && !e->aux_dout) && !unfused && !e->hook_grad[0];
+    e->stem_fold_ready = false;
+    if (folded) {
+        const bool aux = use_d_early != 0;
+        const double pool_px = (double)e->B * (st.Ho / 2) * (st.Wo / 2) * 64;
+        e->pending_flops = 2.0 * (double)st.rows * 64 * 256;
+        e->pending_bytes = conv_out_bytes(e, st) + pool_px * (e->esz + 1) + (double)e->B * (e->H + 2 * RPE_STEM_PAD) * (e->W + 2 * RPE_STEM_PAD) * 4 * e->esz;
+        PROF(e, RPE_PROF_CONV_WGRAD, stream, rpe_stem_wgrad_dz(e->dtype, g0, e->pool_idx, st.y, st.scale, st.shift, st.mean, st.invstd, aux ? e->aux_dout : nullptr, e->aux_ld,
+                                                               aux ? e->aux_df : nullptr, aux ? e->aux_idx : nullptr, aux ? e->aux_w : nullptr, e->x4, e->B, st.Ho, st.Wo,
+                                                               e->main_slab, e->main_slab_bytes, stream));
+        PROF(e, RPE_PROF_BN_BWD, stream, rpe_stem_wgrad_combine(e->dtype, e->main_slab, e->main_slab_bytes, e->stem_s2, e->stem_colsum, st.mean, st.invstd, e->params[st.p_g],
+                                                                e->grads[st.p_g], e->grads[st.p_b], e->c1c2, e->grads[st.p_w], e->B, st.Ho, st.Wo, stream));
+        e->aux_dout = nullptr;
+        for (int i = 0; i < 4; ++i) e->hook_grad[i] = nullptr;
+        TRY(join_side(e, s));
+        e->bwd_next = -2;
+        return 0;
+    }
     if ((use_d_early && !e->aux_dout) || unfused || e->hook_grad[0]) {
         if (use_d_early && e->aux_dout) return rpe_set_error(RPE_ERR_STATE, "resnet50_backward_end: the unfused stem backward (RPE_STEM_UNFUSED, a hook on conv1) needs the dense early gradient");
         PROF(e, RPE_PROF_OTHER, stream, rpe_maxpool3x3s2_bwd(e->dtype, g0, e->pool_idx, use_d_early ? e->early_grad : nullptr, g1, e->B, st.Ho, st.Wo, 64, stream));
diff --git a/rgb-proprioceptive-pose-estimator_amd/csrc/norm.hip b/rgb-proprioceptive-pose-estimator_amd/csrc/norm.hip
--- a/rgb-proprioceptive-pose-estimator_amd/csrc/norm.hip
+++ b/rgb-proprioceptive-pose-estimator_amd/csrc/norm.hip
@@ -1,4 +1,5 @@
 #include "common.h"
+#include "stem_dz.h"
 #include <cstdlib>
 
 namespace rpe {
@@ -584,71 +585,6 @@
     }
 }
 
-struct StemAux {
-    const float* dout;
-    long ld;
-    const float* depth_feat;
-    const unsigned char* idx;
-    const float* w;
-};
-
-template <typename T>
-__device__ __forceinline__ void stem_dz_block(const T* __restrict__ dpool, const unsigned char* __restrict__ pidx, const StemAux& ax, const float* axw,
-                                              const float* sc, const float* sh, const float (*yy)[Elem<T>::kChunk], int b, int oh, int ow, int c0,
-                                              int Ho, int Wo, float (*dz)[Elem<T>::kChunk]) {
-    constexpr int CE = Elem<T>::kChunk;
-    const long o00 = (((long)b * Ho + oh) * Wo + ow) * 64 + c0;
-    const bool right = ow + 1 < Wo, below = oh + 1 < Ho;
-    float d[4][CE];
-    unsigned long long taps[4];
-    const long wo[4] = {o00, right ? o00 + 64 : o00, below ? o00 + (long)Wo * 64 : o00, (right && below) ? o00 + (long)Wo * 64 + 64 : o00};
-    const bool wok[4] = {true, right, below, right && below};
-    u32x4 wraw[4];
-#pragma unroll
-    for (int k = 0; k < 4; ++k) {
-        wraw[k] = *(const u32x4*)(dpool + wo[k]);
-        taps[k] = CE == 8 ? *(const unsigned long long*)(pidx + wo[k]) : (unsigned long long)*(const unsigned*)(pidx + wo[k]);
-    }
-    const long apos = (long)oh * Wo + ow, aflat = (long)b * Ho * Wo + apos;
-    const unsigned char* awp = ax.dout ? ax.idx + aflat : pidx;
-    const float* agp = ax.dout ? ax.dout + (long)b * ax.ld + apos : (const float*)dpool;
-    const float* adp = (ax.dout && ax.depth_feat) ? ax.depth_feat + aflat : (const float*)dpool;
-    const int awin = (int)*awp;
-    const float ag = *agp, adf = *adp;
-#pragma unroll
-    for (int k = 0; k < 4; ++k) {
-        chunk_to_f<T>(wraw[k], d[k]);
-        if (!wok[k]) {
-#pragma unroll
-            for (int e = 0; e < CE; ++e) d[k][e] = 0.f;
-            taps[k] = ~0ull;
-        }
-    }
-#pragma unroll
-    for (int e = 0; e < CE; ++e) {
-        const unsigned t0 = (unsigned)(taps[0] >> (8 * e)) & 0xffu, t1 = (unsigned)(taps[1] >> (8 * e)) & 0xffu;
-        const unsigned t2 = (unsigned)(taps[2] >> (8 * e)) & 0xffu, t3 = (unsigned)(taps[3] >> (8 * e)) & 0xffu;
-        dz[0][e] = t0 == 4u ? d[0][e] : 0.f;
-        dz[1][e] = (t0 == 5u ? d[0][e] : 0.f) + (t1 == 3u ? d[1][e] : 0.f);
-        dz[2][e] = (t0 == 7u ? d[0][e] : 0.f) + (t2 == 1u ? d[2][e] : 0.f);
-        dz[3][e] = (t0 == 8u ? d[0][e] : 0.f) + (t1 == 6u ? d[1][e] : 0.f) + (t2 == 2u ? d[2][e] : 0.f) + (t3 == 0u ? d[3][e] : 0.f);
-    }
-    if (ax.dout) {
-        const int win = awin;
-        float g = ag;
-        if (ax.depth_feat) g *= adf;
-#pragma unroll
-        for (int k = 0; k < 4; ++k)
-#pragma unroll
-            for (int e = 0; e < CE; ++e) dz[k][e] += win == k ? g * axw[e] : 0.f;
-    }
-#pragma unroll
-    for (int k = 0; k < 4; ++k)
-#pragma unroll
-        for (int e = 0; e < CE; ++e)
-            if (!(fmaf(yy[k][e], sc[e], sh[e]) > 0.f)) dz[k][e] = 0.f;
-}
-
 template <typename T>
 __global__ __launch_bounds__(256) void stem_bwd_reduce_kernel(const T* __restrict__ dpool, const unsigned char* __restrict__ pidx, const StemAux ax,
                                                              const T* __restrict__ y, const float* __restrict__ scale, const float* __restrict__ shift,
diff --git a/rgb-proprioceptive-pose-estimator_amd/csrc/stem_dz.h b/rgb-proprioceptive-pose-estimator_amd/csrc/stem_dz.h
--- /dev/null
+++ b/rgb-proprioceptive-pose-estimator_amd/csrc/stem_dz.h
@@ -0,0 +1,71 @@
+#pragma once
+#include "common.h"
+
+namespace rpe {
+
+struct StemAux {
+    const float* dout;
+    long ld;
+    const float* depth_feat;
+    const unsigned char* idx;
+    const float* w;
+};
+
+template <typename T>
+__device__ __forceinline__ void stem_dz_block(const T* __restrict__ dpool, const unsigned char* __restrict__ pidx, const StemAux& ax, const float* axw,
+                                              const float* sc, const float* sh, const float (*yy)[Elem<T>::kChunk], int b, int oh, int ow, int c0,
+                                              int Ho, int Wo, float (*dz)[Elem<T>::kChunk]) {
+    constexpr int CE = Elem<T>::kChunk;
+    const long o00 = (((long)b * Ho + oh) * Wo + ow) * 64 + c0;
+    const bool right = ow + 1 < Wo, below = oh + 1 < Ho;
+    float d[4][CE];
+    unsigned long long taps[4];
+    const long wo[4] = {o00, right ? o00 + 64 : o00, below ? o00 + (long)Wo * 64 : o00, (right && below) ? o00 + (long)Wo * 64 + 64 : o00};
+    const bool wok[4] = {true, right, below, right && below};
+    u32x4 wraw[4];
+#pragma unroll
+    for (int k = 0; k < 4; ++k) {
+        wraw[k] = *(const u32x4*)(dpool + wo[k]);
+        taps[k] = CE == 8 ? *(const unsigned long long*)(pidx + wo[k]) : (unsigned long long)*(const unsigned*)(pidx + wo[k]);
+    }
+    const long apos = (long)oh * Wo + ow, aflat = (long)b * Ho * Wo + apos;
+    const unsigned char* awp = ax.dout ? ax.idx + aflat : pidx;
+    const float* agp = ax.dout ? ax.dout + (long)b * ax.ld + apos : (const float*)dpool;
+    const float* adp = (ax.dout && ax.depth_feat) ? ax.depth_feat + aflat : (const float*)dpool;
+    const int awin = (int)*awp;
+    const float ag = *agp, adf = *adp;
+#pragma unroll
+    for (int k = 0; k < 4; ++k) {
+        chunk_to_f<T>(wraw[k], d[k]);
+        if (!wok[k]) {
+#pragma unroll
+            for (int e = 0; e < CE; ++e) d[k][e] = 0.f;
+            taps[k] = ~0ull;
+        }
+    }
+#pragma unroll
+    for (int e = 0; e < CE; ++e) {
+        const unsigned t0 = (unsigned)(taps[0] >> (8 * e)) & 0xffu, t1 = (unsigned)(taps[1] >> (8 * e)) & 0xffu;
+        const unsigned t2 = (unsigned)(taps[2] >> (8 * e)) & 0xffu, t3 = (unsigned)(taps[3] >> (8 * e)) & 0xffu;
+        dz[0][e] = t0 == 4u ? d[0][e] : 0.f;
+        dz[1][e] = (t0 == 5u ? d[0][e] : 0.f) + (t1 == 3u ? d[1][e] : 0.f);
+        dz[2][e] = (t0 == 7u ? d[0][e] : 0.f) + (t2 == 1u ? d[2][e] : 0.f);
+        dz[3][e] = (t0 == 8u ? d[0][e] : 0.f) + (t1 == 6u ? d[1][e] : 0.f) + (t2 == 2u ? d[2][e] : 0.f) + (t3 == 0u ? d[3][e] : 0.f);
+    }
+    if (ax.dout) {
+        const int win = awin;
+        float g = ag;
+        if (ax.depth_feat) g *= adf;
+#pragma unroll
+        for (int k = 0; k < 4; ++k)
+#pragma unroll
+            for (int e = 0; e < CE; ++e) dz[k][e] += win == k ? g * axw[e] : 0.f;
+    }
+#pragma unroll
+    for (int k = 0; k < 4; ++k)
+#pragma unroll
+        for (int e = 0; e < CE; ++e)
+            if (!(fmaf(yy[k][e], sc[e], sh[e]) > 0.f)) dz[k][e] = 0.f;
+}
+
+}
diff --git a/rgb-proprioceptive-pose-estimator_amd/csrc/stem_fold.hip b/rgb-proprioceptive-pose-estimator_amd/csrc/stem_fold.hip
--- /dev/null
+++ b/rgb-proprioceptive-pose-estimator_amd/csrc/stem_fold.hip
@@ -0,0 +1,403 @@
+#include "igemm_impl.h"
+#include "stem_dz.h"
+#include <cstring>
+
+namespace rpe {
+
+constexpr int kSfTilePx = 16;
+constexpr int kSfTileRows = 4 * kSfTilePx;
+constexpr int kSfTargetWgs = 512;
+
+template <typename T> struct StemFoldArgs {
+    const T* dpool;
+    const unsigned char* pidx;
+    StemAux ax;
+    const T* y;
+    const T* x4;
+    const float *scale, *shift, *mean, *invstd;
+    float* slab;
+    float* part;
+    int B, H, W, Ho, Wo;
+    int XW;
+    unsigned img_stride;
+    long x4_elems;
+    FastDiv div_wo, div_ho;
+    int np;
+    int tiles, tiles_per_wg, nwg, rev;
+};
+
+__device__ __forceinline__ unsigned sf_div(unsigned n, const FastDiv& f) {
+    const unsigned q = __umulhi(n, f.mul) >> f.shr;
+    return f.d <= 1 ? n : q;
+}
+
+template <typename T>
+__global__ __launch_bounds__(256, 2) void stem_wgrad_dz_kernel(const StemFoldArgs<T> p) {
+    static_assert(sizeof(T) == 2, "16-bit element types only");
+    constexpr int CE = 8, ES = 2;
+    constexpr int BI = 64, BJ = 256, BMK = kSfTileRows, KSUB = BMK / 32;
+    constexpr int CPI = BI / CE, CPJ = BJ / CE;
+    constexpr int PT = BMK * CPI, QT = BMK * CPJ, STAGE = PT + QT;
+    constexpr int NPJ = QT / 256;
+    constexpr int WI = BI / 2, WJ = BJ / 2, FI = WI / 16, FJ = WJ / 16;
+    __shared__ u32x4 lds[2 * STAGE];
+
+    const int tid = threadIdx.x, lane = tid & 63, wave = tid >> 6;
+    const int wave_i = wave >> 1, wave_j = wave & 1;
+    const int wave_u = __builtin_amdgcn_readfirstlane(wave);
+    const int half = wave_u >> 1;
+    const int lb = xcd_remap_dir(blockIdx.x, p.nwg, p.rev);
+    const int t_begin = min(p.tiles, lb * p.tiles_per_wg), t_end = min(p.tiles, t_begin + p.tiles_per_wg);
+    const int nsteps = t_end - t_begin;
+
+    typedef __attribute__((address_space(3))) char lds_char;
+    constexpr unsigned OOB = 0x80000000u;
+    auto clamp31 = [](long bytes) -> int { return (int)(bytes < 0 ? 0 : (bytes > 0x7fffffffL ? 0x7fffffffL : bytes)); };
+    const int pp_first = t_begin < p.tiles ? t_begin * kSfTilePx : 0;
+    const unsigned b0 = (unsigned)__builtin_amdgcn_readfirstlane((int)sf_div(sf_div((unsigned)pp_first, p.div_wo), p.div_ho));
+    const long q_base = (long)b0 * p.img_stride;
+    const __amdgpu_buffer_rsrc_t rs_q = __builtin_amdgcn_make_buffer_rsrc((void*)(p.x4 + q_base), 0, clamp31((p.x4_elems - q_base) * (long)ES), 0x00020000);
+    const int q_slot = tid % CPJ, q_r = tid / CPJ, q_q = q_r & 3, q_k0 = q_r >> 2;
+    unsigned q_tap[2];
+#pragma unroll
+    for (int u = 0; u < 2; ++u) {
+        const int row = q_r + 8 * u, cc = q_slot ^ tn_swz<T, CPJ>(row);
+        q_tap[u] = (unsigned)((2 * (q_q >> 1) + (cc >> 2)) * p.XW + 2 * (q_q & 1) + 2 * (cc & 3));
+    }
+    auto dma_q = [&](int tile, int st) {
+        const unsigned lds_u = (unsigned)__builtin_amdgcn_readfirstlane((int)(unsigned)(uintptr_t)((lds_char*)lds + st * (STAGE * 16) + PT * 16));
+#pragma unroll
+        for (int i = 0; i < NPJ; ++i) {
+            const unsigned pp = (unsigned)(tile * kSfTilePx + q_k0 + 2 * i);
+            const unsigned prow = sf_div(pp, p.div_wo), ow = pp - prow * (unsigned)p.Wo;
+            const unsigned b = sf_div(prow, p.div_ho), oh = prow - b * (unsigned)p.Ho;
+            const unsigned pix = __umul24(4u * oh, (unsigned)p.XW) + 4u * ow + q_tap[i & 1];
+            const unsigned vo = pp < (unsigned)p.np ? (__umul24(b - b0, p.img_stride) + 4u * pix) * ES : OOB;
+            dma16_asm(rs_q, lds_u + (unsigned)((i * 4 + wave_u) * 1024), vo);
+        }
+    };
+
+    const int pt = tid & 127, p_k = pt >> 3, p_cc = pt & 7, c0 = p_cc * CE;
+    float s1[CE], s2[CE];
+#pragma unroll
+    for (int e = 0; e < CE; ++e) { s1[e] = 0.f; s2[e] = 0.f; }
+    auto produce = [&](int tile, int st) {
+        float sc[CE], sf[CE], mu[CE], is[CE], axw[CE];
+#pragma unroll
+        for (int e = 0; e < CE; ++e) { sc[e] = p.scale[c0 + e]; sf[e] = p.shift[c0 + e]; mu[e] = p.mean[c0 + e]; is[e] = p.invstd[c0 + e]; }
+        const float* axp = p.ax.dout ? p.ax.w : p.scale;
+#pragma unroll
+        for (int e = 0; e < CE; ++e) axw[e] = axp[c0 + e];
+        if (!p.ax.dout) {
+#pragma unroll
+            for (int e = 0; e < CE; ++e) axw[e] = 0.f;
+        }
+        const int pp_raw = tile * kSfTilePx + p_k;
+        const bool live = pp_raw < p.np;
+        const unsigned pp = (unsigned)(live ? pp_raw : p.np - 1);
+        const unsigned prow = sf_div(pp, p.div_wo), ow = pp - prow * (unsigned)p.Wo;
+        const unsigned b = sf_div(prow, p.div_ho), oh = prow - b * (unsigned)p.Ho;
+        const long p00 = (((long)b * p.H + 2 * oh) * p.W + 2 * ow) * 64 + c0;
+        float yy[4][CE], dz[4][CE];
+        chunk_to_f<T>(*(const u32x4*)(p.y + p00), yy[0]);
+        chunk_to_f<T>(*(const u32x4*)(p.y + p00 + 64), yy[1]);
+        chunk_to_f<T>(*(const u32x4*)(p.y + p00 + (long)p.W * 64), yy[2]);
+        chunk_to_f<T>(*(const u32x4*)(p.y + p00 + (long)p.W * 64 + 64), yy[3]);
+        stem_dz_block<T>(p.dpool, p.pidx, p.ax, axw, sc, sf, yy, (int)b, (int)oh, (int)ow, c0, p.Ho, p.Wo, dz);
+        u32x4* pbase = lds + st * STAGE;
+#pragma unroll
+        for (int k = 0; k < 4; ++k) {
+#pragma unroll
+            for (int e = 0; e < CE; ++e) {
+                if (!live) dz[k][e] = 0.f;
+                s1[e] += dz[k][e];
+                s2[e] += dz[k][e] * (yy[k][e] - mu[e]) * is[e];
+            }
+            const int row = 4 * p_k + k;
+            pbase[row * CPI + (p_cc ^ tn_swz<T, CPI>(row))] = f_to_chunk<T>(dz[k]);
+        }
+    };
+
+    f32x4 acc[FI][FJ];
+#pragma unroll
+    for (int a = 0; a < FI; ++a)
+#pragma unroll
+        for (int b = 0; b < FJ; ++b) acc[a][b] = f32x4{0.f, 0.f, 0.f, 0.f};
+
+    const int fg = lane >> 4, fl = lane & 15;
+    auto compute = [&](int cur) {
+        const char* pb = (const char*)(lds + cur * STAGE);
+        const char* qb = (const char*)(lds + cur * STAGE + PT);
+#pragma unroll
+        for (int ks = 0; ks < KSUB; ++ks) {
+            const int rb = ks * 32;
+            const int q = fl >> 2, pp = fl & 3;
+            u32x4 pf[FI], qf[FJ];
+#pragma unroll
+            for (int a = 0; a < FI; ++a) {
+                const int col = wave_i * WI + a * 16 + 4 * pp;
+                unsigned w[4];
+#pragma unroll
+                for (int h = 0; h < 2; ++h) {
+                    const int row = rb + 8 * fg + 4 * h + q;
+                    const int chunk = (col >> 3) ^ tn_swz<T, CPI>(row);
+                    const char* ad = pb + (row * CPI + chunk) * 16 + (col & 7) * 2;
+                    s16x4 t = __builtin_amdgcn_ds_read_tr16_b64_v4i16((__attribute__((address_space(3))) s16x4*)(ad));
+                    u32x2 tt = __builtin_bit_cast(u32x2, t);
+                    w[2 * h] = tt.x; w[2 * h + 1] = tt.y;
+                }
+                pf[a] = u32x4{w[0], w[1], w[2], w[3]};
+            }
+#pragma unroll
+            for (int b = 0; b < FJ; ++b) {
+                const int col = wave_j * WJ + b * 16 + 4 * pp;
+                unsigned w[4];
+#pragma unroll
+                for (int h = 0; h < 2; ++h) {
+                    const int row = rb + 8 * fg + 4 * h + q;
+                    const int chunk = (col >> 3) ^ tn_swz<T, CPJ>(row);
+                    const char* ad = qb + (row * CPJ + chunk) * 16 + (col & 7) * 2;
+                    s16x4 t = __builtin_amdgcn_ds_read_tr16_b64_v4i16((__attribute__((address_space(3))) s16x4*)(ad));
+                    u32x2 tt = __builtin_bit_cast(u32x2, t);
+                    w[2 * h] = tt.x; w[2 * h + 1] = tt.y;
+                }
+                qf[b] = u32x4{w[0], w[1], w[2], w[3]};
+            }
+#pragma unroll
+            for (int a = 0; a < FI; ++a)
+#pragma unroll
+                for (int b = 0; b < FJ; ++b) Mma<T>::run(pf[a], qf[b], acc[a][b]);
+        }
+    };
+
+    if (nsteps > 0) {
+        dma_q(t_begin, 0);
+        if (half == 0) produce(t_begin, 0);
+    }
+    wait_vmcnt<0>();
+    __builtin_amdgcn_s_barrier();
+    for (int st = 0; st < nsteps; ++st) {
+        const int slot = st & 1;
+        if (st + 1 < nsteps) {
+            dma_q(t_begin + st + 1, slot ^ 1);
+            if (half == ((st + 1) & 1)) produce(t_begin + st + 1, slot ^ 1);
+        }
+        compute(slot);
+        wait_vmcnt<0>();
+        __builtin_amdgcn_s_barrier();
+    }
+
+    float* slab = p.slab + (long)lb * (BI * BJ);
+#pragma unroll
+    for (int a = 0; a < FI; ++a)
+#pragma unroll
+        for (int b = 0; b < FJ; ++b) *(f32x4*)(slab + ((((wave * FI + a) * FJ + b) * 64 + lane) << 2)) = acc[a][b];
+
+    float* sh = (float*)lds;
+    const int pl = tid >> 3;
+#pragma unroll
+    for (int e = 0; e < CE; ++e) { sh[(pl * 64 + c0 + e) * 2] = s1[e]; sh[(pl * 64 + c0 + e) * 2 + 1] = s2[e]; }
+    __syncthreads();
+    if (tid < 128) {
+        const int c = tid >> 1, which = tid & 1;
+        float t = 0.f;
+        for (int k = 0; k < 32; ++k) t += sh[(k * 64 + c) * 2 + which];
+        p.part[((long)lb * 2 + which) * 64 + c] = t;
+    }
+}
+
+template <typename T>
+__global__ __launch_bounds__(256) void stem_colsum_rows_kernel(const T* __restrict__ x4, float* __restrict__ rows, int XW, int Wy) {
+    __shared__ float sh[32][32];
+    const int t = threadIdx.x & 7, slice = threadIdx.x >> 3;
+    const T* src = x4 + (long)blockIdx.x * XW * 4;
+    float a[4] = {0.f, 0.f, 0.f, 0.f};
+    for (int ow = slice; ow < Wy; ow += 32) {
+        const u32x2 v = *(const u32x2*)(src + (long)(2 * ow + t) * 4);
+        const T* e = (const T*)&v;
+#pragma unroll
+        for (int ch = 0; ch < 4; ++ch) a[ch] += Elem<T>::to_f(e[ch]);
+    }
+#pragma unroll
+    for (int ch = 0; ch < 4; ++ch) sh[slice][t * 4 + ch] = a[ch];
+    __syncthreads();
+    if (threadIdx.x < 32) {
+        float s = 0.f;
+        for (int k = 0; k < 32; ++k) s += sh[k][threadIdx.x];
+        rows[(long)blockIdx.x * 32 + threadIdx.x] = s;
+    }
+}
+
+__global__ __launch_bounds__(1024) void stem_colsum_finish_kernel(const float* __restrict__ rows, float* __restrict__ s, int B, int XH, int Hy) {
+    __shared__ double sh[32][32];
+    const int r = blockIdx.x, tc = threadIdx.x & 31, slice = threadIdx.x >> 5;
+    const long n = (long)B * Hy;
+    double a = 0.0;
+    for (long i = slice; i < n; i += 32) {
+        const long b = i / Hy, oh = i - b * Hy;
+        a += (double)rows[(b * XH + 2 * oh + r) * 32 + tc];
+    }
+    sh[slice][tc] = a;
+    __syncthreads();
+    if (threadIdx.x < 32) {
+        double t = 0.0;
+        for (int k = 0; k < 32; ++k) t += sh[k][threadIdx.x];
+        s[r * 32 + threadIdx.x] = (float)t;
+    }
+}
+
+__global__ __launch_bounds__(256) void stem_wgrad_combine_kernel(const float* __restrict__ part, int nwg, const float* __restrict__ s1p,
+                                                                const float* __restrict__ s2p, const float* __restrict__ colsum,
+                                                                const float* __restrict__ mean, const float* __restrict__ invstd,
+                                                                const float* __restrict__ gamma, double count, float* __restrict__ dgamma,
+                                                                float* __restrict__ dbeta, float* __restrict__ c1c2, float* __restrict__ dw) {
+    __shared__ double sh[2][256];
+    const int c = blockIdx.x, tid = threadIdx.x;
+    double a = 0.0, b = 0.0;
+    for (int w = tid; w < nwg; w += 256) { a += (double)part[((long)w * 2) * 64 + c]; b += (double)part[((long)w * 2 + 1) * 64 + c]; }
+    sh[0][tid] = a; sh[1][tid] = b;
+    __syncthreads();
+    for (int o = 128; o > 0; o >>= 1) {
+        if (tid < o) { sh[0][tid] += sh[0][tid + o]; sh[1][tid] += sh[1][tid + o]; }
+        __syncthreads();
+    }
+    const double sum_dz = sh[0][0], sum_dzx = sh[1][0];
+    const double c1 = sum_dz / count, c2 = sum_dzx / count;
+    const double r = (double)invstd[c], g = (double)gamma[c], mu = (double)mean[c];
+    if (tid < 147) {
+        const int ch = tid / 49, kh = (tid % 49) / 7, kw = tid % 7;
+        const int j = (kh * 8 + kw) * 4 + ch;
+        const double A = g * r, Cp = -g * r * r * c2;
+        const double sj = (double)colsum[j];
+        dw[(long)c * 147 + tid] = (float)(A * ((double)s1p[c * 256 + j] - c1 * sj) + Cp * ((double)s2p[c * 256 + j] - mu * sj));
+    }
+    if (tid == 0) {
+        if (dbeta) dbeta[c] = (float)sum_dz;
+        if (dgamma) dgamma[c] = (float)sum_dzx;
+        c1c2[c] = (float)c1;
+        c1c2[64 + c] = (float)c2;
+    }
+}
+
+struct StemFoldPlan {
+    int Ho, Wo, np, tiles, tiles_per_wg, nwg;
+    long slab_floats, part_floats, bytes;
+};
+
+static int stem_fold_plan(int dtype, int B, int H, int W, StemFoldPlan& pl) {
+    if (dtype != RPE_BF16 && dtype != RPE_F16) return rpe_set_error(RPE_ERR_DTYPE, "stem_wgrad_dz: 16-bit element types only");
+    if (B <= 0 || H <= 0 || W <= 0 || ((H | W) & 1)) return rpe_set_error(RPE_ERR_SHAPE, "stem_wgrad_dz: H and W must be even");
+    const long np = (long)B * (H / 2) * (W / 2);
+    const long xh = 2L * H + 2 * RPE_STEM_PAD, xw = 2L * W + 2 * RPE_STEM_PAD;
+    if (np >= (1L << 27) || xh * xw * 4 >= (1L << 24))
+        return rpe_set_error(RPE_ERR_SHAPE, "stem_wgrad_dz: an image of 2^24 elements or more (offsets are built with 24-bit multiplies)");
+    pl.Ho = H / 2; pl.Wo = W / 2; pl.np = (int)np;
+    pl.tiles = (int)((np + kSfTilePx - 1) / kSfTilePx);
+    pl.tiles_per_wg = (pl.tiles + kSfTargetWgs - 1) / kSfTargetWgs;
+    pl.nwg = (pl.tiles + pl.tiles_per_wg - 1) / pl.tiles_per_wg;
+    const long span = ((long)pl.tiles_per_wg * kSfTilePx / ((long)pl.Ho * pl.Wo) + 2) * xh * xw * 4 * 2;
+    if (span >= (1L << 31)) return rpe_set_error(RPE_ERR_SHAPE, "stem_wgrad_dz: one workgroup's share of the images spans 2 GiB or more");
+    pl.slab_floats = (long)pl.nwg * 64 * 256;
+    pl.part_floats = (long)pl.nwg * 2 * 64;
+    pl.bytes = (pl.slab_floats + pl.part_floats + 64L * 256) * 4;
+    return 0;
+}
+
+template <typename T>
+static int stem_wgrad_dz_launch(const StemFoldPlan& pl, const void* dpool, const unsigned char* pidx, const StemAux& ax, const void* y, const float* scale,
+                                const float* shift, const float* mean, const float* invstd, const void* x4, int B, int H, int W, float* ws, hipStream_t s) {
+    StemFoldArgs<T> a;
+    memset(&a, 0, sizeof(a));
+    a.dpool = (const T*)dpool; a.pidx = pidx; a.ax = ax; a.y = (const T*)y; a.x4 = (const T*)x4;
+    a.scale = scale; a.shift = shift; a.mean = mean; a.invstd = invstd;
+    a.slab = ws; a.part = ws + pl.slab_floats;
+    a.B = B; a.H = H; a.W = W; a.Ho = pl.Ho; a.Wo = pl.Wo;
+    a.XW = 2 * W + 2 * RPE_STEM_PAD;
+    a.img_stride = (unsigned)((2L * H + 2 * RPE_STEM_PAD) * a.XW * 4);
+    a.x4_elems = (long)B * a.img_stride;
+    a.div_wo = make_fastdiv((unsigned)pl.Wo); a.div_ho = make_fastdiv((unsigned)pl.Ho);
+    a.np = pl.np; a.tiles = pl.tiles; a.tiles_per_wg = pl.tiles_per_wg; a.nwg = pl.nwg;
+    a.rev = walk_take();
+    note_kernel("stem_wgrad_dz_kernel");
+    hipLaunchKernelGGL((stem_wgrad_dz_kernel<T>), dim3((unsigned)pl.nwg), dim3(256), 0, s, a);
+    RPE_CHECK_LAUNCH();
+    return 0;
+}
+
+}
+
+using namespace rpe;
+
+extern "C" {
+
+long rpe_stem_wgrad_dz_workspace_bytes(int dtype, int B, int H, int W) {
+    StemFoldPlan pl;
+    return stem_fold_plan(dtype, B, H, W, pl) ? -1 : pl.bytes;
+}
+
+int rpe_stem_wgrad_dz_geometry(int dtype, int B, int H, int W, int* workgroups, int* tiles, int* tile_rows, int* tiles_per_workgroup) {
+    StemFoldPlan pl;
+    if (int e = stem_fold_plan(dtype, B, H, W, pl)) return e;
+    if (workgroups) *workgroups = pl.nwg;
+    if (tiles) *tiles = pl.tiles;
+    if (tile_rows) *tile_rows = kSfTileRows;
+    if (tiles_per_workgroup) *tiles_per_workgroup = pl.tiles_per_wg;
+    return 0;
+}
+
+int rpe_stem_wgrad_dz(int dtype, const void* dpool, const unsigned char* pool_idx, const void* y, const float* scale, const float* shift, const float* mean,
+                      const float* invstd, const float* aux_dout, long aux_ld, const float* aux_depth_feat, const unsigned char* aux_idx,
+                      const float* aux_w, const void* x4, int B, int H, int W, void* workspace, long workspace_bytes, void* stream) {
+    StemFoldPlan pl;
+    if (int e = stem_fold_plan(dtype, B, H, W, pl)) return e;
+    if (aux_dout && (!aux_idx || !aux_w)) return rpe_set_error(RPE_ERR_SHAPE, "stem_wgrad_dz: aux gradient needs its winner indices and weight");
+    if (!workspace || workspace_bytes < pl.bytes) return rpe_set_error(RPE_ERR_WORKSPACE, "stem_wgrad_dz: workspace smaller than rpe_stem_wgrad_dz_workspace_bytes()");
+    if ((((uintptr_t)workspace) | ((uintptr_t)x4) | ((uintptr_t)y) | ((uintptr_t)dpool)) & 15)
+        return rpe_set_error(RPE_ERR_ALIGN, "stem_wgrad_dz: operands and workspace must be 16-byte aligned");
+    const StemAux ax{aux_dout, aux_ld, aux_depth_feat, aux_idx, aux_w};
+    if (dtype == RPE_BF16) return stem_wgrad_dz_launch<bf16>(pl, dpool, pool_idx, ax, y, scale, shift, mean, invstd, x4, B, H, W, (float*)workspace, (hipStream_t)stream);
+    return stem_wgrad_dz_launch<f16>(pl, dpool, pool_idx, ax, y, scale, shift, mean, invstd, x4, B, H, W, (float*)workspace, (hipStream_t)stream);
+}
+
+long rpe_stem_im2col_colsum_workspace_bytes(int B, int H, int W) {
+    if (B <= 0 || H <= 0 || W <= 0 || ((H | W) & 1)) return -1;
+    return (long)B * (2L * H + 2 * RPE_STEM_PAD) * 32 * 4;
+}
+
+int rpe_stem_im2col_colsum(int dtype, const void* x4, float* colsum, int B, int H, int W, void* workspace, long workspace_bytes, void* stream) {
+    if (dtype != RPE_BF16 && dtype != RPE_F16) return rpe_set_error(RPE_ERR_DTYPE, "stem_im2col_colsum: 16-bit element types only");
+    const long need = rpe_stem_im2col_colsum_workspace_bytes(B, H, W);
+    if (need < 0) return rpe_set_error(RPE_ERR_SHAPE, "stem_im2col_colsum: H and W must be even");
+    if (!workspace || workspace_bytes < need) return rpe_set_error(RPE_ERR_WORKSPACE, "stem_im2col_colsum: workspace smaller than rpe_stem_im2col_colsum_workspace_bytes()");
+    const int XH = 2 * H + 2 * RPE_STEM_PAD, XW = 2 * W + 2 * RPE_STEM_PAD;
+    hipStream_t s = (hipStream_t)stream;
+    note_kernel("stem_colsum_rows_kernel");
+    if (dtype == RPE_BF16) hipLaunchKernelGGL((stem_colsum_rows_kernel<bf16>), dim3((unsigned)((long)B * XH)), dim3(256), 0, s, (const bf16*)x4, (float*)workspace, XW, W);
+    else hipLaunchKernelGGL((stem_colsum_rows_kernel<f16>), dim3((unsigned)((long)B * XH)), dim3(256), 0, s, (const f16*)x4, (float*)workspace, XW, W);
+    RPE_CHECK_LAUNCH();
+    prof_split(s, "stem_colsum_finish_kernel");
+    hipLaunchKernelGGL(stem_colsum_finish_kernel, dim3(8), dim3(1024), 0, s, (const float*)workspace, colsum, B, XH, H);
+    RPE_CHECK_LAUNCH();
+    return 0;
+}
+
+int rpe_stem_wgrad_combine(int dtype, void* workspace, long workspace_bytes, const float* s2_packed, const float* colsum, const float* mean,
+                           const float* invstd, const float* gamma, float* dgamma, float* dbeta, float* c1c2, float* dw_oihw, int B, int H, int W,
+                           void* stream) {
+    StemFoldPlan pl;
+    if (int e = stem_fold_plan(dtype, B, H, W, pl)) return e;
+    if (!workspace || workspace_bytes < pl.bytes) return rpe_set_error(RPE_ERR_WORKSPACE, "stem_wgrad_combine: workspace smaller than rpe_stem_wgrad_dz_workspace_bytes()");
+    hipStream_t s = (hipStream_t)stream;
+    float* ws = (float*)workspace;
+    float* s1p = ws + pl.slab_floats + pl.part_floats;
+    note_kernel("tn_reduce_kernel");
+    hipLaunchKernelGGL((tn_reduce_kernel<64, 256>), dim3(64), dim3(512), 0, s, (const float*)ws, s1p, 64, 256, 256, 1, 1, pl.nwg, 0);
+    RPE_CHECK_LAUNCH();
+    prof_split(s, "stem_wgrad_combine_kernel");
+    hipLaunchKernelGGL(stem_wgrad_combine_kernel, dim3(64), dim3(256), 0, s, (const float*)(ws + pl.slab_floats), pl.nwg, (const float*)s1p, s2_packed, colsum,
+                       mean, invstd, gamma, (double)B * H * W, dgamma, dbeta, c1c2, dw_oihw);
+    RPE_CHECK_LAUNCH();
+    return 0;
+}
+
+}
```

After: 14240 images/s. 0.966x the previous value.
